# mrluin/TextualDegRemoval

Hardware: AMD Instinct MI355X
Metric: train images/sec (512x512, bs=4/GPU) (higher is better)
Workload: dtype f32 (3xbf16-split MFMA: 24-bit operand significands on the full fp32 exponent range, fp32 accumulate; unscaled gradients, no loss scale, no step-skip guard; tensors fp32 -- the MASA-encoder ResidualBlock activations / gradients as three bf16 planes whose sum IS the fp32 value, bit for bit)

## Files before the change

### include/tdr.h

```cpp
#ifndef TDR_H
#define TDR_H
#include <stdint.h>
#ifdef __cplusplus
extern "C" {
#endif

#define TDR_ABI_VERSION 110
int tdr_version(void);
const char* tdr_last_error(void);

typedef struct TdrStepGuard {
    float scale, inv_scale, max_scale;
    int good, growth_interval;
    int step, skipped, finite;
    float bc1, bc2_sqrt;
} TdrStepGuard;

typedef struct TdrConvDesc {
    int N, Cin, H, W;
    int Cout, OH, OW;
    int KH, stride, dil, pad;
    const float* in;  int64_t in_ns;
    int gate;
    const float* kscale; int64_t kscale_ns;
    const void* wp;  int64_t wp_ns;  int Mpad;
    int wp_fmt;
    float* out; int64_t out_ns;
    int epi;
    const float* bias;  int64_t bias_ns;
    const float* scale; int64_t scale_ns;
    const float* bias2; int64_t bias2_ns; float bias2_mul;
    const float* res;   int64_t res_ns;
    const float* mask;  int64_t mask_ns;
    const float* aux;   int64_t aux_ns;
    int relu;
} TdrConvDesc;

int tdr_conv_forward(const TdrConvDesc* d, void* stream);

int tdr_conv_ck(int KH_eff);
int64_t tdr_packed_weight_floats(int M, int Kch, int KH_eff);
int tdr_pack_weights(const float* w, int Cout, int Cin, int KH, int mode, float* wp, void* stream);
int64_t tdr_packed_weight_bytes_bx3(int M, int Kch, int KH_eff);
int tdr_pack_weights_bx3(const float* w, int Cout, int Cin, int KH, int mode, void* wp, void* stream);
int tdr_pack_weights_bx3_batch(const float* w, int64_t w_stride, int B, int Cout, int Cin, int KH, int mode, void* wp,
                               void* stream);
int64_t tdr_packed_weight_bytes_hx2(int M, int Kch, int KH_eff);
int tdr_pack_weights_hx2(const float* w, int Cout, int Cin, int KH, int mode, void* wp, void* stream);
int tdr_conv_force_cfg(int kh, int cfg);
typedef struct TdrPackJob {
    const float* w; void* wp;
    int Cout, Cin, KH, mode, fmt;
    int M, Kch, KHe, CK, Mx;
    int64_t total;
    int64_t first_block;
} TdrPackJob;
int tdr_pack_job_init(TdrPackJob* job, const float* w, int Cout, int Cin, int KH, int mode, int fmt, void* wp);
int tdr_pack_weights_multi(const TdrPackJob* jobs_dev, int n_jobs, int64_t total_blocks, void* stream);
int tdr_pack_patches(const float* blk, int B, int G, int C, int BH, int BW, int PH, int PW, int pstep, int dil,
                     int off, float* wp, void* stream);

typedef struct TdrConvP16Desc {
    int N, Cin, H, W, Cout;
    const void* in;
    const void* wp; int Mpad; int wp_fmt;
    const float* bias;
    const float* res32;  int64_t res32_ns;
    const void*  res16;
    const float* mask32; int64_t mask32_ns;
    const void*  mask16;
    int relu;
    float* out32; int64_t out32_ns;
    void*  out16;
} TdrConvP16Desc;
int64_t tdr_p16_bytes(int N, int C, int H, int W);
int tdr_p16_from_f32(const float* src, int64_t src_ns, int N, int C, int H, int W, void* dst, void* stream);
int tdr_p16_to_f32(const void* src, int N, int C, int H, int W, float* dst, int64_t dst_ns, void* stream);
int64_t tdr_p16_bytes_fmt(int N, int C, int H, int W, int fmt);
int tdr_p16_from_f32_fmt(const float* src, int64_t src_ns, int N, int C, int H, int W, void* dst, int fmt, void* stream);
int tdr_p16_to_f32_fmt(const void* src, int N, int C, int H, int W, float* dst, int64_t dst_ns, int fmt, void* stream);
int tdr_conv3x3_p16(const TdrConvP16Desc* d, void* stream);
int tdr_conv3x3_p16_force_cfg(int cfg);
typedef struct TdrWgradP16Desc {
    int N, Cin, H, W, Cout;
    const void* in16;
    const void* dout16;
    float* g;
    float* db;
    float* ws; int64_t ws_floats;
    int fmt;
} TdrWgradP16Desc;
int64_t tdr_wgrad3x3_p16_ws_floats(const TdrWgradP16Desc* d);
int tdr_wgrad3x3_p16(const TdrWgradP16Desc* d, void* stream);

typedef struct TdrWgradDesc {
    int N, Cin, H, W, Cout, OH, OW, KH, stride, pad;
    const float* in;   int64_t in_ns;  int gate;
    const float* dout; int64_t dout_ns;
    float* g;
    float* db;
    int per_image;
    float* ws; int64_t ws_floats;
    int math;
} TdrWgradDesc;
int64_t tdr_wgrad_ws_floats(const TdrWgradDesc* d);
int tdr_conv_wgrad(const TdrWgradDesc* d, void* stream);

typedef struct TdrWg1GroupEntry {
    const float* in; const float* dout; float* part; float* dbpart; float* g; float* db;
} TdrWg1GroupEntry;
int tdr_wgrad1x1_group_supported(const TdrWgradDesc* d);
int64_t tdr_wgrad1x1_group_ws_floats(const TdrWgradDesc* d, int nprob);
int tdr_wgrad1x1_group(const TdrWgradDesc* d, int nprob, const void* table, void* stream);

int64_t tdr_wgrad3x3_p16_group_ws_floats(const TdrWgradP16Desc* d, int nprob);
int tdr_wgrad3x3_p16_group_plan(const TdrWgradP16Desc* d, int nprob, int* nsplit, int* units, int* units_per_wg);
int tdr_wgrad3x3_p16_group(const TdrWgradP16Desc* d, int nprob, const void* table, void* stream);

int tdr_layernorm2d_fwd(const float* x, int64_t x_ns, const float* w, const float* b, float eps, int center,
                        int N, int C, int HW, float* y, float* mu, float* rstd, void* stream);
int64_t tdr_ln_ws_floats(int N, int C, int HW);
int tdr_layernorm2d_bwd(const float* go, const float* x, int64_t x_ns, const float* mu, const float* rstd,
                        const float* w, const float* add, int64_t add_ns, int add_C, int center,
                        int N, int C, int HW, float* gx, float* gw, float* gb, float* ws, void* stream);

int64_t tdr_dwsg_ws_floats(int N, int C, int H, int W);
int tdr_dwsg_fwd(const float* t, const float* w, const float* b, int N, int C, int H, int W,
                 float* g, float* pooled, float* ws, void* stream);
int tdr_dwsg_bwd(const float* dg, const float* t, const float* w, const float* b, int N, int C, int H, int W,
                 float* dt, float* dw, float* db, float* ws, void* stream);
int tdr_dwsg_bwd_biased(const float* dg, const float* dg_bias, float dg_bias_mul, const float* t, const float* w, const float* b,
                        int N, int C, int H, int W, float* dt, float* dw, float* db, float* ws, void* stream);
int tdr_dwsg_bwd_parts_supported(int W);
int tdr_dw_param_finish(const float* ws, int N, int C, int H, int W, float* dw , float* db , void* stream);

int tdr_dwgelu_fwd(const float* t, const float* w, const float* b, int N, int C, int H, int W, float* g, void* stream);
int tdr_dwgelu_bwd(const float* dg, const float* t, const float* w, const float* b, int N, int C, int H, int W,
                   float* dt, float* dw, float* db, float* ws, void* stream);
int tdr_dwconv_fwd(const float* t, const float* w, const float* b, int N, int planes, int H, int W, float* out,
                   void* stream);
int tdr_dwconv_bwd(const float* dout, const float* t, const float* w, int N, int planes, int H, int W, float* dt,
                   float* dw, float* db, float* ws, void* stream);
int tdr_dwconv_act_fwd(const float* t, const float* w, const float* b, int N, int planes, int H, int W, int relu, float* out,
                       void* stream);
int tdr_dwconv_act_bwd(const float* dout, const float* act, const float* t, const float* w, int N, int planes, int H, int W,
                       float* dt, float* dw, float* db, float* ws, void* stream);
int tdr_dwpair_fwd(const float* t, const float* w, const float* b, int N, int C, int H, int W, int relu, float* out,
                   int64_t out_ns, void* stream);
int tdr_dwpair_bwd(const float* dout, int64_t dout_ns, const float* act, int64_t act_ns, const float* t, const float* w, int N,
                   int C, int H, int W, float* dt, float* dw, float* db, float* ws, void* stream);
int tdr_dwconv_halves_fwd(const float* t, const float* w, const float* b, int N, int planes, int H, int W, int relu, float* outA,
                          float* outB, int64_t out_ns, void* stream);
int tdr_dwconv_halves_bwd(const float* doutA, const float* doutB, int64_t dout_ns, const float* actA, const float* actB,
                          int64_t act_ns, const float* t, const float* w, int N, int planes, int H, int W, float* dt, float* dw,
                          float* db, float* ws, void* stream);

int tdr_row_sumsq(const float* x, int64_t x_ns, int N, int rows, int HW, float* out, void* stream);
int tdr_mdta_pad(int C);
int tdr_mdta_softmax(const float* G, const float* ss, const float* temp, int N, int C, int heads, float* A, float* AT,
                     void* stream);
int tdr_mdta_bwd(const float* G, const float* ss, const float* temp, const float* A, const float* dA, int N, int C,
                 int heads, float* W, float* dtemp, float* ws, void* stream);
int tdr_attn_fold_proj(const float* AT, const float* Wo, int N, int C, int heads, float* Wf, void* stream);
int tdr_axpby_dev(const float* a, const float* alpha, const float* b, int64_t numel, float* out, void* stream);
int tdr_dot(const float* a, const float* b, int64_t numel, float* out, float* ws, void* stream);
int tdr_pixel_shuffle2(const float* in, int N, int C, int H, int W, float* out, void* stream);

int tdr_sca_fwd(const float* pooled, const float* wsca, const float* bsca, int N, int C, float* s, void* stream);
int tdr_sca_bwd(const float* G3, const float* S3, const float* w3, const float* b3, const float* beta,
                const float* s, const float* pooled, const float* wsca, int N, int C,
                float* dw3, float* db3, float* dbeta, float* dwsca, float* dbsca, float* dpooled,
                float* ws , void* stream);
int tdr_scaled_conv_param_grads(const float* G, const float* S, const float* w, const float* b,
                                const float* gamma, int Cout, int Cin, float* dw, float* db, float* dgamma,
                                void* stream);

int64_t tdr_chansum_ws_floats(int N, int C, int HW);
int tdr_channel_sum(const float* x, int64_t x_ns, int N, int C, int HW, float* out, float* ws, void* stream);

int tdr_copy_rows(const float* src, int64_t src_ns, float* dst, int64_t dst_ns, int N, int64_t len, void* stream);
int tdr_add_rows(const float* src, int64_t src_ns, float* dst, int64_t dst_ns, int N, int64_t len, void* stream);
int tdr_pixel_unshuffle2(const float* in, int N, int C, int H, int W, float* out, void* stream);
int tdr_pad_crop(const float* src, int N, int C, int Hs, int Ws, float* dst, int Hd, int Wd, void* stream);
int tdr_crop_augment(const float* src, int64_t src_ns, int N, int C, int Hs, int Ws, const int* top, const int* left,
                     const int* mode, const float* noise, const float* sigma, int P, float* out, void* stream);

int64_t tdr_ssim3d_ws_floats(int H, int W);
int tdr_ssim3d(const float* img1, const float* img2, int H, int W, int C, float max_value, float* ws, float* out,
// ... 309 lines not shown
```

### textualdegremoval_amd/_lib.py

```python
import ctypes as C
import os

import torch

_HERE = os.path.dirname(os.path.abspath(__file__))
LIB_PATH = os.environ.get('TDR_LIB_PATH', os.path.join(_HERE, 'libtdr_hip.so'))

ABI_VERSION = 110
c_fp = C.c_void_p
i32, i64, f32 = C.c_int, C.c_int64, C.c_float


class TdrConvDesc(C.Structure):
    _fields_ = [
        ('N', i32), ('Cin', i32), ('H', i32), ('W', i32),
        ('Cout', i32), ('OH', i32), ('OW', i32),
        ('KH', i32), ('stride', i32), ('dil', i32), ('pad', i32),
        ('inp', c_fp), ('in_ns', i64),
        ('gate', i32),
        ('kscale', c_fp), ('kscale_ns', i64),
        ('wp', c_fp), ('wp_ns', i64), ('Mpad', i32), ('wp_fmt', i32),
        ('out', c_fp), ('out_ns', i64),
        ('epi', i32),
        ('bias', c_fp), ('bias_ns', i64),
        ('scale', c_fp), ('scale_ns', i64),
        ('bias2', c_fp), ('bias2_ns', i64), ('bias2_mul', f32),
        ('res', c_fp), ('res_ns', i64),
        ('mask', c_fp), ('mask_ns', i64),
        ('aux', c_fp), ('aux_ns', i64),
        ('relu', i32),
    ]


class TdrConvP16Desc(C.Structure):
    _fields_ = [
        ('N', i32), ('Cin', i32), ('H', i32), ('W', i32), ('Cout', i32),
        ('inp', c_fp),
        ('wp', c_fp), ('Mpad', i32), ('wp_fmt', i32),
        ('bias', c_fp),
        ('res32', c_fp), ('res32_ns', i64),
        ('res16', c_fp),
        ('mask32', c_fp), ('mask32_ns', i64),
        ('mask16', c_fp),
        ('relu', i32),
        ('out32', c_fp), ('out32_ns', i64),
        ('out16', c_fp),
    ]


class TdrWgradP16Desc(C.Structure):
    _fields_ = [('N', i32), ('Cin', i32), ('H', i32), ('W', i32), ('Cout', i32),
                ('in16', c_fp), ('dout16', c_fp), ('g', c_fp), ('db', c_fp), ('ws', c_fp), ('ws_floats', i64), ('fmt', i32)]


class TdrPackJob(C.Structure):
    _fields_ = [
        ('w', c_fp), ('wp', c_fp),
        ('Cout', i32), ('Cin', i32), ('KH', i32), ('mode', i32), ('fmt', i32),
        ('M', i32), ('Kch', i32), ('KHe', i32), ('CK', i32), ('Mx', i32),
        ('total', i64), ('first_block', i64),
    ]


class TdrWgradDesc(C.Structure):
    _fields_ = [
        ('N', i32), ('Cin', i32), ('H', i32), ('W', i32), ('Cout', i32), ('OH', i32), ('OW', i32),
        ('KH', i32), ('stride', i32), ('pad', i32),
        ('inp', c_fp), ('in_ns', i64), ('gate', i32),
        ('dout', c_fp), ('dout_ns', i64),
        ('g', c_fp),
        ('db', c_fp),
        ('per_image', i32),
        ('ws', c_fp), ('ws_floats', i64),
        ('math', i32),
    ]


class TdrNafTailDesc(C.Structure):
    _fields_ = [('N', i32), ('C', i32), ('HW', i32), ('w_fmt', i32), ('c_out', i32), ('eps', f32),
                ('g', c_fp), ('g_ns', i64), ('sca', c_fp), ('x', c_fp), ('x_ns', i64),
                ('w3', c_fp), ('w4', c_fp), ('w5', c_fp),
                ('b3', c_fp), ('beta', c_fp), ('lnw', c_fp), ('lnb', c_fp), ('b4', c_fp), ('b5', c_fp), ('gamma', c_fp),
                ('y', c_fp), ('y_ns', i64), ('mu', c_fp), ('rs', c_fp), ('yn', c_fp), ('yn_ns', i64),
                ('t4', c_fp), ('t4_ns', i64), ('out', c_fp), ('out_ns', i64)]


class TdrNafTailBwdDesc(C.Structure):
    _fields_ = [('N', i32), ('C', i32), ('HW', i32), ('w_fmt', i32), ('c_out', i32),
                ('dout', c_fp), ('dout_ns', i64), ('gamma', c_fp), ('t4', c_fp), ('t4_ns', i64), ('y', c_fp), ('y_ns', i64),
                ('mu', c_fp), ('rs', c_fp), ('lnw', c_fp), ('w5t', c_fp), ('w4t', c_fp),
                ('dt4', c_fp), ('dt4_ns', i64), ('dy', c_fp), ('dy_ns', i64), ('gw', c_fp), ('gb', c_fp), ('ws', c_fp),
                ('w3t', c_fp), ('beta', c_fp), ('sca', c_fp), ('dgp', c_fp), ('dgp_ns', i64)]


class TdrNafHeadBwdDesc(C.Structure):
    _fields_ = [('N', i32), ('C', i32), ('HW', i32), ('w_fmt', i32),
                ('dt1', c_fp), ('dt1_ns', i64), ('x', c_fp), ('x_ns', i64), ('mu', c_fp), ('rs', c_fp), ('lnw', c_fp),
                ('w1t', c_fp), ('res', c_fp), ('res_ns', i64), ('dx', c_fp), ('dx_ns', i64), ('gw', c_fp), ('gb', c_fp), ('ws', c_fp)]


class TdrNafHeadFwdDesc(C.Structure):
    _fields_ = [('N', i32), ('C', i32), ('HW', i32), ('w_fmt', i32),
                ('x', c_fp), ('x_ns', i64), ('lnw', c_fp), ('lnb', c_fp), ('eps', f32), ('w1', c_fp), ('b1', c_fp),
                ('mu', c_fp), ('rs', c_fp), ('xn', c_fp), ('xn_ns', i64), ('t1', c_fp), ('t1_ns', i64)]


class TdrSfDynVecDesc(C.Structure):
    _fields_ = [('N', i32), ('c', i32), ('GK', i32), ('KK', i32), ('d', i32), ('eps', f32), ('momentum', f32)] + \
               [(k, c_fp) for k in ('ap', 'wconv', 'bn_w', 'bn_b', 'fc_w', 'fc_b', 'f0_w', 'f0_b', 'f1_w', 'f1_b', 'run_mean', 'run_var', 'nbt',
                                    'taps', 'ah', 'al', 'xhat', 'rstd', 'z', 'att')] + [('use_running', i32)]


class TdrSfDynVecBwdDesc(C.Structure):
    _fields_ = [('N', i32), ('c', i32), ('GK', i32), ('KK', i32), ('d', i32)] + \
               [(k, c_fp) for k in ('ap', 'wconv', 'bn_w', 'fc_w', 'f0_w', 'f1_w', 'taps', 'xhat', 'rstd', 'z', 'att', 'dtaps', 'dah', 'dal',
                                    'dap', 'g_wconv', 'g_bn_w', 'g_bn_b', 'g_fc_w', 'g_fc_b', 'g_f0_w', 'g_f0_b', 'g_f1_w', 'g_f1_b', 'ws')]


class TdrStepGuard(C.Structure):
    _fields_ = [('scale', f32), ('inv_scale', f32), ('max_scale', f32), ('good', i32), ('growth_interval', i32),
                ('step', i32), ('skipped', i32), ('finite', i32), ('bc1', f32), ('bc2_sqrt', f32)]


SIGNATURES = {
    'tdr_version': (i32, []),
    'tdr_last_error': (C.c_char_p, []),
    'tdr_conv_forward': (i32, [C.POINTER(TdrConvDesc), c_fp]),
    'tdr_conv_ck': (i32, [i32]),
    'tdr_ssim_y64_ws_doubles': (i64, [i32, i32]),
    'tdr_ssim_y64': (i32, [c_fp, c_fp, i32, i32, c_fp, c_fp, c_fp]),
    'tdr_local_avgpool_ws_floats': (i64, [i32, i32, i32, i32]),
    'tdr_local_avgpool': (i32, [c_fp, i32, i32, i32, i32, i32, c_fp, c_fp, c_fp]),
    'tdr_p16_bytes': (i64, [i32, i32, i32, i32]),
    'tdr_p16_bytes_fmt': (i64, [i32, i32, i32, i32, i32]),
    'tdr_p16_from_f32_fmt': (i32, [c_fp, i64, i32, i32, i32, i32, c_fp, i32, c_fp]),
    'tdr_p16_to_f32_fmt': (i32, [c_fp, i32, i32, i32, i32, c_fp, i64, i32, c_fp]),
    'tdr_p16_from_f32': (i32, [c_fp, i64, i32, i32, i32, i32, c_fp, c_fp]),
    'tdr_p16_to_f32': (i32, [c_fp, i32, i32, i32, i32, c_fp, i64, c_fp]),
    'tdr_conv3x3_p16': (i32, [C.POINTER(TdrConvP16Desc), c_fp]),
    'tdr_conv3x3_p16_force_cfg': (i32, [i32]),
    'tdr_wgrad3x3_p16_ws_floats': (i64, [C.POINTER(TdrWgradP16Desc)]),
    'tdr_wgrad3x3_p16': (i32, [C.POINTER(TdrWgradP16Desc), c_fp]),
    'tdr_packed_weight_floats': (i64, [i32, i32, i32]),
    'tdr_pack_weights': (i32, [c_fp, i32, i32, i32, i32, c_fp, c_fp]),
    'tdr_packed_weight_bytes_bx3': (i64, [i32, i32, i32]),
    'tdr_pack_weights_bx3': (i32, [c_fp, i32, i32, i32, i32, c_fp, c_fp]),
    'tdr_pack_job_init': (i32, [C.POINTER(TdrPackJob), c_fp, i32, i32, i32, i32, i32, c_fp]),
    'tdr_pack_weights_multi': (i32, [c_fp, i32, i64, c_fp]),
    'tdr_pack_patches': (i32, [c_fp, i32, i32, i32, i32, i32, i32, i32, i32, i32, i32, c_fp, c_fp]),
    'tdr_wgrad_ws_floats': (i64, [C.POINTER(TdrWgradDesc)]),
    'tdr_conv_wgrad': (i32, [C.POINTER(TdrWgradDesc), c_fp]),
    'tdr_wgrad1x1_group_supported': (i32, [C.POINTER(TdrWgradDesc)]),
    'tdr_wgrad1x1_group_ws_floats': (i64, [C.POINTER(TdrWgradDesc), i32]),
    'tdr_wgrad1x1_group': (i32, [C.POINTER(TdrWgradDesc), i32, c_fp, c_fp]),
    'tdr_wgrad3x3_p16_group_ws_floats': (i64, [C.POINTER(TdrWgradP16Desc), i32]),
    'tdr_wgrad3x3_p16_group_plan': (i32, [C.POINTER(TdrWgradP16Desc), i32, C.POINTER(i32), C.POINTER(i32), C.POINTER(i32)]),
    'tdr_wgrad3x3_p16_group': (i32, [C.POINTER(TdrWgradP16Desc), i32, c_fp, c_fp]),
    'tdr_layernorm2d_fwd': (i32, [c_fp, i64, c_fp, c_fp, f32, i32, i32, i32, i32, c_fp, c_fp, c_fp, c_fp]),
    'tdr_ln_ws_floats': (i64, [i32, i32, i32]),
    'tdr_layernorm2d_bwd': (i32, [c_fp, c_fp, i64, c_fp, c_fp, c_fp, c_fp, i64, i32, i32, i32, i32, i32, c_fp, c_fp, c_fp,
                                  c_fp, c_fp]),
    'tdr_dwsg_ws_floats': (i64, [i32, i32, i32, i32]),
    'tdr_dwsg_fwd': (i32, [c_fp, c_fp, c_fp, i32, i32, i32, i32, c_fp, c_fp, c_fp, c_fp]),
    'tdr_dwsg_bwd': (i32, [c_fp, c_fp, c_fp, c_fp, i32, i32, i32, i32, c_fp, c_fp, c_fp, c_fp, c_fp]),
    'tdr_dwsg_bwd_biased': (i32, [c_fp, c_fp, f32, c_fp, c_fp, c_fp, i32, i32, i32, i32, c_fp, c_fp, c_fp, c_fp, c_fp]),
    'tdr_dwsg_bwd_parts_supported': (i32, [i32]),
    'tdr_dw_param_finish': (i32, [c_fp, i32, i32, i32, i32, c_fp, c_fp, c_fp]),
    'tdr_dwgelu_fwd': (i32, [c_fp, c_fp, c_fp, i32, i32, i32, i32, c_fp, c_fp]),
    'tdr_dwgelu_bwd': (i32, [c_fp, c_fp, c_fp, c_fp, i32, i32, i32, i32, c_fp, c_fp, c_fp, c_fp, c_fp]),
    'tdr_dwconv_fwd': (i32, [c_fp, c_fp, c_fp, i32, i32, i32, i32, c_fp, c_fp]),
    'tdr_dwconv_act_fwd': (i32, [c_fp, c_fp, c_fp, i32, i32, i32, i32, i32, c_fp, c_fp]),
    'tdr_dwconv_act_bwd': (i32, [c_fp, c_fp, c_fp, c_fp, i32, i32, i32, i32, c_fp, c_fp, c_fp, c_fp, c_fp]),
    'tdr_dwpair_fwd': (i32, [c_fp, c_fp, c_fp, i32, i32, i32, i32, i32, c_fp, i64, c_fp]),
    'tdr_dwpair_bwd': (i32, [c_fp, i64, c_fp, i64, c_fp, c_fp, i32, i32, i32, i32, c_fp, c_fp, c_fp, c_fp, c_fp]),
    'tdr_dwconv_halves_fwd': (i32, [c_fp, c_fp, c_fp, i32, i32, i32, i32, i32, c_fp, c_fp, i64, c_fp]),
    'tdr_dwconv_halves_bwd': (i32, [c_fp, c_fp, i64, c_fp, c_fp, i64, c_fp, c_fp, i32, i32, i32, i32, c_fp, c_fp, c_fp, c_fp, c_fp]),
    'tdr_dwconv_bwd': (i32, [c_fp, c_fp, c_fp, i32, i32, i32, i32, c_fp, c_fp, c_fp, c_fp, c_fp]),
    'tdr_row_sumsq': (i32, [c_fp, i64, i32, i32, i32, c_fp, c_fp]),
    'tdr_mdta_pad': (i32, [i32]),
    'tdr_mdta_softmax': (i32, [c_fp, c_fp, c_fp, i32, i32, i32, c_fp, c_fp, c_fp]),
    'tdr_mdta_bwd': (i32, [c_fp, c_fp, c_fp, c_fp, c_fp, i32, i32, i32, c_fp, c_fp, c_fp, c_fp]),
    'tdr_attn_fold_proj': (i32, [c_fp, c_fp, i32, i32, i32, c_fp, c_fp]),
    'tdr_axpby_dev': (i32, [c_fp, c_fp, c_fp, i64, c_fp, c_fp]),
# ... 192 lines not shown
```

### textualdegremoval_amd/csrc/tdr_conv_bx3.hip

```cpp
#include <stdlib.h>
#include "tdr_common.h"
#include "tdr_conv_epi.h"
#include "tdr_pack.h"
#include "../../include/tdr.h"

typedef __bf16 bf16x8 __attribute__((ext_vector_type(8)));


namespace {

constexpr int bx_cmax(int a, int b) { return a > b ? a : b; }
constexpr int bx_plane(int NT, int TW, int KH, int S) {
    return (((NT * 32 / TW) - 1) * S + KH) * ((TW - 1) * S + KH);
}
constexpr int bx_max_plane(int NT, int KH, int S) {
    return bx_cmax(bx_plane(NT, 8, KH, S), bx_cmax(bx_plane(NT, 16, KH, S), bx_plane(NT, 32, KH, S)));
}

__device__ __forceinline__ void split3(float x, __bf16& h, __bf16& m, __bf16& l) {
    h = (__bf16)x;
    const float r = x - (float)h;
    m = (__bf16)r;
    l = (__bf16)(r - (float)m);
}

typedef _Float16 f16x8 __attribute__((ext_vector_type(8)));
union Frag {
    uint4 u;
    bf16x8 v;
    f16x8 hv;
};

enum { SCH_BX3 = 0, SCH_HX2 = 1, SCH_H1 = 2 };

#ifndef TDR_CONV_OCC
#define TDR_CONV_OCC 4
#endif
template <int KH, int S, int WM, int TM, int TN, int EPI, bool GATE, int SCH, int AD = 0>
__global__ __launch_bounds__(256, (KH == 3 && S == 1 && WM == 1 && TM == 1 && TN == 2 && AD != 9) ? TDR_CONV_OCC : ((KH == 3 && S == 1 && WM == 2 && TM == 1 && TN == 4 && AD == 3) ? 3 : 2)) void conv_bx3_kernel(ConvArgs a) {
    constexpr int NS = SCH == SCH_BX3 ? 3 : (SCH == SCH_HX2 ? 2 : 1);
    constexpr int NSW = SCH == SCH_BX3 ? 3 : 2;
    constexpr int NP = SCH == SCH_BX3 ? 6 : (SCH == SCH_HX2 ? 3 : 1);
    constexpr int WN = 4 / WM;
    constexpr int BM = 32 * TM * WM;
    constexpr int NT = TN * WN;
    constexpr int TAPS = KH * KH;
    constexpr int NIT = (bx_max_plane(NT, KH, S) + 127) / 128;
    constexpr int PF = (KH == 1) ? 2 : 1;
    static_assert(AD == 0 || (KH == 3 && 9 % AD == 0), "ring depth must divide the 9 taps");

    extern __shared__ __attribute__((aligned(16))) uint4 smem4[];

    const int tid = threadIdx.x, lane = tid & 63, wave = __builtin_amdgcn_readfirstlane(tid >> 6);
    const int wm = wave / WN, wn = wave % WN;
    const int j = lane & 31, kk = lane >> 5;
    const int TW = 1 << a.tw_log2, SR = 32 >> a.tw_log2, TH = NT * SR;
    const int LH = (TH - 1) * S + KH, LW = (TW - 1) * S + KH;
    const int plane = LH * LW;
    int logical;
    {
        const int T = gridDim.x, b = blockIdx.x;
        const int q = T >> 3, r = T & 7, xcd = b & 7, slot = b >> 3;
        logical = (xcd < r ? xcd * (q + 1) : r * (q + 1) + (xcd - r) * q) + slot;
    }
    const int mtile = logical % a.mtiles, ptile = logical / a.mtiles;
    const int tx = ptile % a.tiles_x, ty = ptile / a.tiles_x;
    const int m0 = mtile * BM;
    const int n = blockIdx.z;
    const int oy0 = ty * TH, ox0 = tx * TW;
    const int iy0 = oy0 * S - a.pad, ix0 = ox0 * S - a.pad;
    const long HWin = (long)a.H * a.W;

    const int sg = wave >> 1;
    const int sp0 = (wave & 1) * 64 + lane;
    int gsafe[NIT];
    unsigned okmask = 0, inplane = 0;
#pragma unroll
    for (int it = 0; it < NIT; ++it) {
        const int p = sp0 + 128 * it;
        const int r = p / LW, x = p - r * LW;
        const int gy = iy0 + r, gx = ix0 + x;
        const bool inp = p < plane;
        const bool ok = inp && gy >= 0 && gy < a.H && gx >= 0 && gx < a.W;
        gsafe[it] = ok ? gy * a.W + gx : 0;
        okmask |= (ok ? 1u : 0u) << it;
        inplane |= (inp ? 1u : 0u) << it;
    }
    const float* in_n = a.in + (long)n * a.in_ns;
    const float* ks_n = a.kscale ? a.kscale + (long)n * a.kscale_ns : nullptr;
    const int ngroups = (a.Cin + 15) >> 4;

    float rin[PF][NIT][8];
    float rin2[GATE ? PF : 1][GATE ? NIT : 1][GATE ? 8 : 1];
    float rks[PF][8];
    auto load_group = [&](int g, int set) {
#pragma unroll
        for (int i = 0; i < 8; ++i) {
            const int ci = min(g * 16 + sg * 8 + i, a.Cin - 1);
            const float* base = in_n + (long)ci * HWin;
            rks[set][i] = ks_n ? ks_n[ci] : 1.f;
#pragma unroll
            for (int it = 0; it < NIT; ++it) {
                rin[set][it][i] = base[gsafe[it]];
                if (GATE) rin2[set][it][i] = base[gsafe[it] + a.gate_off];
            }
        }
    };
    auto store_group = [&](int g, int set, int buf) {
        uint4* sb = smem4 + (buf * (2 * NS) + sg) * plane;
        const int cbase = g * 16 + sg * 8;
#pragma unroll
        for (int it = 0; it < NIT; ++it) {
            Frag h, m, l;
            const bool ok = (okmask >> it) & 1u;
            float vv[8];
#pragma unroll
            for (int i = 0; i < 8; ++i) {
                float v = rin[set][it][i];
                if (GATE) v *= rin2[set][it][i];
                v *= rks[set][i];
                vv[i] = (ok && cbase + i < a.Cin) ? v : 0.f;
            }
            if constexpr (SCH == SCH_HX2) {
                unsigned hd[4], md[4];
#pragma unroll
                for (int i = 0; i < 4; ++i) tdr_split2_f16(vv[2 * i], vv[2 * i + 1], hd[i], md[i]);
                h.u = make_uint4(hd[0], hd[1], hd[2], hd[3]);
                m.u = make_uint4(md[0], md[1], md[2], md[3]);
            } else {
#pragma unroll
                for (int i = 0; i < 8; ++i) {
                    float v = vv[i];
                    asm volatile("" : "+v"(v));
                    if constexpr (SCH == SCH_H1) {
                        h.hv[i] = (_Float16)v;
                    } else {
                        __bf16 hh, mm, ll;
                        split3(v, hh, mm, ll);
                        h.v[i] = hh; m.v[i] = mm; l.v[i] = ll;
                    }
                }
            }
            if ((inplane >> it) & 1u) {
                const int p = sp0 + 128 * it;
                sb[p] = h.u;
                if constexpr (NS >= 2) sb[2 * plane + p] = m.u;
                if constexpr (NS == 3) sb[4 * plane + p] = l.u;
            }
        }
    };

    int bbase[TN];
#pragma unroll
    for (int tn = 0; tn < TN; ++tn) {
        const int t = wn * TN + tn;
        const int py = t * SR + (j >> a.tw_log2), px = j & (TW - 1);
        bbase[tn] = kk * plane + py * S * LW + px * S;
    }
    const int MT = a.Mpad >> 5;
    const uint4* wfrag[TM];
#pragma unroll
    for (int tm = 0; tm < TM; ++tm) {
        const int mt = min((m0 >> 5) + wm * TM + tm, MT - 1);
        wfrag[tm] = reinterpret_cast<const uint4*>(a.wp) + (long)n * (a.wp_ns >> 2) + (long)mt * (NSW * 64) + lane;
    }
    const long wstep = (long)MT * (NSW * 64);

    f32x16 acc[TM][TN];
#pragma unroll
    for (int tm = 0; tm < TM; ++tm)
#pragma unroll
        for (int tn = 0; tn < TN; ++tn)
#pragma unroll
            for (int r = 0; r < 16; ++r) acc[tm][tn][r] = 0.f;

    Frag af[TM][NS], afn[TM][NS];
    Frag aq[AD > 0 ? AD : 1][TM][NS];
    auto load_a = [&](Frag (&dst)[TM][NS], long gt) {
#pragma unroll
        for (int tm = 0; tm < TM; ++tm)
#pragma unroll
            for (int s = 0; s < NS; ++s) dst[tm][s].u = wfrag[tm][gt * wstep + s * 64];
    };

    if constexpr (AD > 0) {
#pragma unroll
        for (int d = 0; d < AD; ++d) load_a(aq[d], min((long)d, (long)ngroups * TAPS - 1));
    } else {
        load_a(af, 0);
    }
#pragma unroll
    for (int p = 0; p < PF; ++p)
        if (p < ngroups) load_group(p, p);
    store_group(0, 0, 0);
    __syncthreads();

    for (int g0 = 0; g0 < ngroups; g0 += PF) {
#pragma unroll
        for (int u = 0; u < PF; ++u) {
            const int g = g0 + u;
            if (g < ngroups) {
                const int buf = a.single_buf ? 0 : (g & 1);
                const uint4* sb = smem4 + buf * (2 * NS) * plane;
                constexpr int IGT = (PF == 1 && KH == 3 && AD > 0 && AD < TAPS) ? TAPS - AD : -1;
                if (PF == 1 && IGT < 0 && g + 1 < ngroups) load_group(g + 1, 0);
#pragma unroll
                for (int tap = 0; tap < TAPS; ++tap) {
                    const int tapoff = (tap / KH) * LW + (tap % KH);
                    if (tap == IGT && g + 1 < ngroups) {
                        load_group(g + 1, 0);
                        __builtin_amdgcn_sched_barrier(0);
                    }
                    const long gtn = min((long)g * TAPS + tap + 1, (long)ngroups * TAPS - 1);
                    if (AD == 0) load_a(afn, gtn);
                    Frag (&afc)[TM][NS] = AD > 0 ? aq[AD > 0 ? tap % (AD > 0 ? AD : 1) : 0] : af;
                    if (PF > 1 && tap == 0 && g + PF < ngroups) load_group(g + PF, u);
                    Frag bf[TN][NS];
#pragma unroll
                    for (int tn = 0; tn < TN; ++tn)
#pragma unroll
                        for (int s = 0; s < NS; ++s) bf[tn][s].u = sb[s * 2 * plane + bbase[tn] + tapoff];
                    constexpr int SA[6] = {2, 0, 1, 1, 0, 0}, SB[6] = {0, 2, 1, 0, 1, 0};
                    constexpr int HA[3] = {1, 0, 0}, HB[3] = {0, 1, 0};
#pragma unroll
                    for (int q = 0; q < NP; ++q)
#pragma unroll
                        for (int tm = 0; tm < TM; ++tm)
#pragma unroll
                            for (int tn = 0; tn < TN; ++tn) {
                                if constexpr (SCH == SCH_H1)
                                    acc[tm][tn] = __builtin_amdgcn_mfma_f32_32x32x16_f16(afc[tm][0].hv, bf[tn][0].hv, acc[tm][tn], 0, 0, 0);
                                else if constexpr (SCH == SCH_HX2)
                                    acc[tm][tn] = __builtin_amdgcn_mfma_f32_32x32x16_f16(afc[tm][HA[q]].hv, bf[tn][HB[q]].hv, acc[tm][tn], 0, 0, 0);
                                else
                                    acc[tm][tn] = __builtin_amdgcn_mfma_f32_32x32x16_bf16(afc[tm][SA[q]].v, bf[tn][SB[q]].v, acc[tm][tn], 0, 0, 0);
                            }
                    if constexpr (AD > 0) {
                        load_a(aq[tap % (AD > 0 ? AD : 1)], min((long)g * TAPS + tap + AD, (long)ngroups * TAPS - 1));
                    } else {
#pragma unroll
                        for (int tm = 0; tm < TM; ++tm)
#pragma unroll
                            for (int s = 0; s < NS; ++s) af[tm][s] = afn[tm][s];
                    }
                }
                {
                    if (a.single_buf) __syncthreads();
                    if (g + 1 < ngroups) store_group(g + 1, (u + 1) % PF, a.single_buf ? 0 : (buf ^ 1));
                    __syncthreads();
                }
            }
        }
    }

    if constexpr (EPI != EPI_PSHUF) {
        if (a.vec_epi) {
            __syncthreads();
            conv_epilogue_vec<TM, TN, EPI>(a, acc, n, m0, wm, wn, oy0, ox0, lane, reinterpret_cast<float*>(smem4) + wave * (32 * 36));
            return;
        }
    }
    conv_epilogue<TM, TN, EPI>(a, acc, n, m0, wm, wn, oy0, ox0, j, kk);
}

__device__ __forceinline__ int swz1(int slot) { return slot ^ ((slot >> 4) & 3); }

template <int WM, int TM, int TN, int EPI, bool GATE, int SCH = SCH_HX2>
__global__ __launch_bounds__(256, 2) void conv1x1_hx2_kernel(ConvArgs a) {
    constexpr int NS = SCH == SCH_H1 ? 1 : 2, NSW = 2, NP = SCH == SCH_H1 ? 1 : 3;
    constexpr int WN = 4 / WM;
    constexpr int BM = 32 * TM * WM;
    constexpr int NT = TN * WN;
    constexpr int NPX = 32 * NT;
    constexpr int QUADS = NPX / 4;
    constexpr int OCT = 256 / QUADS;
    constexpr int KS = 8 * OCT;
    constexpr int GPS = KS / 16;
    constexpr int PFD = GATE ? 1 : 2;

    extern __shared__ __attribute__((aligned(16))) uint4 smem4[];

    const int tid = threadIdx.x, lane = tid & 63, wave = __builtin_amdgcn_readfirstlane(tid >> 6);
    const int wm = wave / WN, wn = wave % WN;
    const int j = lane & 31, kk = lane >> 5;
    const int TW = 1 << a.tw_log2, SR = 32 >> a.tw_log2, TH = NT * SR;
    int logical;
    {
        const int T = gridDim.x, b = blockIdx.x;
        const int q = T >> 3, r = T & 7, xcd = b & 7, slot = b >> 3;
        logical = (xcd < r ? xcd * (q + 1) : r * (q + 1) + (xcd - r) * q) + slot;
    }
    const int mtile = logical % a.mtiles, ptile = logical / a.mtiles;
    const int tx = ptile % a.tiles_x, ty = ptile / a.tiles_x;
    const int m0 = mtile * BM;
    const int n = blockIdx.z;
    const int oy0 = ty * TH, ox0 = tx * TW;
    const long HWin = (long)a.H * a.W;

    const int so = tid / QUADS, sq = tid % QUADS;
    const int p0 = 4 * sq;
    const int gy = oy0 + (p0 >> a.tw_log2), gx = ox0 + (p0 & (TW - 1));
    const bool pok = gy < a.H && gx < a.W;
    const long goff = pok ? (long)gy * a.W + gx : 0;
    const float* in_n = a.in + (long)n * a.in_ns;
    const float* ks_n = a.kscale ? a.kscale + (long)n * a.kscale_ns : nullptr;
    const int ngroups = (a.Cin + 15) >> 4;
    const int nstages = (a.Cin + KS - 1) / KS;

    float4 rin[PFD][8];
    float4 rin2[GATE ? PFD : 1][GATE ? 8 : 1];
    float rks[PFD][8];
    auto load_stage = [&](int st, int set) {
        const int cbase = st * KS + so * 8;
#pragma unroll
        for (int i = 0; i < 8; ++i) {
            const int ci = cbase + i;
            rin[set][i] = make_float4(0.f, 0.f, 0.f, 0.f);
            rks[set][i] = 1.f;
            if (GATE) rin2[set][i] = make_float4(0.f, 0.f, 0.f, 0.f);
            if (pok && ci < a.Cin) {
                const float* src = in_n + (long)ci * HWin + goff;
                rin[set][i] = *reinterpret_cast<const float4*>(src);
                if (GATE) rin2[set][i] = *reinterpret_cast<const float4*>(src + a.gate_off);
                if (ks_n) rks[set][i] = ks_n[ci];
            }
        }
    };
    int wslot[4];
#pragma unroll
    for (int i = 0; i < 4; ++i) wslot[i] = so * NPX + swz1(p0 + i);
    auto store_stage = [&](int set, int buf) {
        uint4* sb = smem4 + buf * (NS * OCT * NPX);
#pragma unroll
        for (int px = 0; px < 4; ++px) {
            Frag h, m;
            float vv[8];
#pragma unroll
            for (int i = 0; i < 8; ++i) {
                const float4 q4 = rin[set][i];
                float v = px == 0 ? q4.x : (px == 1 ? q4.y : (px == 2 ? q4.z : q4.w));
                if (GATE) {
                    const float4 g4 = rin2[set][i];
                    v *= px == 0 ? g4.x : (px == 1 ? g4.y : (px == 2 ? g4.z : g4.w));
                }
                vv[i] = v * rks[set][i];
            }
            if constexpr (NS == 2) {
                unsigned hd[4], md[4];
#pragma unroll
                for (int i = 0; i < 4; ++i) tdr_split2_f16(vv[2 * i], vv[2 * i + 1], hd[i], md[i]);
                h.u = make_uint4(hd[0], hd[1], hd[2], hd[3]);
                m.u = make_uint4(md[0], md[1], md[2], md[3]);
            } else {
#pragma unroll
                for (int i = 0; i < 8; ++i) h.hv[i] = (_Float16)vv[i];
            }
            sb[wslot[px]] = h.u;
            if constexpr (NS == 2) sb[OCT * NPX + wslot[px]] = m.u;
        }
    };

    int bslot[TN];
#pragma unroll
    for (int tn = 0; tn < TN; ++tn) bslot[tn] = kk * NPX + swz1(32 * (wn * TN + tn) + j);
    const int MT = a.Mpad >> 5;
    const uint4* wfrag[TM];
#pragma unroll
    for (int tm = 0; tm < TM; ++tm) {
        const int mt = min((m0 >> 5) + wm * TM + tm, MT - 1);
        wfrag[tm] = reinterpret_cast<const uint4*>(a.wp) + (long)n * (a.wp_ns >> 2) + (long)mt * (NSW * 64) + lane;
    }
    const long wstep = (long)MT * (NSW * 64);

    f32x16 acc[TM][TN];
#pragma unroll
    for (int tm = 0; tm < TM; ++tm)
#pragma unroll
        for (int tn = 0; tn < TN; ++tn)
#pragma unroll
            for (int r = 0; r < 16; ++r) acc[tm][tn][r] = 0.f;

    Frag af[TM][NS], afn[TM][NS];
    auto load_a = [&](Frag (&dst)[TM][NS], long g) {
#pragma unroll
        for (int tm = 0; tm < TM; ++tm)
#pragma unroll
            for (int s = 0; s < NS; ++s) dst[tm][s].u = wfrag[tm][g * wstep + s * 64];
    };

    load_a(af, 0);
#pragma unroll
    for (int p = 0; p < PFD; ++p)
        if (p < nstages) load_stage(p, p);
    store_stage(0, 0);
    __syncthreads();

    for (int s0 = 0; s0 < nstages; s0 += PFD) {
#pragma unroll
        for (int u = 0; u < PFD; ++u) {
            const int st = s0 + u;
            if (st < nstages) {
                const int buf = st & 1;
                const uint4* sb = smem4 + buf * (NS * OCT * NPX);
#pragma unroll
                for (int gg = 0; gg < GPS; ++gg) {
                    const int g = st * GPS + gg;
                    if (g < ngroups) {
                        load_a(afn, min(g + 1, ngroups - 1));
                        if (gg == 0 && st + PFD < nstages) load_stage(st + PFD, u);
                        Frag bf[TN][NS];
#pragma unroll
                        for (int tn = 0; tn < TN; ++tn)
#pragma unroll
                            for (int s = 0; s < NS; ++s) bf[tn][s].u = sb[s * (OCT * NPX) + 2 * gg * NPX + bslot[tn]];
                        constexpr int HA[3] = {1, 0, 0}, HB[3] = {0, 1, 0};
#pragma unroll
                        for (int q = 0; q < NP; ++q)
#pragma unroll
                            for (int tm = 0; tm < TM; ++tm)
#pragma unroll
                                for (int tn = 0; tn < TN; ++tn) {
                                    if constexpr (SCH == SCH_H1)
                                        acc[tm][tn] = __builtin_amdgcn_mfma_f32_32x32x16_f16(af[tm][0].hv, bf[tn][0].hv, acc[tm][tn], 0, 0, 0);
                                    else
                                        acc[tm][tn] = __builtin_amdgcn_mfma_f32_32x32x16_f16(af[tm][HA[q]].hv, bf[tn][HB[q]].hv, acc[tm][tn], 0, 0, 0);
                                }
#pragma unroll
                        for (int tm = 0; tm < TM; ++tm)
#pragma unroll
                            for (int s = 0; s < NS; ++s) af[tm][s] = afn[tm][s];
                    }
                }
                if (st + 1 < nstages) store_stage((u + 1) % PFD, buf ^ 1);
                __syncthreads();
            }
        }
    }

    if constexpr (EPI != EPI_PSHUF) {
        if (a.vec_epi) {
            conv_epilogue_vec<TM, TN, EPI>(a, acc, n, m0, wm, wn, oy0, ox0, lane, reinterpret_cast<float*>(smem4) + wave * (32 * 36));
            return;
        }
    }
    conv_epilogue<TM, TN, EPI>(a, acc, n, m0, wm, wn, oy0, ox0, j, kk);
}

template <int WM, int TM, int TN, int EPI, bool GATE, int SCH>
int launch_c1_hx2(const ConvArgs& a, int N, hipStream_t st) {
    constexpr int WN = 4 / WM;
    constexpr int BM = 32 * TM * WM;
    constexpr int NT = TN * WN;
    const int TW = 1 << a.tw_log2, SR = 32 >> a.tw_log2, TH = NT * SR;
    ConvArgs b = a;
    b.tiles_x = tdr_cdiv(a.OW, TW);
    const int tiles_y = tdr_cdiv(a.OH, TH);
    b.mtiles = tdr_cdiv(a.Cout, BM);
    dim3 grid(b.tiles_x * tiles_y * b.mtiles, 1, N);
    b.single_buf = 0;
    const size_t lds = 2 * 32768;
    auto kern = conv1x1_hx2_kernel<WM, TM, TN, EPI, GATE, SCH>;
    static bool attr_set = false;
    if (!attr_set) {
        (void)hipFuncSetAttribute(reinterpret_cast<const void*>(kern), hipFuncAttributeMaxDynamicSharedMemorySize, 160 * 1024);
        attr_set = true;
    }
    hipLaunchKernelGGL(kern, grid, dim3(256), lds, st, b);
    TDR_LAUNCH_CHECK("conv1x1_hx2_kernel");
    return TDR_OK;
}

inline bool c1_hx2_ok(const ConvArgs& a, int npx, int bm, int N) {
    static const bool off = tdr_tune_env("TDR_C1_OLD") != nullptr;
    static const int min_stages = tdr_tune_env("TDR_C1_STAGES") ? atoi(tdr_tune_env("TDR_C1_STAGES")) : 4;
    static const long max_blocks = tdr_tune_env("TDR_C1_BLOCKS") ? atol(tdr_tune_env("TDR_C1_BLOCKS")) : 512;
    const int ks = 8192 / npx;
    const long blocks = (long)tdr_cdiv((long)a.OH * a.OW, npx) * tdr_cdiv(a.Cout, bm) * N;
    return !off && blocks <= max_blocks && (a.Cin + ks - 1) / ks >= min_stages && a.pad == 0 && a.W % 4 == 0 && a.in_ns % 4 == 0 && (reinterpret_cast<uintptr_t>(a.in) & 15) == 0 &&
           a.H == a.OH && a.W == a.OW;
}

template <int KH, int S, int WM, int TM, int TN, int EPI, bool GATE, int SCH>
int launch_bx_cfg_s(const ConvArgs& a, int N, hipStream_t st) {
    if constexpr (KH == 1 && S == 1 && SCH != SCH_BX3 && EPI != EPI_PSHUF)
        if (c1_hx2_ok(a, 32 * TN * (4 / WM), 32 * TM * WM, N)) return launch_c1_hx2<WM, TM, TN, EPI, GATE, SCH>(a, N, st);
    constexpr int NS = SCH == SCH_BX3 ? 3 : (SCH == SCH_HX2 ? 2 : 1);
    constexpr int WN = 4 / WM;
    constexpr int BM = 32 * TM * WM;
    constexpr int NT = TN * WN;
    const int TW = 1 << a.tw_log2, SR = 32 >> a.tw_log2, TH = NT * SR;
    const int LH = (TH - 1) * S + KH, LW = (TW - 1) * S + KH;
    ConvArgs b = a;
    static const int single_env = tdr_tune_env("TDR_BX_SINGLE") ? atoi(tdr_tune_env("TDR_BX_SINGLE")) : 2;
    b.single_buf = (KH == 3 && (a.Cin + 15) / 16 <= single_env) ? 1 : 0;
    size_t lds = (size_t)(b.single_buf ? 1 : 2) * (2 * NS) * LH * LW * 16;
    if (lds < 4 * 32 * 36 * sizeof(float)) lds = 4 * 32 * 36 * sizeof(float);
    b.tiles_x = tdr_cdiv(a.OW, TW);
    const int tiles_y = tdr_cdiv(a.OH, TH);
    b.mtiles = tdr_cdiv(a.Cout, BM);
    dim3 grid(b.tiles_x * tiles_y * b.mtiles, 1, N);
    if constexpr (KH == 3 && S == 1 && SCH == SCH_HX2 && EPI == EPI_STD && !GATE) {
        static const int ring3 = tdr_tune_env("TDR_RING3") ? atoi(tdr_tune_env("TDR_RING3")) : 1;
        static const long ring_blocks3 = tdr_tune_env("TDR_RING_BLOCKS") ? atol(tdr_tune_env("TDR_RING_BLOCKS")) : 512;
        if (ring3 && ((long)grid.x * N > ring_blocks3 || TM != 1)) {
            auto kern = conv_bx3_kernel<KH, S, WM, TM, TN, EPI, GATE, SCH, 3>;
            static bool attr_set = false;
            if (!attr_set) {
                (void)hipFuncSetAttribute(reinterpret_cast<const void*>(kern), hipFuncAttributeMaxDynamicSharedMemorySize, 160 * 1024);
                attr_set = true;
            }
            hipLaunchKernelGGL(kern, grid, dim3(256), lds, st, b);
            TDR_LAUNCH_CHECK("conv_bx3_kernel(ring3)");
            return TDR_OK;
        }
    }
    if constexpr (KH == 3 && S == 1 && TM == 1 && SCH == SCH_HX2 && EPI == EPI_STD) {
        static const long ring_blocks = tdr_tune_env("TDR_RING_BLOCKS") ? atol(tdr_tune_env("TDR_RING_BLOCKS")) : 512;
        if ((long)grid.x * N <= ring_blocks) {
            auto kern = conv_bx3_kernel<KH, S, WM, TM, TN, EPI, GATE, SCH, 9>;
            static bool attr_set = false;
            if (!attr_set) {
                (void)hipFuncSetAttribute(reinterpret_cast<const void*>(kern), hipFuncAttributeMaxDynamicSharedMemorySize, 160 * 1024);
                attr_set = true;
            }
            hipLaunchKernelGGL(kern, grid, dim3(256), lds, st, b);
            TDR_LAUNCH_CHECK("conv_bx3_kernel(ring)");
            return TDR_OK;
        }
    }
    auto kern = conv_bx3_kernel<KH, S, WM, TM, TN, EPI, GATE, SCH>;
    static bool attr_set = false;
    if (!attr_set) {
        (void)hipFuncSetAttribute(reinterpret_cast<const void*>(kern), hipFuncAttributeMaxDynamicSharedMemorySize, 160 * 1024);
        attr_set = true;
    }
    hipLaunchKernelGGL(kern, grid, dim3(256), lds, st, b);
    TDR_LAUNCH_CHECK("conv_bx3_kernel");
    return TDR_OK;
}

int g_force_cfg[2] = {tdr_tune_env("TDR_BX_CFG1") ? atoi(tdr_tune_env("TDR_BX_CFG1")) : 0, tdr_tune_env("TDR_BX_CFG3") ? atoi(tdr_tune_env("TDR_BX_CFG3")) : 0};

template <int KH, int S, int WM, int TM, int TN, int EPI, bool GATE>
int launch_bx_cfg(const ConvArgs& a, int N, hipStream_t st) {
    if (a.scheme == SCH_HX2) return launch_bx_cfg_s<KH, S, WM, TM, TN, EPI, GATE, SCH_HX2>(a, N, st);
    if (a.scheme == SCH_H1) return launch_bx_cfg_s<KH, S, WM, TM, TN, EPI, GATE, SCH_H1>(a, N, st);
    return launch_bx_cfg_s<KH, S, WM, TM, TN, EPI, GATE, SCH_BX3>(a, N, st);
}

template <int KH, int S, int EPI, bool GATE>
int launch_bx_shape(const ConvArgs& a, int N, hipStream_t st) {
    const long pix = (long)a.OH * a.OW;
    auto blocks = [&](int bm, int bn) { return (long)tdr_cdiv(a.Cout, bm) * tdr_cdiv(pix, bn) * N; };
    if constexpr (S == 2) {
        if (a.Cout <= 32) return launch_bx_cfg<KH, S, 1, 1, 1, EPI, GATE>(a, N, st);
        if (a.Cout <= 64 || blocks(128, 64) < 512) return launch_bx_cfg<KH, S, 2, 1, 1, EPI, GATE>(a, N, st);
        return launch_bx_cfg<KH, S, 2, 2, 1, EPI, GATE>(a, N, st);
    } else {
        if (a.Cout <= 32) {
            if (blocks(32, 256) >= 512) return launch_bx_cfg<KH, S, 1, 1, 2, EPI, GATE>(a, N, st);
            return launch_bx_cfg<KH, S, 1, 1, 1, EPI, GATE>(a, N, st);
        }
        if (g_force_cfg[KH == 1 ? 0 : 1] == 0 && a.scheme == SCH_BX3 && a.Cin <= (KH == 1 ? 128 : 64) && blocks(64, 128) >= 2048)
            return launch_bx_cfg<KH, S, 2, 1, 2, EPI, GATE>(a, N, st);
        if constexpr (KH == 1) {
            const int force = g_force_cfg[0];
            if (force == 1) return launch_bx_cfg<KH, S, 2, 2, 2, EPI, GATE>(a, N, st);
            if (force == 2) return launch_bx_cfg<KH, S, 2, 1, 4, EPI, GATE>(a, N, st);
            if (force == 3) return launch_bx_cfg<KH, S, 2, 1, 2, EPI, GATE>(a, N, st);
            if (force == 4) return launch_bx_cfg<KH, S, 1, 1, 2, EPI, GATE>(a, N, st);
            if (force == 5) return launch_bx_cfg<KH, S, 4, 2, 2, EPI, GATE>(a, N, st);
            if (a.Cout > 64 && blocks(128, 128) >= 512) return launch_bx_cfg<KH, S, 2, 2, 2, EPI, GATE>(a, N, st);
            if (a.Cin >= 768 && a.Cout >= 256 && blocks(256, 64) >= 256 && blocks(256, 64) <= 512)
                return launch_bx_cfg<KH, S, 4, 2, 2, EPI, GATE>(a, N, st);
        } else {
            const int force3 = g_force_cfg[1];
            if (force3 == 1) return launch_bx_cfg<KH, S, 2, 2, 4, EPI, GATE>(a, N, st);
            if (force3 == 2) return launch_bx_cfg<KH, S, 2, 1, 4, EPI, GATE>(a, N, st);
            if (force3 == 3) return launch_bx_cfg<KH, S, 2, 1, 2, EPI, GATE>(a, N, st);
            if (force3 == 4) return launch_bx_cfg<KH, S, 2, 2, 2, EPI, GATE>(a, N, st);
            const bool tall_ok = blocks(128, 256) >= 1024 || a.Cout % 128 != 0 || a.scheme != SCH_HX2;
            if (a.Cout > 64 && blocks(128, 256) >= 512 && tall_ok) return launch_bx_cfg<KH, S, 2, 2, 4, EPI, GATE>(a, N, st);
        }
        if (blocks(64, 256) >= 512) return launch_bx_cfg<KH, S, 2, 1, 4, EPI, GATE>(a, N, st);
        return launch_bx_cfg<KH, S, 2, 1, 2, EPI, GATE>(a, N, st);
    }
}

__global__ void pack_weights_bx3_kernel(const float* __restrict__ w, long w_bs, int Cout, int Cin, int KH, int mode, int M,
                                        int Kch, int KHe, int MT, long total, uint4* __restrict__ wp, long wp_bs16) {
    const float* wb = w + (long)blockIdx.y * w_bs;
    uint4* ob = wp + (long)blockIdx.y * wp_bs16;
    for (long i = blockIdx.x * (long)blockDim.x + threadIdx.x; i < total; i += (long)gridDim.x * blockDim.x)
        tdr_pack_bx3_frag(wb, Cin, KH, mode, M, Kch, KHe, MT, i, ob);
}

__global__ void pack_weights_hx2_kernel(const float* __restrict__ w, int Cout, int Cin, int KH, int mode, int M, int Kch, int KHe,
                                        int MT, long total, uint4* __restrict__ wp) {
    for (long i = blockIdx.x * (long)blockDim.x + threadIdx.x; i < total; i += (long)gridDim.x * blockDim.x)
        tdr_pack_hx2_frag(w, Cin, KH, mode, M, Kch, KHe, MT, i, wp);
}

}

extern "C" int tdr_conv_force_cfg(int kh, int cfg) {
    g_force_cfg[kh == 1 ? 0 : 1] = cfg;
    return TDR_OK;
}

extern "C" int64_t tdr_packed_weight_bytes_bx3(int M, int Kch, int KH_eff) {
    const long MT = (M + 31) / 32;
    return (long)((Kch + 15) / 16) * KH_eff * KH_eff * MT * 3 * 1024;
}

extern "C" int tdr_pack_weights_bx3(const float* w, int Cout, int Cin, int KH, int mode, void* wp, void* stream) {
    TDR_REQUIRE(w && wp, "tdr_pack_weights_bx3: null pointer");
    TDR_REQUIRE(mode >= 0 && mode <= 3, "tdr_pack_weights_bx3: bad mode %d", mode);
    int M, Kch, KHe;
    if (mode == 0) { M = Cout; Kch = Cin; KHe = KH; }
    else if (mode == 1) { M = Cin; Kch = Cout; KHe = KH; }
    else if (mode == 2) { TDR_REQUIRE(KH == 2, "mode 2 needs a 2x2 kernel"); M = 4 * Cin; Kch = Cout; KHe = 1; }
    else { TDR_REQUIRE(KH == 3, "mode 3 needs a 3x3 kernel"); M = 4 * Cin; Kch = Cout; KHe = 2; }
    const int MT = (M + 31) / 32;
    const long total = (long)((Kch + 15) / 16) * KHe * KHe * MT * 64;
    const int blocks = (int)((total + 255) / 256 < 4096 ? (total + 255) / 256 : 4096);
    hipLaunchKernelGGL(pack_weights_bx3_kernel, dim3(blocks), dim3(256), 0, (hipStream_t)stream, w, 0L, Cout, Cin, KH, mode, M,
                       Kch, KHe, MT, total, (uint4*)wp, 0L);
    TDR_LAUNCH_CHECK("pack_weights_bx3_kernel");
    return TDR_OK;
}

extern "C" int64_t tdr_packed_weight_bytes_hx2(int M, int Kch, int KH_eff) {
    const long MT = (M + 31) / 32;
    return (long)((Kch + 15) / 16) * KH_eff * KH_eff * MT * 2 * 1024;
}

extern "C" int tdr_pack_weights_hx2(const float* w, int Cout, int Cin, int KH, int mode, void* wp, void* stream) {
    TDR_REQUIRE(w && wp, "tdr_pack_weights_hx2: null pointer");
    TDR_REQUIRE(mode >= 0 && mode <= 3, "tdr_pack_weights_hx2: bad mode %d", mode);
    int M, Kch, KHe;
    if (mode == 0) { M = Cout; Kch = Cin; KHe = KH; }
    else if (mode == 1) { M = Cin; Kch = Cout; KHe = KH; }
    else if (mode == 2) { TDR_REQUIRE(KH == 2, "mode 2 needs a 2x2 kernel"); M = 4 * Cin; Kch = Cout; KHe = 1; }
    else { TDR_REQUIRE(KH == 3, "mode 3 needs a 3x3 kernel"); M = 4 * Cin; Kch = Cout; KHe = 2; }
    const int MT = (M + 31) / 32;
    const long total = (long)((Kch + 15) / 16) * KHe * KHe * MT * 64;
    const int blocks = (int)((total + 255) / 256 < 4096 ? (total + 255) / 256 : 4096);
    hipLaunchKernelGGL(pack_weights_hx2_kernel, dim3(blocks), dim3(256), 0, (hipStream_t)stream, w, Cout, Cin, KH, mode, M, Kch,
                       KHe, MT, total, (uint4*)wp);
    TDR_LAUNCH_CHECK("pack_weights_hx2_kernel");
    return TDR_OK;
}

extern "C" int tdr_pack_weights_bx3_batch(const float* w, int64_t w_stride, int B, int Cout, int Cin, int KH, int mode, void* wp,
                                          void* stream) {
    TDR_REQUIRE(w && wp && B > 0, "tdr_pack_weights_bx3_batch: bad argument");
    TDR_REQUIRE(mode == 0 || mode == 1, "tdr_pack_weights_bx3_batch: mode 0 or 1 only (got %d)", mode);
    const int M = mode == 0 ? Cout : Cin, Kch = mode == 0 ? Cin : Cout;
    const int MT = (M + 31) / 32;
    const long total = (long)((Kch + 15) / 16) * KH * KH * MT * 64;
    const long per_b16 = tdr_packed_weight_bytes_bx3(M, Kch, KH) / 16;
    const int blocks = (int)((total + 255) / 256 < 1024 ? (total + 255) / 256 : 1024);
    hipLaunchKernelGGL(pack_weights_bx3_kernel, dim3(blocks, B), dim3(256), 0, (hipStream_t)stream, w, (long)w_stride, Cout, Cin,
                       KH, mode, M, Kch, KH, MT, total, (uint4*)wp, per_b16);
    TDR_LAUNCH_CHECK("pack_weights_bx3_kernel(batch)");
    return TDR_OK;
}

int tdr_conv_forward_bx3(const TdrConvDesc* d, void* stream) {
    TDR_REQUIRE(d->dil == 1 && d->wp_ns % 4 == 0, "tdr_conv_forward: split-bf16 path needs dil=1 (and wp_ns a multiple of 4 floats)");
    ConvArgs a;
    a.in = d->in; a.in_ns = d->in_ns; a.Cin = d->Cin; a.H = d->H; a.W = d->W;
    a.wp = (const float*)d->wp; a.wp_ns = d->wp_ns; a.Mpad = d->Mpad; a.Cout = d->Cout;
    a.scheme = d->wp_fmt == 3 ? SCH_H1 : (d->wp_fmt == 2 ? SCH_HX2 : SCH_BX3);
    a.out = d->out; a.out_ns = d->out_ns; a.OH = d->OH; a.OW = d->OW;
    a.pad = d->pad;
    a.tw_log2 = d->OW >= 24 ? 5 : (d->OW >= 12 ? 4 : 3);
    a.tiles_x = 0;
    a.kscale = d->kscale; a.kscale_ns = d->kscale_ns;
    a.gate_off = (long)d->Cin * d->H * d->W;
    a.bias = d->bias; a.bias_ns = d->bias_ns; a.scale = d->scale; a.scale_ns = d->scale_ns;
    a.bias2 = d->bias2; a.bias2_ns = d->bias2_ns; a.bias2_mul = d->bias2_mul;
    a.res = d->res; a.res_ns = d->res_ns; a.mask = d->mask; a.mask_ns = d->mask_ns;
    a.aux = d->aux; a.aux_ns = d->aux_ns; a.relu = d->relu;
    auto al16 = [](const void* p) { return (reinterpret_cast<uintptr_t>(p) & 15) == 0; };
    a.vec_epi = (d->OW % 4 == 0 && d->out_ns % 4 == 0 && al16(d->out) && (!d->res || (d->res_ns % 4 == 0 && al16(d->res))) &&
                 (!d->mask || (d->mask_ns % 4 == 0 && al16(d->mask))) && (!d->aux || (d->aux_ns % 4 == 0 && al16(d->aux)))) ? 1 : 0;
    hipStream_t st = (hipStream_t)stream;
    const int N = d->N;
    const int key = d->KH * 100 + d->stride * 10 + d->epi;
    const bool g = d->gate != 0;
    switch (key) {
        case 110: return g ? launch_bx_shape<1, 1, EPI_STD, true>(a, N, st) : launch_bx_shape<1, 1, EPI_STD, false>(a, N, st);
        case 111: if (!g) return launch_bx_shape<1, 1, EPI_GATEBWD, false>(a, N, st); break;
        case 112: if (!g) return launch_bx_shape<1, 1, EPI_PSHUF, false>(a, N, st); break;
        case 310: if (!g) return launch_bx_shape<3, 1, EPI_STD, false>(a, N, st); break;
        case 312: if (!g) return launch_bx_shape<3, 1, EPI_PSHUF, false>(a, N, st); break;
        case 320: if (!g) return launch_bx_shape<3, 2, EPI_STD, false>(a, N, st); break;
        case 220: if (!g) return launch_bx_shape<2, 2, EPI_STD, false>(a, N, st); break;
        case 212: if (!g) return launch_bx_shape<2, 1, EPI_PSHUF, false>(a, N, st); break;
        default: break;
    }
    tdr_set_error("tdr_conv_forward(bx3): unsupported (KH=%d stride=%d epi=%d gate=%d)", d->KH, d->stride, d->epi, d->gate);
    return TDR_ERR_UNSUPPORTED;
}
```

### textualdegremoval_amd/csrc/tdr_conv_epi.h

```cpp
#pragma once
#include "tdr_common.h"

namespace {

enum { EPI_STD = 0, EPI_GATEBWD = 1, EPI_PSHUF = 2 };

struct ConvArgs {
    const float* in; long in_ns; int Cin, H, W;
    const float* wp; long wp_ns; int Mpad, Cout;
    float* out; long out_ns; int OH, OW;
    int pad, tw_log2, tiles_x, mtiles;
    const float* kscale; long kscale_ns;
    long gate_off;
    const float* bias; long bias_ns;
    const float* scale; long scale_ns;
    const float* bias2; long bias2_ns; float bias2_mul;
    const float* res; long res_ns;
    const float* mask; long mask_ns;
    const float* aux; long aux_ns;
    int relu;
    int vec_epi;
    int single_buf;
    int scheme;
};

template <int TM, int TN, int EPI>
__device__ __forceinline__ void conv_epilogue(const ConvArgs& a, f32x16 (&acc)[TM][TN], int n, int m0, int wm, int wn,
                                              int oy0, int ox0, int j, int kk) {
    const int TW = 1 << a.tw_log2, SR = 32 >> a.tw_log2;
    const long HWo = (long)a.OH * a.OW;
#pragma unroll
    for (int tn = 0; tn < TN; ++tn) {
        const int t = wn * TN + tn;
        const int oy = oy0 + t * SR + (j >> a.tw_log2), ox = ox0 + (j & (TW - 1));
        const bool pvalid = oy < a.OH && ox < a.OW;
        const long pix = pvalid ? (long)oy * a.OW + ox : 0;
#pragma unroll
        for (int tm = 0; tm < TM; ++tm) {
            const int mb = m0 + (wm * TM + tm) * 32 + 4 * kk;
            if (EPI == EPI_PSHUF) {
                const long OW2 = 2L * a.OW;
                const long p2 = pvalid ? (2L * oy) * OW2 + 2L * ox : 0;
                float2 r0[4], r1[4];
                if (a.res) {
#pragma unroll
                    for (int q = 0; q < 4; ++q) {
                        const int c = min(mb + 8 * q, a.Cout - 4) >> 2;
                        const float* rp = a.res + (long)n * a.res_ns + (long)c * 4 * HWo + p2;
                        r0[q] = *reinterpret_cast<const float2*>(rp);
                        r1[q] = *reinterpret_cast<const float2*>(rp + OW2);
                    }
                }
#pragma unroll
                for (int q = 0; q < 4; ++q) {
                    const int m = mb + 8 * q;
                    float v0 = acc[tm][tn][4 * q + 0], v1 = acc[tm][tn][4 * q + 1];
                    float v2 = acc[tm][tn][4 * q + 2], v3 = acc[tm][tn][4 * q + 3];
                    if (a.res) { v0 += r0[q].x; v1 += r0[q].y; v2 += r1[q].x; v3 += r1[q].y; }
                    if (pvalid && m < a.Cout) {
                        float* o = a.out + (long)n * a.out_ns + (long)(m >> 2) * 4 * HWo + p2;
                        *reinterpret_cast<float2*>(o) = make_float2(v0, v1);
                        *reinterpret_cast<float2*>(o + OW2) = make_float2(v2, v3);
                    }
                }
            } else if (EPI == EPI_GATEBWD) {
                const float* ax = a.aux + (long)n * a.aux_ns;
                const long half = (long)a.Cout * HWo;
                float a0[16], a1[16];
#pragma unroll
                for (int r = 0; r < 16; ++r) {
                    const int mc = min(mb + (r & 3) + 8 * (r >> 2), a.Cout - 1);
                    const long o = (long)mc * HWo + pix;
                    a0[r] = ax[o];
                    a1[r] = ax[o + half];
                }
                float* op = a.out + (long)n * a.out_ns;
#pragma unroll
                for (int r = 0; r < 16; ++r) {
                    const int m = mb + (r & 3) + 8 * (r >> 2);
                    if (pvalid && m < a.Cout) {
                        const long o = (long)m * HWo + pix;
                        const float v = acc[tm][tn][r];
                        op[o] = v * a1[r];
                        op[o + half] = v * a0[r];
                    }
                }
            } else {
                float v[16];
#pragma unroll
                for (int r = 0; r < 16; ++r) v[r] = acc[tm][tn][r];
                if (a.bias) {
                    float tv[16];
#pragma unroll
                    for (int r = 0; r < 16; ++r) tv[r] = a.bias[(long)n * a.bias_ns + min(mb + (r & 3) + 8 * (r >> 2), a.Cout - 1)];
#pragma unroll
                    for (int r = 0; r < 16; ++r) v[r] += tv[r];
                }
                if (a.scale) {
                    float tv[16];
#pragma unroll
                    for (int r = 0; r < 16; ++r) tv[r] = a.scale[(long)n * a.scale_ns + min(mb + (r & 3) + 8 * (r >> 2), a.Cout - 1)];
#pragma unroll
                    for (int r = 0; r < 16; ++r) v[r] *= tv[r];
                }
                if (a.bias2) {
                    float tv[16];
#pragma unroll
                    for (int r = 0; r < 16; ++r) tv[r] = a.bias2[(long)n * a.bias2_ns + min(mb + (r & 3) + 8 * (r >> 2), a.Cout - 1)];
#pragma unroll
                    for (int r = 0; r < 16; ++r) v[r] += a.bias2_mul * tv[r];
                }
                if (a.res) {
                    float tv[16];
#pragma unroll
                    for (int r = 0; r < 16; ++r)
                        tv[r] = a.res[(long)n * a.res_ns + (long)min(mb + (r & 3) + 8 * (r >> 2), a.Cout - 1) * HWo + pix];
#pragma unroll
                    for (int r = 0; r < 16; ++r) v[r] += tv[r];
                }
                if (a.relu == 1) {
#pragma unroll
                    for (int r = 0; r < 16; ++r) v[r] = fmaxf(v[r], 0.f);
                } else if (a.relu == 2) {
#pragma unroll
                    for (int r = 0; r < 16; ++r) v[r] = 0.5f * v[r] * (1.f + erff(v[r] * 0.70710678118654752f));
                } else if (a.relu == 3) {
#pragma unroll
                    for (int r = 0; r < 16; ++r) v[r] = v[r] / (1.f + expf(-1.702f * v[r]));
                }
                if (a.mask) {
                    float tv[16];
#pragma unroll
                    for (int r = 0; r < 16; ++r)
                        tv[r] = a.mask[(long)n * a.mask_ns + (long)min(mb + (r & 3) + 8 * (r >> 2), a.Cout - 1) * HWo + pix];
#pragma unroll
                    for (int r = 0; r < 16; ++r) v[r] = tv[r] > 0.f ? v[r] : 0.f;
                }
                float* op = a.out + (long)n * a.out_ns + pix;
#pragma unroll
                for (int r = 0; r < 16; ++r) {
                    const int m = mb + (r & 3) + 8 * (r >> 2);
                    if (pvalid && m < a.Cout) op[(long)m * HWo] = v[r];
                }
            }
        }
    }
}


template <int TM, int TN, int EPI>
__device__ __forceinline__ void conv_epilogue_vec(const ConvArgs& a, f32x16 (&acc)[TM][TN], int n, int m0, int wm, int wn,
                                                  int oy0, int ox0, int lane, float* sw) {
    static_assert(EPI == EPI_STD || EPI == EPI_GATEBWD, "vector epilogue: STD / GATEBWD");
    const int j = lane & 31, kk = lane >> 5;
    const int TW = 1 << a.tw_log2, SR = 32 >> a.tw_log2;
    const long HWo = (long)a.OH * a.OW;
    const int c4 = (lane & 7) * 4;
    const int r0 = lane >> 3;
    const f32x4 z4 = {0.f, 0.f, 0.f, 0.f};
#pragma unroll
    for (int tn = 0; tn < TN; ++tn) {
        const int t = wn * TN + tn;
        const int oy = oy0 + t * SR + (c4 >> a.tw_log2), ox = ox0 + (c4 & (TW - 1));
        const bool pvalid = oy < a.OH && ox < a.OW;
        const long pix = pvalid ? (long)oy * a.OW + ox : 0;
#pragma unroll
        for (int tm = 0; tm < TM; ++tm) {
#pragma unroll
            for (int r = 0; r < 16; ++r) sw[((r & 3) + 8 * (r >> 2) + 4 * kk) * 36 + j] = acc[tm][tn][r];
            f32x4 v[4];
            int mrow[4];
#pragma unroll
            for (int i = 0; i < 4; ++i) {
                v[i] = *reinterpret_cast<const f32x4*>(sw + (r0 + 8 * i) * 36 + c4);
                mrow[i] = m0 + (wm * TM + tm) * 32 + r0 + 8 * i;
            }
            if (EPI == EPI_GATEBWD) {
                const float* ax = a.aux + (long)n * a.aux_ns;
                const long half = (long)a.Cout * HWo;
                f32x4 a0[4], a1[4];
#pragma unroll
                for (int i = 0; i < 4; ++i) {
                    const long o = (long)min(mrow[i], a.Cout - 1) * HWo + pix;
                    a0[i] = *reinterpret_cast<const f32x4*>(ax + o);
                    a1[i] = *reinterpret_cast<const f32x4*>(ax + o + half);
                }
                float* op = a.out + (long)n * a.out_ns;
#pragma unroll
                for (int i = 0; i < 4; ++i)
                    if (pvalid && mrow[i] < a.Cout) {
                        const long o = (long)mrow[i] * HWo + pix;
                        *reinterpret_cast<f32x4*>(op + o) = v[i] * a1[i];
                        *reinterpret_cast<f32x4*>(op + o + half) = v[i] * a0[i];
                    }
            } else {
                f32x4 rv[4], mv[4];
                if (a.res) {
#pragma unroll
                    for (int i = 0; i < 4; ++i)
                        rv[i] = *reinterpret_cast<const f32x4*>(a.res + (long)n * a.res_ns + (long)min(mrow[i], a.Cout - 1) * HWo + pix);
                }
                if (a.mask) {
#pragma unroll
                    for (int i = 0; i < 4; ++i)
                        mv[i] = *reinterpret_cast<const f32x4*>(a.mask + (long)n * a.mask_ns + (long)min(mrow[i], a.Cout - 1) * HWo + pix);
                }
#pragma unroll
                for (int i = 0; i < 4; ++i) {
                    const int mc = min(mrow[i], a.Cout - 1);
                    f32x4 x = v[i];
                    if (a.bias) x += a.bias[(long)n * a.bias_ns + mc];
                    if (a.scale) x *= a.scale[(long)n * a.scale_ns + mc];
                    if (a.bias2) x += a.bias2_mul * a.bias2[(long)n * a.bias2_ns + mc];
                    if (a.res) x += rv[i];
                    if (a.relu == 1) {
#pragma unroll
                        for (int e = 0; e < 4; ++e) x[e] = fmaxf(x[e], 0.f);
                    } else if (a.relu == 2) {
#pragma unroll
                        for (int e = 0; e < 4; ++e) x[e] = 0.5f * x[e] * (1.f + erff(x[e] * 0.70710678118654752f));
                    } else if (a.relu == 3) {
#pragma unroll
                        for (int e = 0; e < 4; ++e) x[e] = x[e] / (1.f + expf(-1.702f * x[e]));
                    }
                    if (a.mask) {
#pragma unroll
                        for (int e = 0; e < 4; ++e) x[e] = mv[i][e] > 0.f ? x[e] : 0.f;
                    }
                    if (pvalid && mrow[i] < a.Cout)
                        *reinterpret_cast<f32x4*>(a.out + (long)n * a.out_ns + (long)mrow[i] * HWo + pix) = x;
                }
            }
        }
    }
    (void)z4;
}

}
```

### textualdegremoval_amd/csrc/tdr_conv_mfma.hip

```cpp
#include "tdr_common.h"
#include "tdr_conv_epi.h"
#include "tdr_pack.h"
#include "../../include/tdr.h"

namespace {

constexpr int cmax(int a, int b) { return a > b ? a : b; }
constexpr int plane_elems(int NT, int TW, int KH, int S, int D) {
    return (((NT * 32 / TW) - 1) * S + (KH - 1) * D + 1) * ((TW - 1) * S + (KH - 1) * D + 1);
}
constexpr int max_plane(int NT, int KH, int S, int D) {
    return cmax(plane_elems(NT, 8, KH, S, D), cmax(plane_elems(NT, 16, KH, S, D), plane_elems(NT, 32, KH, S, D)));
}

template <int KH, int S, int D, int CK, int WM, int TM, int TN, int EPI, bool GATE>
__global__ __launch_bounds__(256) void conv_mfma_kernel(ConvArgs a) {
    constexpr int WN = 4 / WM;
    constexpr int BM = 32 * TM * WM;
    constexpr int NT = TN * WN;
    constexpr int TAPS = KH * KH;
    constexpr int KC = CK * TAPS;
    constexpr int MAXPIT = (max_plane(NT, KH, S, D) + 63) / 64;
    constexpr int CPW = CK / 4;
    constexpr int W4 = KC * BM / 4;
// ... 92 lines not shown
        const int t = wn * TN + tn;
        const int py = t * SR + (j >> a.tw_log2), px = j & (TW - 1);
        bbase[tn] = kk * plane + py * S * LW + px * S;
    }
    const int abase = kk * BM + wm * TM * 32 + j;

    f32x16 acc[TM][TN];
#pragma unroll
    for (int tm = 0; tm < TM; ++tm)
#pragma unroll
        for (int tn = 0; tn < TN; ++tn)
#pragma unroll
            for (int r = 0; r < 16; ++r) acc[tm][tn][r] = 0.f;

    load_chunk(0);
    for (int ch = 0; ch < nchunks; ++ch) {
        {
            __syncthreads();
            store_chunk(ch);
            __syncthreads();
        }
        if (ch + 1 < nchunks) load_chunk(ch + 1);
#pragma unroll
        for (int tap = 0; tap < TAPS; ++tap) {
            const int tapoff = (tap / KH) * D * LW + (tap % KH) * D;
#pragma unroll
            for (int c2 = 0; c2 < CK / 2; ++c2) {
                float af[TM], bf[TN];
#pragma unroll
                for (int tm = 0; tm < TM; ++tm)
                    af[tm] = s_w[abase + (tap * CK + 2 * c2) * BM + tm * 32];
#pragma unroll
                for (int tn = 0; tn < TN; ++tn)
                    bf[tn] = s_in[bbase[tn] + 2 * c2 * plane + tapoff];
#pragma unroll
                for (int tm = 0; tm < TM; ++tm)
#pragma unroll
                    for (int tn = 0; tn < TN; ++tn)
                        acc[tm][tn] = __builtin_amdgcn_mfma_f32_32x32x2f32(af[tm], bf[tn], acc[tm][tn], 0, 0, 0);
            }
        }
    }

    conv_epilogue<TM, TN, EPI>(a, acc, n, m0, wm, wn, oy0, ox0, j, kk);
}

template <int KH, int S, int D, int CK, int WM, int TM, int TN, int EPI, bool GATE>
int launch_cfg(const ConvArgs& a, int N, hipStream_t st) {
    constexpr int WN = 4 / WM;
    constexpr int BM = 32 * TM * WM;
    constexpr int NT = TN * WN;
    constexpr int KC = CK * KH * KH;
    const int TW = 1 << a.tw_log2, SR = 32 >> a.tw_log2, TH = NT * SR;
    const int LH = (TH - 1) * S + (KH - 1) * D + 1, LW = (TW - 1) * S + (KH - 1) * D + 1;
    const size_t lds = (size_t)(KC * BM + CK * LH * LW) * sizeof(float);
    ConvArgs b = a;
    b.tiles_x = tdr_cdiv(a.OW, TW);
    const int tiles_y = tdr_cdiv(a.OH, TH);
    dim3 grid(b.tiles_x * tiles_y, tdr_cdiv(a.Cout, BM), N);
    auto kern = conv_mfma_kernel<KH, S, D, CK, WM, TM, TN, EPI, GATE>;
    static bool attr_set = false;
    if (!attr_set) {
        (void)hipFuncSetAttribute(reinterpret_cast<const void*>(kern), hipFuncAttributeMaxDynamicSharedMemorySize, 160 * 1024);
        attr_set = true;
    }
    hipLaunchKernelGGL(kern, grid, dim3(256), lds, st, b);
    TDR_LAUNCH_CHECK("conv_mfma_kernel");
    return TDR_OK;
}

template <int KH, int S, int D, int CK, int EPI, bool GATE>
int launch_shape(const ConvArgs& a, int N, hipStream_t st) {
    const long pix = (long)a.OH * a.OW;
    auto blocks = [&](int bm, int bn) { return (long)tdr_cdiv(a.Cout, bm) * tdr_cdiv(pix, bn) * N; };
    if (a.Cout <= 32) {
        if (blocks(32, 256) < 256) return launch_cfg<KH, S, D, CK, 1, 1, 1, EPI, GATE>(a, N, st);
        return launch_cfg<KH, S, D, CK, 1, 1, 2, EPI, GATE>(a, N, st);
    }
    if (a.Cout > 64 && blocks(128, 128) >= 512) return launch_cfg<KH, S, D, CK, 2, 2, 2, EPI, GATE>(a, N, st);
    if (blocks(64, 128) >= 512) return launch_cfg<KH, S, D, CK, 2, 1, 2, EPI, GATE>(a, N, st);
    return launch_cfg<KH, S, D, CK, 2, 1, 1, EPI, GATE>(a, N, st);
}

__global__ void pack_weights_kernel(const float* __restrict__ w, int Cout, int Cin, int KH, int mode, int CK,
                                    int M, int Kch, int KHe, int Mpad, long total, float* __restrict__ wp) {
    for (long i = blockIdx.x * (long)blockDim.x + threadIdx.x; i < total; i += (long)gridDim.x * blockDim.x)
        wp[i] = tdr_pack_f32_elem(w, Cin, KH, mode, CK, M, Kch, KHe, Mpad, i);
}

__global__ void pack_patches_kernel(const float* __restrict__ blk, int G, int C, int BH, int BW, int PH, int PW, int pstep,
                                    int dil, int off, int CK, int Mpad, long per_b, long total, float* __restrict__ wp) {
    for (long i = blockIdx.x * (long)blockDim.x + threadIdx.x; i < total; i += (long)gridDim.x * blockDim.x) {
        const long b = i / per_b;
        long r = i % per_b;
        const int m = (int)(r % Mpad); r /= Mpad;
        const int ck = (int)(r % CK); r /= CK;
        const int tap = (int)(r % 9);
        const int chunk = (int)(r / 9);
        const int c = chunk * CK + ck;
        float v = 0.f;
        if (m < G * PH * PW && c < C) {
            const int g = m / (PH * PW), q = m % (PH * PW);
            const int py = q / PW, px = q % PW;
            const int y = py * pstep + (tap / 3) * dil + off, x = px * pstep + (tap % 3) * dil + off;
            v = blk[(((b * G + g) * C + c) * BH + y) * BW + x];
        }
        wp[i] = v;
    }
}

}

extern "C" int tdr_conv_ck(int KH_eff) { return KH_eff == 1 ? 32 : (KH_eff == 2 ? 16 : 8); }

extern "C" int64_t tdr_packed_weight_floats(int M, int Kch, int KH_eff) {
    const int CK = tdr_conv_ck(KH_eff);
    const long Mpad = (M + 31) / 32 * 32;
    return (long)((Kch + CK - 1) / CK) * KH_eff * KH_eff * CK * Mpad;
}

extern "C" int tdr_pack_weights(const float* w, int Cout, int Cin, int KH, int mode, float* wp, void* stream) {
    TDR_REQUIRE(w && wp, "tdr_pack_weights: null pointer");
    TDR_REQUIRE(mode >= 0 && mode <= 3, "tdr_pack_weights: bad mode %d", mode);
    int M, Kch, KHe;
    if (mode == 0) { M = Cout; Kch = Cin; KHe = KH; }
    else if (mode == 1) { M = Cin; Kch = Cout; KHe = KH; }
    else if (mode == 2) { TDR_REQUIRE(KH == 2, "mode 2 needs a 2x2 kernel"); M = 4 * Cin; Kch = Cout; KHe = 1; }
    else { TDR_REQUIRE(KH == 3, "mode 3 needs a 3x3 kernel"); M = 4 * Cin; Kch = Cout; KHe = 2; }
    const int CK = tdr_conv_ck(KHe);
    const int Mpad = (M + 31) / 32 * 32;
    const long total = tdr_packed_weight_floats(M, Kch, KHe);
    const int blocks = (int)((total + 255) / 256 < 4096 ? (total + 255) / 256 : 4096);
    hipLaunchKernelGGL(pack_weights_kernel, dim3(blocks), dim3(256), 0, (hipStream_t)stream, w, Cout, Cin, KH, mode, CK,
                       M, Kch, KHe, Mpad, total, wp);
    TDR_LAUNCH_CHECK("pack_weights_kernel");
    return TDR_OK;
}

extern "C" int tdr_pack_patches(const float* blk, int B, int G, int C, int BH, int BW, int PH, int PW, int pstep, int dil,
                                int off, float* wp, void* stream) {
    TDR_REQUIRE(blk && wp, "tdr_pack_patches: null pointer");
    const int CK = 8;
    const int Mpad = (G * PH * PW + 31) / 32 * 32;
    const long per_b = (long)((C + CK - 1) / CK) * 9 * CK * Mpad;
    const long total = per_b * B;
    const int blocks = (int)((total + 255) / 256 < 8192 ? (total + 255) / 256 : 8192);
    hipLaunchKernelGGL(pack_patches_kernel, dim3(blocks), dim3(256), 0, (hipStream_t)stream, blk, G, C, BH, BW, PH, PW,
                       pstep, dil, off, CK, Mpad, per_b, total, wp);
    TDR_LAUNCH_CHECK("pack_patches_kernel");
    return TDR_OK;
}

extern "C" int tdr_conv_forward(const TdrConvDesc* d, void* stream) {
    TDR_REQUIRE(d && d->in && d->wp && d->out, "tdr_conv_forward: null pointer");
    TDR_REQUIRE(d->N > 0 && d->Cin > 0 && d->Cout > 0 && d->OH > 0 && d->OW > 0, "tdr_conv_forward: bad shape");
    TDR_REQUIRE(d->Mpad % 32 == 0 && d->Mpad >= d->Cout, "tdr_conv_forward: Mpad %d invalid for Cout %d", d->Mpad, d->Cout);
    TDR_REQUIRE(d->epi != EPI_GATEBWD || d->aux, "tdr_conv_forward: GATEBWD needs aux");
    if (d->wp_fmt >= 1 && d->wp_fmt <= 3) return tdr_conv_forward_bx3(d, stream);
    TDR_REQUIRE(d->wp_fmt == 0, "tdr_conv_forward: unknown wp_fmt %d", d->wp_fmt);
    ConvArgs a;
    a.in = d->in; a.in_ns = d->in_ns; a.Cin = d->Cin; a.H = d->H; a.W = d->W;
    a.wp = (const float*)d->wp; a.wp_ns = d->wp_ns; a.Mpad = d->Mpad; a.Cout = d->Cout;
    a.out = d->out; a.out_ns = d->out_ns; a.OH = d->OH; a.OW = d->OW;
    a.pad = d->pad;
    a.tw_log2 = d->OW >= 24 ? 5 : (d->OW >= 12 ? 4 : 3);
    a.tiles_x = 0;
    a.kscale = d->kscale; a.kscale_ns = d->kscale_ns;
    a.gate_off = (long)d->Cin * d->H * d->W;
    a.bias = d->bias; a.bias_ns = d->bias_ns; a.scale = d->scale; a.scale_ns = d->scale_ns;
    a.bias2 = d->bias2; a.bias2_ns = d->bias2_ns; a.bias2_mul = d->bias2_mul;
    a.res = d->res; a.res_ns = d->res_ns; a.mask = d->mask; a.mask_ns = d->mask_ns;
    a.aux = d->aux; a.aux_ns = d->aux_ns; a.relu = d->relu;
    a.vec_epi = 0; a.single_buf = 0; a.scheme = 0;
    hipStream_t st = (hipStream_t)stream;
    const int N = d->N;
    const int key = d->KH * 1000 + d->stride * 100 + d->dil * 10 + d->epi;
    const bool g = d->gate != 0;
    switch (key) {
        case 1110: return g ? launch_shape<1, 1, 1, 32, EPI_STD, true>(a, N, st)
                            : launch_shape<1, 1, 1, 32, EPI_STD, false>(a, N, st);
        case 1111: if (!g) return launch_shape<1, 1, 1, 32, EPI_GATEBWD, false>(a, N, st); break;
        case 1112: if (!g) return launch_shape<1, 1, 1, 32, EPI_PSHUF, false>(a, N, st); break;
        case 3110: if (!g) return launch_shape<3, 1, 1, 8, EPI_STD, false>(a, N, st); break;
        case 3112: if (!g) return launch_shape<3, 1, 1, 8, EPI_PSHUF, false>(a, N, st); break;
        case 3120: if (!g) return launch_shape<3, 1, 2, 8, EPI_STD, false>(a, N, st); break;
        case 3130: if (!g) return launch_shape<3, 1, 3, 8, EPI_STD, false>(a, N, st); break;
        case 3210: if (!g) return launch_shape<3, 2, 1, 8, EPI_STD, false>(a, N, st); break;
        case 2210: if (!g) return launch_shape<2, 2, 1, 16, EPI_STD, false>(a, N, st); break;
        case 2112: if (!g) return launch_shape<2, 1, 1, 16, EPI_PSHUF, false>(a, N, st); break;
        default: break;
    }
    tdr_set_error("tdr_conv_forward: unsupported (KH=%d stride=%d dil=%d epi=%d gate=%d)", d->KH, d->stride, d->dil,
                  d->epi, d->gate);
    return TDR_ERR_UNSUPPORTED;
}

namespace {
__global__ __launch_bounds__(256) void pack_multi_kernel(const TdrPackJob* __restrict__ jobs, int n_jobs) {
    int lo = 0, hi = n_jobs - 1;
    while (lo < hi) {
        const int mid = (lo + hi + 1) >> 1;
        if (jobs[mid].first_block <= (long)blockIdx.x) lo = mid; else hi = mid - 1;
    }
    const TdrPackJob jb = jobs[lo];
    const long i = ((long)blockIdx.x - jb.first_block) * 256 + threadIdx.x;
    if (i >= jb.total) return;
    if (jb.fmt == 0)
        reinterpret_cast<float*>(jb.wp)[i] = tdr_pack_f32_elem(jb.w, jb.Cin, jb.KH, jb.mode, jb.CK, jb.M, jb.Kch, jb.KHe, jb.Mx, i);
    else if (jb.fmt == 1 && jb.KHe == 3 && jb.mode == 0)
        tdr_pack_bx3_alltaps9<0>(jb.w, jb.Cin, jb.M, jb.Kch, jb.Mx, i, reinterpret_cast<uint4*>(jb.wp));
    else if (jb.fmt == 1 && jb.KHe == 3 && jb.mode == 1)
        tdr_pack_bx3_alltaps9<1>(jb.w, jb.Cin, jb.M, jb.Kch, jb.Mx, i, reinterpret_cast<uint4*>(jb.wp));
    else if (jb.fmt == 1)
        tdr_pack_bx3_frag(jb.w, jb.Cin, jb.KH, jb.mode, jb.M, jb.Kch, jb.KHe, jb.Mx, i, reinterpret_cast<uint4*>(jb.wp));
    else if (jb.mode == 0 && jb.KHe == 1)
        tdr_pack_hx2_fwd_alltaps<1>(jb.w, jb.Cin, jb.M, jb.Kch, jb.Mx, i, reinterpret_cast<uint4*>(jb.wp));
    else if (jb.mode == 0 && jb.KHe == 2)
        tdr_pack_hx2_fwd_alltaps<4>(jb.w, jb.Cin, jb.M, jb.Kch, jb.Mx, i, reinterpret_cast<uint4*>(jb.wp));
    else if (jb.mode == 0 && jb.KHe == 3)
        tdr_pack_hx2_fwd_alltaps<9>(jb.w, jb.Cin, jb.M, jb.Kch, jb.Mx, i, reinterpret_cast<uint4*>(jb.wp));
    else
        tdr_pack_hx2_frag(jb.w, jb.Cin, jb.KH, jb.mode, jb.M, jb.Kch, jb.KHe, jb.Mx, i, reinterpret_cast<uint4*>(jb.wp));
}
}

extern "C" int tdr_pack_job_init(TdrPackJob* job, const float* w, int Cout, int Cin, int KH, int mode, int fmt, void* wp) {
    TDR_REQUIRE(job && w && wp, "tdr_pack_job_init: null pointer");
    TDR_REQUIRE(mode >= 0 && mode <= 3 && fmt >= 0 && fmt <= 2, "tdr_pack_job_init: bad mode/fmt");
    int M, Kch, KHe;
    if (mode == 0) { M = Cout; Kch = Cin; KHe = KH; }
    else if (mode == 1) { M = Cin; Kch = Cout; KHe = KH; }
    else if (mode == 2) { TDR_REQUIRE(KH == 2, "mode 2 needs a 2x2 kernel"); M = 4 * Cin; Kch = Cout; KHe = 1; }
    else { TDR_REQUIRE(KH == 3, "mode 3 needs a 3x3 kernel"); M = 4 * Cin; Kch = Cout; KHe = 2; }
    job->w = w; job->wp = wp; job->Cout = Cout; job->Cin = Cin; job->KH = KH; job->mode = mode; job->fmt = fmt;
    job->M = M; job->Kch = Kch; job->KHe = KHe;
    if (fmt == 0) {
        job->CK = tdr_conv_ck(KHe);
        job->Mx = (M + 31) / 32 * 32;
        job->total = tdr_packed_weight_floats(M, Kch, KHe);
    } else {
        job->CK = 16;
        job->Mx = (M + 31) / 32;
        job->total = (long)((Kch + 15) / 16) * KHe * KHe * job->Mx * 64;
        if (fmt == 2 && mode == 0 && KHe >= 1 && KHe <= 3) job->total = (long)((Kch + 15) / 16) * job->Mx * 64;
        if (fmt == 1 && KHe == 3 && mode <= 1) job->total = (long)((Kch + 15) / 16) * job->Mx * 64;
    }
    job->first_block = 0;
    return TDR_OK;
}

extern "C" int tdr_pack_weights_multi(const TdrPackJob* jobs_dev, int n_jobs, int64_t total_blocks, void* stream) {
    TDR_REQUIRE(jobs_dev && n_jobs > 0 && total_blocks > 0 && total_blocks < (1LL << 31), "tdr_pack_weights_multi: bad argument");
    hipLaunchKernelGGL(pack_multi_kernel, dim3((unsigned)total_blocks), dim3(256), 0, (hipStream_t)stream, jobs_dev, n_jobs);
    TDR_LAUNCH_CHECK("pack_multi_kernel");
    return TDR_OK;
}
```

### textualdegremoval_amd/csrc/tdr_conv_p16.hip

```cpp
#include <stdlib.h>
#include <stdint.h>
#include <type_traits>
#include "tdr_common.h"
#include "../../include/tdr.h"

typedef _Float16 pf16x8 __attribute__((ext_vector_type(8)));
typedef _Float16 pf16x4 __attribute__((ext_vector_type(4)));
typedef __bf16 pbf16x8 __attribute__((ext_vector_type(8)));
typedef unsigned pu32x4 __attribute__((ext_vector_type(4)));

namespace {

enum { PF_TRI = 1, PF_PAIR = 2 };
template <int PF> struct PlaneFmt { static constexpr int NS = PF == PF_TRI ? 3 : 2; };

__device__ __forceinline__ _Float16 p16_head(float x) {
    const _Float16 h = (_Float16)x;
    return x == 0.f ? __builtin_bit_cast(_Float16, (unsigned short)0x8000) : h;
}
__device__ __forceinline__ bool p16_positive(_Float16 head) { return (__builtin_bit_cast(unsigned short, head) & 0x8000u) == 0; }
__device__ __forceinline__ void p16_split4(float x0, float x1, float x2, float x3, uint2& h, uint2& m) {
    unsigned h0, h1, m0, m1;
    tdr_split2_f16(x0, x1, h0, m0);
    tdr_split2_f16(x2, x3, h1, m1);
    h0 |= (x0 == 0.f ? 0x8000u : 0u) | (x1 == 0.f ? 0x80000000u : 0u);
    h1 |= (x2 == 0.f ? 0x8000u : 0u) | (x3 == 0.f ? 0x80000000u : 0u);
    h = make_uint2(h0, h1);
    m = make_uint2(m0, m1);
}

__device__ __forceinline__ void p24_split4(float x0, float x1, float x2, float x3, uint2& h, uint2& m, uint2& l) {
    unsigned h0, h1, m0, m1, l0, l1;
    tdr_split3_bf16(x0, x1, h0, m0, l0);
    tdr_split3_bf16(x2, x3, h1, m1, l1);
    h0 |= (x0 == 0.f ? 0x8000u : 0u) | (x1 == 0.f ? 0x80000000u : 0u);
    h1 |= (x2 == 0.f ? 0x8000u : 0u) | (x3 == 0.f ? 0x80000000u : 0u);
    h = make_uint2(h0, h1);
    m = make_uint2(m0, m1);
    l = make_uint2(l0, l1);
}
template <int PF>
__device__ __forceinline__ void plane4_to_f32(uint2 v, float (&o)[4]) {
    if constexpr (PF == PF_TRI) {
        o[0] = __builtin_bit_cast(float, v.x << 16); o[1] = __builtin_bit_cast(float, v.x & 0xffff0000u);
        o[2] = __builtin_bit_cast(float, v.y << 16); o[3] = __builtin_bit_cast(float, v.y & 0xffff0000u);
    } else {
        const pf16x4 h = __builtin_bit_cast(pf16x4, v);
#pragma unroll
        for (int e = 0; e < 4; ++e) o[e] = (float)h[e];
    }
}

struct P16Args {
    const uint4* in; long in_ns;
    int Cin, H, W, Hp, Wp;
    const uint4* wp; int MT;
    int Cout;
    const float* bias;
    const float* res32; long res32_ns;
    const uint4* res16; long res16_ns;
    const float* mask32; long mask32_ns;
    const uint4* mask16; long mask16_ns;
    int relu;
    float* out32; long out32_ns;
    uint4* out16; long out16_ns;
    int tiles_x, tiles_y, mtiles;
};

#define P16_GLDS(gptr, lptr)                                                                          \
    __builtin_amdgcn_global_load_lds((__attribute__((address_space(1))) const void*)(gptr),          \
                                     (__attribute__((address_space(3))) void*)(lptr), 16, 0, 0)

template <int N>
__device__ __forceinline__ void wait_barrier() {
    asm volatile("s_waitcnt vmcnt(%0) lgkmcnt(0)\n\ts_barrier" ::"n"(N) : "memory");
}

template <int TM, int TN, int PF = PF_PAIR>
__device__ __forceinline__ void p16_epilogue(const P16Args& a, f32x16 (&acc)[TM][TN], int n, int m0, int wm, int wn, int oy0, int ox0, int j, int kk) {
    constexpr int NS = PlaneFmt<PF>::NS;
    const long PS = (long)a.Hp * a.Wp;
    const long HW = (long)a.H * a.W;
#pragma unroll
    for (int tn = 0; tn < TN; ++tn) {
        const int oy = oy0 + wn * TN + tn, ox = ox0 + j;
        const bool pvalid = oy < a.H && ox < a.W;
        const long pix = pvalid ? (long)oy * a.W + ox : 0;
        const long pslot = pvalid ? (long)(oy + 1) * a.Wp + ox + 1 : 0;
#pragma unroll
        for (int tm = 0; tm < TM; ++tm) {
            __builtin_amdgcn_sched_barrier(0);
            const int mt0 = m0 + (wm * TM + tm) * 32;
            const int mb = mt0 + 4 * kk;
            float v[16];
#pragma unroll
            for (int r = 0; r < 16; ++r) v[r] = acc[tm][tn][r];
            if (a.bias) {
#pragma unroll
                for (int r = 0; r < 16; ++r) v[r] += a.bias[min(mb + (r & 3) + 8 * (r >> 2), a.Cout - 1)];
            }
            if (a.res32) {
                float tv[16];
#pragma unroll
                for (int r = 0; r < 16; ++r)
                    tv[r] = a.res32[(long)n * a.res32_ns + (long)min(mb + (r & 3) + 8 * (r >> 2), a.Cout - 1) * HW + pix];
#pragma unroll
                for (int r = 0; r < 16; ++r) v[r] += tv[r];
            }
            if (a.res16) {
#pragma unroll
                for (int q = 0; q < 4; ++q) {
                    const int oc = min((mt0 >> 3) + q, (a.Cout >> 3) - 1);
                    const char* p = reinterpret_cast<const char*>(a.res16 + (long)n * a.res16_ns + (long)oc * NS * PS + pslot) + kk * 8;
                    float h[4], m[4];
                    plane4_to_f32<PF>(*reinterpret_cast<const uint2*>(p), h);
                    plane4_to_f32<PF>(*reinterpret_cast<const uint2*>(p + PS * 16), m);
                    if constexpr (PF == PF_TRI) {
                        float l[4];
                        plane4_to_f32<PF>(*reinterpret_cast<const uint2*>(p + 2 * PS * 16), l);
#pragma unroll
                        for (int e = 0; e < 4; ++e) v[4 * q + e] += (h[e] + m[e]) + l[e];
                    } else {
#pragma unroll
                        for (int e = 0; e < 4; ++e) v[4 * q + e] += h[e] + m[e];
                    }
                }
            }
            if (a.relu) {
#pragma unroll
                for (int r = 0; r < 16; ++r) v[r] = fmaxf(v[r], 0.f);
            }
            if (a.mask32) {
                float tv[16];
#pragma unroll
                for (int r = 0; r < 16; ++r)
                    tv[r] = a.mask32[(long)n * a.mask32_ns + (long)min(mb + (r & 3) + 8 * (r >> 2), a.Cout - 1) * HW + pix];
#pragma unroll
                for (int r = 0; r < 16; ++r) v[r] = tv[r] > 0.f ? v[r] : 0.f;
            }
            if (a.mask16) {
#pragma unroll
                for (int q = 0; q < 4; ++q) {
                    const int oc = min((mt0 >> 3) + q, (a.Cout >> 3) - 1);
                    const char* p = reinterpret_cast<const char*>(a.mask16 + (long)n * a.mask16_ns + (long)oc * NS * PS + pslot) + kk * 8;
                    const pf16x4 h = *reinterpret_cast<const pf16x4*>(p);
#pragma unroll
                    for (int e = 0; e < 4; ++e) v[4 * q + e] = p16_positive(h[e]) ? v[4 * q + e] : 0.f;
                }
            }
            if (a.out32) {
                float* op = a.out32 + (long)n * a.out32_ns + pix;
#pragma unroll
                for (int r = 0; r < 16; ++r) {
                    const int m = mb + (r & 3) + 8 * (r >> 2);
                    if (pvalid && m < a.Cout) op[(long)m * HW] = v[r];
                }
            }
            if (a.out16) {
#pragma unroll
                for (int q = 0; q < 4; ++q) {
                    if (!pvalid || mt0 + 8 * q >= a.Cout) continue;
                    uint2 pl[NS];
                    if constexpr (PF == PF_TRI) p24_split4(v[4 * q + 0], v[4 * q + 1], v[4 * q + 2], v[4 * q + 3], pl[0], pl[1], pl[2]);
                    else p16_split4(v[4 * q + 0], v[4 * q + 1], v[4 * q + 2], v[4 * q + 3], pl[0], pl[1]);
                    char* base = reinterpret_cast<char*>(a.out16 + (long)n * a.out16_ns + (long)((mt0 >> 3) + q) * NS * PS) + kk * 8;
#pragma unroll
                    for (int s = 0; s < NS; ++s) *reinterpret_cast<uint2*>(base + (s * PS + pslot) * 16) = pl[s];
                    const pf16x4 z = {0, 0, 0, 0};
                    const bool top = oy == 0, bot = oy == a.H - 1, lef = ox == 0, rig = ox == a.W - 1;
                    if (top | bot | lef | rig) {
                        const long Wp = a.Wp;
                        auto zero_at = [&](long sl) {
#pragma unroll
                            for (int s = 0; s < NS; ++s) *reinterpret_cast<pf16x4*>(base + (s * PS + sl) * 16) = z;
                        };
                        if (top) zero_at(ox + 1);
                        if (bot) zero_at((long)(a.H + 1) * Wp + ox + 1);
                        if (lef) zero_at((long)(oy + 1) * Wp);
                        if (rig) zero_at((long)(oy + 1) * Wp + a.W + 1);
                        if (top && lef) zero_at(0);
                        if (top && rig) zero_at(a.W + 1);
                        if (bot && lef) zero_at((long)(a.H + 1) * Wp);
                        if (bot && rig) zero_at((long)(a.H + 1) * Wp + a.W + 1);
                    }
                }
            }
        }
    }
}

template <int TM, int TN>
__device__ __forceinline__ void p16_epilogue_lean(const P16Args& a, f32x16 (&acc)[TM][TN], int n, int m0, int wm, int wn, int oy0, int ox0, int j, int kk) {
    const long PS = (long)a.Hp * a.Wp;
// ... 420 lines not shown
    a.mtiles = 1;
    const int ngroups = a.Cin >> 4;
    const long ntiles = (long)a.tiles_x * a.tiles_y * N;
    const size_t lds = (size_t)(2 * BREG + ngroups * 9 * 128) * 16;
    static const int wgs = tdr_tune_env("TDR_P16_THIN_WGS") ? atoi(tdr_tune_env("TDR_P16_THIN_WGS")) : 512;
    const int grid = (int)(ntiles < wgs ? ntiles : wgs);
    auto kern = conv3x3_p16_thin_kernel<TN, ABL>;
    static bool attr_set = false;
    if (!attr_set) {
        (void)hipFuncSetAttribute(reinterpret_cast<const void*>(kern), hipFuncAttributeMaxDynamicSharedMemorySize, 160 * 1024);
        attr_set = true;
    }
    hipLaunchKernelGGL(kern, dim3(grid), dim3(256), lds, st, a, (int)ntiles);
    TDR_LAUNCH_CHECK("conv3x3_p16_thin_kernel");
    return TDR_OK;
}

__device__ __forceinline__ void p16_glds_asm(const char* src, const uint4* dst) {
    const unsigned l = (unsigned)(uintptr_t)(__attribute__((address_space(3))) const char*)dst;
    unsigned keep;
    asm volatile("s_mov_b32 %0, m0\n\ts_mov_b32 m0, %2\n\ts_nop 0\n\tglobal_load_lds_dwordx4 %1, off\n\ts_mov_b32 m0, %0"
                 : "=&s"(keep) : "v"(src), "s"(l) : "memory");
}

template <int TN, int ABL = 0>
__global__ __launch_bounds__(512) void conv3x3_p16_thin8_kernel(P16Args a, int ntiles) {
    constexpr int TH = 8 * TN, LH = TH + 2, LW = 34, TS = LH * LW;
    constexpr int NBW = (4 * TS + 511) / 512, BREG = 4 * TS;
    extern __shared__ __attribute__((aligned(1024))) uint4 smem4[];
    const int tid = threadIdx.x, lane = tid & 63, wave = __builtin_amdgcn_readfirstlane(tid >> 6);
    const int j = lane & 31, kk = lane >> 5;
    const long PS = (long)a.Hp * a.Wp;
    const int ngroups = a.Cin >> 4;
    pf16x8 aw[18][2];
#pragma unroll
    for (int s2 = 0; s2 < 18; ++s2) {
        const int sc = min(s2, ngroups * 9 - 1);
#pragma unroll
        for (int pl = 0; pl < 2; ++pl)
            aw[s2][pl] = __builtin_bit_cast(pf16x8, a.wp[((long)sc * a.MT * 2 + pl) * 64 + lane]);
    }
    int prc[NBW];
    unsigned plin[NBW];
    bool pok[NBW];
#pragma unroll
    for (int k = 0; k < NBW; ++k) {
        const int f0 = (k * 8 + wave) * 64 + lane;
        pok[k] = f0 < 4 * TS;
        const int f = min(f0, 4 * TS - 1);
        const int op = f / TS, sl = f - op * TS;
        const int r = sl / LW, c = sl - r * LW;
        prc[k] = (r << 8) | c;
        plin[k] = (unsigned)(op * PS * 16);
    }
    const uint4* pb0 = smem4 + kk * 2 * TS + (wave * TN) * LW + j;
    constexpr int HA[3] = {1, 0, 0}, HB[3] = {0, 1, 0};
    const int tiles_xy = a.tiles_x * a.tiles_y;

    auto issue_tile = [&](int t, int buf) {
        const int n = t / tiles_xy, r0 = t - n * tiles_xy;
        const int ty = r0 / a.tiles_x, tx = r0 - ty * a.tiles_x;
        const char* base = reinterpret_cast<const char*>(a.in + (long)n * a.in_ns);
#pragma unroll
        for (int k = 0; k < NBW; ++k) {
            const int gy = min(ty * TH + (prc[k] >> 8), a.Hp - 1), gx = min(tx * 32 + (prc[k] & 255), a.Wp - 1);
            const unsigned off = plin[k] + (unsigned)((gy * a.Wp + gx) * 16);
            if (pok[k])
                for (int g = 0; g < ngroups; ++g)
                    p16_glds_asm(base + (long)g * 64 * PS + off, smem4 + (buf * 2 + g) * BREG + (k * 8 + wave) * 64);
        }
    };
    auto tile_epilogue = [&](int t, f32x16 (&acc)[1][TN]) {
        const int n = t / tiles_xy, r0 = t - n * tiles_xy;
        const int ty = r0 / a.tiles_x, tx = r0 - ty * a.tiles_x;
        p16_epilogue_lean<1, TN>(a, acc, n, 0, 0, wave, ty * TH, tx * 32, j, kk);
    };

    f32x16 acc[1][TN];
    int tprev = -1, it = 0;
    int t = blockIdx.x;
    if (t < ntiles) issue_tile(t, 0);
    asm volatile("s_waitcnt vmcnt(0) lgkmcnt(0)\n\ts_barrier" ::: "memory");
    for (; t < ntiles; t += gridDim.x, ++it) {
        const int buf = it & 1;
        if (tprev >= 0 && !(ABL & 16)) tile_epilogue(tprev, acc);
        const int tnext = t + gridDim.x;
        if (tnext < ntiles && !(ABL & 1)) issue_tile(tnext, buf ^ 1);
#pragma unroll
        for (int tn = 0; tn < TN; ++tn)
#pragma unroll
            for (int r = 0; r < 16; ++r) acc[0][tn][r] = 0.f;
#pragma unroll
        for (int g = 0; g < 2; ++g) {
            if (g < ngroups) {
#pragma unroll
                for (int tap = 0; tap < 9; ++tap) {
                    const uint4* pb = pb0 + (buf * 2 + g) * BREG + (tap / 3) * LW + (tap % 3);
                    pf16x8 bf[TN][2];
#pragma unroll
                    for (int tn = 0; tn < TN; ++tn)
#pragma unroll
                        for (int s2 = 0; s2 < 2; ++s2) bf[tn][s2] = __builtin_bit_cast(pf16x8, pb[s2 * TS + tn * LW]);
#pragma unroll
                    for (int q = 0; q < 3; ++q)
#pragma unroll
                        for (int tn = 0; tn < TN; ++tn)
                            acc[0][tn] = __builtin_amdgcn_mfma_f32_32x32x16_f16(aw[g * 9 + tap][HA[q]], bf[tn][HB[q]], acc[0][tn], 0, 0, 0);
                }
            }
        }
        asm volatile("s_waitcnt vmcnt(0) lgkmcnt(0)\n\ts_barrier" ::: "memory");
        tprev = t;
    }
    if (tprev >= 0) tile_epilogue(tprev, acc);
}

template <int TN, int ABL = 0>
int launch_p16_thin8(const P16Args& a0, int N, hipStream_t st) {
    constexpr int TH = 8 * TN, TS = (TH + 2) * 34, BREG = 4 * TS;
    P16Args a = a0;
    a.tiles_x = tdr_cdiv(a.W, 32);
    a.tiles_y = tdr_cdiv(a.H, TH);
    a.mtiles = 1;
    const long ntiles = (long)a.tiles_x * a.tiles_y * N;
    const size_t lds = (size_t)(4 * BREG) * 16;
    static const int wgs = tdr_tune_env("TDR_P16_THIN8_WGS") ? atoi(tdr_tune_env("TDR_P16_THIN8_WGS")) : 256;
    const int grid = (int)(ntiles < wgs ? ntiles : wgs);
    auto kern = conv3x3_p16_thin8_kernel<TN, ABL>;
    static bool attr_set = false;
    if (!attr_set) {
        (void)hipFuncSetAttribute(reinterpret_cast<const void*>(kern), hipFuncAttributeMaxDynamicSharedMemorySize, 160 * 1024);
        attr_set = true;
    }
    hipLaunchKernelGGL(kern, dim3(grid), dim3(512), lds, st, a, (int)ntiles);
    TDR_LAUNCH_CHECK("conv3x3_p16_thin8_kernel");
    return TDR_OK;
}

template <int PF>
__global__ void p16_from_f32_kernel(const float* __restrict__ src, long src_ns, int C, int H, int W, uint4* __restrict__ dst) {
    constexpr int NS = PlaneFmt<PF>::NS;
    const int Hp = H + 2, Wp = W + 2;
    const long PS = (long)Hp * Wp, HW = (long)H * W;
    const int G = C >> 3;
    const long total = (long)G * PS;
    const int n = blockIdx.y;
    for (long i = blockIdx.x * (long)blockDim.x + threadIdx.x; i < total; i += (long)gridDim.x * blockDim.x) {
        const int oc = (int)(i / PS);
        const long s = i - oc * PS;
        const int y = (int)(s / Wp), x = (int)(s - (long)y * Wp);
        const bool in = y >= 1 && y <= H && x >= 1 && x <= W;
        const float* p = src + (long)n * src_ns + (long)oc * 8 * HW + (in ? (long)(y - 1) * W + x - 1 : 0);
        uint4* o = dst + ((long)n * G + oc) * NS * PS + s;
        if constexpr (PF == PF_TRI) {
            float v[8];
#pragma unroll
            for (int e = 0; e < 8; ++e) v[e] = in ? p[e * HW] : 0.f;
            uint2 h0, m0, l0, h1, m1, l1;
            p24_split4(v[0], v[1], v[2], v[3], h0, m0, l0);
            p24_split4(v[4], v[5], v[6], v[7], h1, m1, l1);
            if (!in) { h0 = make_uint2(0, 0); h1 = h0; }
            o[0] = make_uint4(h0.x, h0.y, h1.x, h1.y);
            o[PS] = make_uint4(m0.x, m0.y, m1.x, m1.y);
            o[2 * PS] = make_uint4(l0.x, l0.y, l1.x, l1.y);
        } else {
            pf16x8 h, m;
#pragma unroll
            for (int e = 0; e < 8; ++e) {
                float v = in ? p[e * HW] : 0.f;
                asm volatile("" : "+v"(v));
                const _Float16 hh = (_Float16)v;
                h[e] = in ? p16_head(v) : hh;
                m[e] = (_Float16)(v - (float)hh);
            }
            o[0] = __builtin_bit_cast(uint4, h);
            o[PS] = __builtin_bit_cast(uint4, m);
        }
    }
}

template <int PF>
__global__ void p16_to_f32_kernel(const uint4* __restrict__ src, int C, int H, int W, float* __restrict__ dst, long dst_ns) {
    constexpr int NS = PlaneFmt<PF>::NS;
    const int Hp = H + 2, Wp = W + 2;
    const long PS = (long)Hp * Wp, HW = (long)H * W;
    const int G = C >> 3;
    const long total = (long)G * HW;
    const int n = blockIdx.y;
    for (long i = blockIdx.x * (long)blockDim.x + threadIdx.x; i < total; i += (long)gridDim.x * blockDim.x) {
        const int oc = (int)(i / HW);
        const long s = i - oc * HW;
        const int y = (int)(s / W), x = (int)(s - (long)y * W);
        const uint4* p = src + ((long)n * G + oc) * NS * PS + (long)(y + 1) * Wp + x + 1;
        float* o = dst + (long)n * dst_ns + (long)(oc * 8) * HW + s;
        if constexpr (PF == PF_TRI) {
            const uint4 h = p[0], m = p[PS], l = p[2 * PS];
            const unsigned hh[4] = {h.x, h.y, h.z, h.w}, mm[4] = {m.x, m.y, m.z, m.w}, ll[4] = {l.x, l.y, l.z, l.w};
#pragma unroll
            for (int e = 0; e < 4; ++e) {
                o[(long)(2 * e) * HW] = (__builtin_bit_cast(float, hh[e] << 16) + __builtin_bit_cast(float, mm[e] << 16)) + __builtin_bit_cast(float, ll[e] << 16);
                o[(long)(2 * e + 1) * HW] = (__builtin_bit_cast(float, hh[e] & 0xffff0000u) + __builtin_bit_cast(float, mm[e] & 0xffff0000u)) +
                                            __builtin_bit_cast(float, ll[e] & 0xffff0000u);
            }
        } else {
            const pf16x8 h = __builtin_bit_cast(pf16x8, p[0]), m = __builtin_bit_cast(pf16x8, p[PS]);
#pragma unroll
            for (int e = 0; e < 8; ++e) o[(long)e * HW] = (float)h[e] + (float)m[e];
        }
    }
}

}

extern "C" int64_t tdr_p16_bytes_fmt(int N, int C, int H, int W, int fmt) {
    return (int64_t)N * (C / 8) * (fmt == PF_TRI ? 3 : 2) * (H + 2) * (W + 2) * 16;
}
extern "C" int64_t tdr_p16_bytes(int N, int C, int H, int W) { return tdr_p16_bytes_fmt(N, C, H, W, PF_PAIR); }

extern "C" int tdr_p16_from_f32_fmt(const float* src, int64_t src_ns, int N, int C, int H, int W, void* dst, int fmt, void* stream) {
    TDR_REQUIRE(src && dst && N > 0, "tdr_p16_from_f32: bad argument");
    TDR_REQUIRE(C % 16 == 0, "tdr_p16_from_f32: C = %d is not a multiple of 16", C);
    TDR_REQUIRE(fmt == PF_TRI || fmt == PF_PAIR, "tdr_p16_from_f32: plane format %d (1: bf16 triple, 2: fp16 pair)", fmt);
    const long total = (long)(C / 8) * (H + 2) * (W + 2);
    const int blocks = (int)((total + 255) / 256 < 8192 ? (total + 255) / 256 : 8192);
    if (fmt == PF_TRI) hipLaunchKernelGGL(p16_from_f32_kernel<PF_TRI>, dim3(blocks, N), dim3(256), 0, (hipStream_t)stream, src, (long)src_ns, C, H, W, (uint4*)dst);
    else hipLaunchKernelGGL(p16_from_f32_kernel<PF_PAIR>, dim3(blocks, N), dim3(256), 0, (hipStream_t)stream, src, (long)src_ns, C, H, W, (uint4*)dst);
    TDR_LAUNCH_CHECK("p16_from_f32_kernel");
    return TDR_OK;
}
extern "C" int tdr_p16_from_f32(const float* src, int64_t src_ns, int N, int C, int H, int W, void* dst, void* stream) {
    return tdr_p16_from_f32_fmt(src, src_ns, N, C, H, W, dst, PF_PAIR, stream);
}

extern "C" int tdr_p16_to_f32_fmt(const void* src, int N, int C, int H, int W, float* dst, int64_t dst_ns, int fmt, void* stream) {
    TDR_REQUIRE(src && dst && N > 0, "tdr_p16_to_f32: bad argument");
    TDR_REQUIRE(C % 16 == 0, "tdr_p16_to_f32: C = %d is not a multiple of 16", C);
    TDR_REQUIRE(fmt == PF_TRI || fmt == PF_PAIR, "tdr_p16_to_f32: plane format %d (1: bf16 triple, 2: fp16 pair)", fmt);
    const long total = (long)(C / 8) * H * W;
    const int blocks = (int)((total + 255) / 256 < 8192 ? (total + 255) / 256 : 8192);
    if (fmt == PF_TRI) hipLaunchKernelGGL(p16_to_f32_kernel<PF_TRI>, dim3(blocks, N), dim3(256), 0, (hipStream_t)stream, (const uint4*)src, C, H, W, dst, (long)dst_ns);
    else hipLaunchKernelGGL(p16_to_f32_kernel<PF_PAIR>, dim3(blocks, N), dim3(256), 0, (hipStream_t)stream, (const uint4*)src, C, H, W, dst, (long)dst_ns);
    TDR_LAUNCH_CHECK("p16_to_f32_kernel");
    return TDR_OK;
}
extern "C" int tdr_p16_to_f32(const void* src, int N, int C, int H, int W, float* dst, int64_t dst_ns, void* stream) {
    return tdr_p16_to_f32_fmt(src, N, C, H, W, dst, dst_ns, PF_PAIR, stream);
}

static int p16_env_cfg() {
    const int c = tdr_tune_env("TDR_P16_CFG") ? atoi(tdr_tune_env("TDR_P16_CFG")) : 0;
    return (((c >= 100 && c < 300) || c >= 400) && !tdr_tune_env("TDR_PROBES")) ? 0 : c;
}
static int g_p16_cfg = p16_env_cfg();
extern "C" int tdr_conv3x3_p16_force_cfg(int cfg) {
    static const bool probes = tdr_tune_env("TDR_PROBES") != nullptr;
    TDR_REQUIRE(probes || cfg < 100 || (cfg >= 300 && cfg < 400), "tdr_conv3x3_p16_force_cfg: configuration %d is a timing ablation (set TDR_PROBES=1)", cfg);
    g_p16_cfg = cfg;
    return TDR_OK;
}

extern "C" int tdr_conv3x3_p16(const TdrConvP16Desc* d, void* stream) {
    TDR_REQUIRE(d && d->in && d->wp && (d->out32 || d->out16), "tdr_conv3x3_p16: null pointer");
    TDR_REQUIRE(d->Cin % 16 == 0 && d->Cin >= 16, "tdr_conv3x3_p16: Cin = %d is not a multiple of 16", d->Cin);
    TDR_REQUIRE(!d->out16 || d->Cout % 16 == 0, "tdr_conv3x3_p16: P16 output needs Cout %% 16 == 0 (got %d)", d->Cout);
    TDR_REQUIRE((!d->res16 && !d->mask16) || d->Cout % 8 == 0, "tdr_conv3x3_p16: P16 residual / mask need Cout %% 8 == 0");
    TDR_REQUIRE(d->wp_fmt == 2 || d->wp_fmt == 1, "tdr_conv3x3_p16: weights must be the 2-way fp16 split pack (wp_fmt 2, pair planes) or the 3-way bf16 split pack (wp_fmt 1, triple planes)");
    const int NSd = d->wp_fmt == 1 ? 3 : 2;
    P16Args a;
    a.in = (const uint4*)d->in; a.in_ns = (long)(d->Cin / 8) * NSd * (d->H + 2) * (d->W + 2);
    a.Cin = d->Cin; a.H = d->H; a.W = d->W; a.Hp = d->H + 2; a.Wp = d->W + 2;
    a.wp = (const uint4*)d->wp; a.MT = d->Mpad >> 5; a.Cout = d->Cout;
    a.bias = d->bias;
    a.res32 = d->res32; a.res32_ns = d->res32_ns;
    a.res16 = (const uint4*)d->res16; a.res16_ns = (long)(d->Cout / 8) * NSd * (d->H + 2) * (d->W + 2);
    a.mask32 = d->mask32; a.mask32_ns = d->mask32_ns;
    a.mask16 = (const uint4*)d->mask16; a.mask16_ns = a.res16_ns;
    a.relu = d->relu;
    a.out32 = d->out32; a.out32_ns = d->out32_ns;
    a.out16 = (uint4*)d->out16; a.out16_ns = a.res16_ns;
    a.tiles_x = a.tiles_y = a.mtiles = 0;
    hipStream_t st = (hipStream_t)stream;
    const int N = d->N;
    auto blocks = [&](int bm, int th) { return (long)tdr_cdiv(d->Cout, bm) * tdr_cdiv(d->H, th) * tdr_cdiv(d->W, 32) * N; };
    int cfg = g_p16_cfg;
    if (d->wp_fmt == 1) {
        constexpr int T = PF_TRI;
        if (cfg < 300) cfg = 0;
        if (cfg == 0) {
            if (d->Cout <= 32) cfg = 308;
            else if (d->Cout <= 64) cfg = 303;
            else if (d->Cout % 128 == 0 && blocks(128, 8) >= 256) cfg = 302;
            else cfg = 301;
        }
        switch (cfg) {
            case 301: return launch_p16<2, 2, 1, 4, true, 0, true, T>(a, N, st);
            case 302: return launch_p16<2, 2, 2, 4, true, 0, true, T>(a, N, st);
            case 303: return launch_p16<1, 2, 2, 2, true, 0, true, T>(a, N, st);
            case 304: return launch_p16<2, 2, 2, 2, true, 0, true, T>(a, N, st);
            case 306: return launch_p16<2, 2, 4, 2, true, 0, true, T>(a, N, st);
            case 307: return launch_p16<2, 1, 2, 4, true, 0, true, T>(a, N, st);
            case 308: return launch_p16<1, 2, 1, 4, true, 0, true, T>(a, N, st);
            case 309: return launch_p16<1, 1, 1, 4, true, 0, true, T>(a, N, st);
            case 311: return launch_p16<2, 2, 1, 4, true, 0, false, T>(a, N, st);
            case 312: return launch_p16<2, 2, 2, 4, true, 0, false, T>(a, N, st);
            case 321: return launch_p16<2, 2, 1, 4, false, 0, false, T>(a, N, st);
            case 401: return launch_p16<2, 2, 1, 4, true, 1, true, T>(a, N, st);
            case 402: return launch_p16<2, 2, 1, 4, true, 2, true, T>(a, N, st);
            case 403: return launch_p16<2, 2, 1, 4, true, 3, true, T>(a, N, st);
            case 404: return launch_p16<2, 2, 1, 4, true, 4, true, T>(a, N, st);
            case 407: return launch_p16<2, 2, 1, 4, true, 7, true, T>(a, N, st);
            case 408: return launch_p16<2, 2, 1, 4, true, 8, true, T>(a, N, st);
            case 416: return launch_p16<2, 2, 1, 4, true, 16, true, T>(a, N, st);
            case 423: return launch_p16<2, 2, 1, 4, true, 23, true, T>(a, N, st);
            case 431: return launch_p16<2, 2, 1, 4, true, 31, true, T>(a, N, st);
            case 501: return launch_p16<2, 2, 2, 4, true, 1, true, T>(a, N, st);
            case 507: return launch_p16<2, 2, 2, 4, true, 7, true, T>(a, N, st);
            case 516: return launch_p16<2, 2, 2, 4, true, 16, true, T>(a, N, st);
            case 523: return launch_p16<2, 2, 2, 4, true, 23, true, T>(a, N, st);
            default: break;
        }
        tdr_set_error("tdr_conv3x3_p16: unknown triple-plane tile configuration %d", cfg);
        return TDR_ERR_ARG;
    }
    if (cfg >= 300) cfg = 0;
    if (cfg >= 32 && cfg <= 36 && d->Cin <= 32 && d->Cout <= 32)
        return cfg == 32 ? launch_p16_thin8<1>(a, N, st) : (cfg == 33 ? launch_p16_thin8<2>(a, N, st) : (cfg == 34 ? launch_p16_thin8<1, 1>(a, N, st) :
               (cfg == 35 ? launch_p16_thin8<1, 16>(a, N, st) : launch_p16_thin8<1, 17>(a, N, st))));
    if (cfg >= 130 && cfg <= 132 && d->Cin <= 32 && d->Cout <= 32)
        return cfg == 130 ? launch_p16_thin<2, 1>(a, N, st) : (cfg == 131 ? launch_p16_thin<2, 16>(a, N, st) : launch_p16_thin<2, 17>(a, N, st));
    if ((cfg == 0 || cfg == 30 || cfg == 31) && d->Cin <= 32 && d->Cout <= 32) {
// ... 47 lines not shown
```

### textualdegremoval_amd/csrc/tdr_error.cpp

```cpp
#include <stdarg.h>
#include <stdio.h>
#include "../../include/tdr.h"
static thread_local char g_err[512] = "";
void tdr_set_error(const char* fmt, ...) {
    va_list ap;
    va_start(ap, fmt);
    vsnprintf(g_err, sizeof(g_err), fmt, ap);
    va_end(ap);
}
extern "C" const char* tdr_last_error(void) { return g_err; }
extern "C" int tdr_version(void) { return 110; }
```

### textualdegremoval_amd/engine.py

```python
import contextlib
import os
import types

import torch

from . import kernels as K
from . import leaves as L
from .kernels import (EPI_GATEBWD, EPI_PSHUF, PACK_DGRAD_2X2S2, PACK_DGRAD_3X3S2, PACK_DGRAD_S1, PACK_FWD)

LN_EPS = 1e-6
FUSE_TAIL = True
FUSE_HEAD = True
FUSE_CONV3_DGRAD = True
INFER_KERNELS = True


def _sub(P, pre):
    n = len(pre)
    return {k[n:]: v for k, v in P.items() if k.startswith(pre)}


def _put(G, pre, g):
    for k, v in g.items():
        G[pre + k] = v
# ... 44 lines not shown
                w5p, P['conv5.bias'], P['gamma'].view(-1))
        if lean:
            return K.naf_tail_infer(*args, c_out=c_out), None
        out, y, mu2, rs2, yn, t4 = K.naf_tail_fwd(*args, c_out=c_out)
        if not keep:
            return out, None
        return out, (x, xn, mu1, rs1, t1, g, pooled, s, y, yn, mu2, rs2, t4, c_out)
    wp, mp, *_ = K.pack_weights(P['conv3.weight'], PACK_FWD)
    y = K.conv_forward(g, wp, mp, c, 1, kscale=s, bias=P['conv3.bias'], scale=P['beta'].view(-1), res=x)
    if not keep:
        g = None
    yn, mu2, rs2 = K.layernorm2d_fwd(y, P['norm2.weight'], P['norm2.bias'], LN_EPS)
    wp, mp, *_ = K.pack_weights(P['conv4.weight'], PACK_FWD)
    t4 = K.conv_forward(yn, wp, mp, 2 * c, 1, bias=P['conv4.bias'])
    if not keep:
        yn = None
    wp, mp, *_ = K.pack_weights(P['conv5.weight'][:c_out], PACK_FWD)
    out = K.conv_forward(t4, wp, mp, c_out, 1, gate=True, bias=P['conv5.bias'], scale=P['gamma'].view(-1), res=y)
    if not keep:
        return out, None
    saved = (x, xn, mu1, rs1, t1, g, pooled, s, y, yn, mu2, rs2, t4, c_out)
    return out, saved


def _dgrad_is_hx2():
    return K.MATH == 'hx2' and K.GRAD_SCALED


def _dgrad_fused_ok():
    return _dgrad_is_hx2() or K.MATH == 'bx3'


def naf_bwd(dout, P, saved):
    x, xn, mu1, rs1, t1, g, pooled, s, y, yn, mu2, rs2, t4, c_out = saved
    N, c, H, W = x.shape
    dev = x.device
    G = {}
    beta, gamma = P['beta'].view(-1), P['gamma'].view(-1)
    late = L.current is not None and DEFER_LN_FINISH
    def fmt5(dw5, db5, dgam):
        g = {}
        if c_out == c:
            g['conv5.weight'], g['conv5.bias'], g['gamma'] = dw5.view(c, c, 1, 1), db5, dgam.view(1, c, 1, 1)
        else:
            fw = torch.zeros(c, c, 1, 1, dtype=torch.float32, device=dev)
            fb = torch.zeros(c, dtype=torch.float32, device=dev)
            fg = torch.zeros(1, c, 1, 1, dtype=torch.float32, device=dev)
            K.copy_rows(dw5, 0, fw, 0, 1, c_out * c)
            K.copy_rows(db5, 0, fb, 0, 1, c_out)
            K.copy_rows(dgam, 0, fg, 0, 1, c_out)
            g['conv5.weight'], g['conv5.bias'], g['gamma'] = fw, fb, fg
        return g

    def post5(G5, S5):
        return fmt5(*K.side_keep(*K.scaled_conv_param_grads(G5.view(c_out, c), S5, P['conv5.weight'], P['conv5.bias'], gamma)))
    L.leaf_wgrad1x1((t4, dout), (t4, dout, c_out, c, True), post5, G, scp=(P['conv5.weight'], P['conv5.bias'], gamma, c_out, c, fmt5))
    fused = FUSE_TAIL and K.naf_tail_supported(c, H * W, c_out) and dout.is_contiguous() and \
        _dgrad_fused_ok()
    if fused:
        w5t, w4t = K.pack_weights(P['conv5.weight'][:c_out], PACK_DGRAD_S1)[0], K.pack_weights(P['conv4.weight'], PACK_DGRAD_S1)[0]
        if FUSE_CONV3_DGRAD:
            w3t = K.pack_weights(P['conv3.weight'], PACK_DGRAD_S1)[0]
            dy, dt4, gw2, gb2, dgp = K.naf_tail_bwd(dout, gamma, t4, y, mu2, rs2, P['norm2.weight'], w5t, w4t, w3tp=w3t, beta=beta,
                                                    sca=s.contiguous(), defer_finish=late)
        else:
            dy, dt4, gw2, gb2 = K.naf_tail_bwd(dout, gamma, t4, y, mu2, rs2, P['norm2.weight'], w5t, w4t, defer_finish=late)
        if late:
            L.leaf_fin(('norm2.weight', 'norm2.bias'), gw2, G)
        else:
            G['norm2.weight'], G['norm2.bias'] = gw2, gb2
    else:
        wp, mp, *_ = K.pack_weights(P['conv5.weight'][:c_out], PACK_DGRAD_S1)
        dt4 = K.conv_forward(dout, wp, mp, c, 1, epi=EPI_GATEBWD, kscale=gamma, aux=t4)
    L.leaf_wgrad1x1((yn, dt4), (yn, dt4, 2 * c, c, False),
                    lambda g4, b4: {'conv4.weight': g4.view(2 * c, c, 1, 1), 'conv4.bias': b4}, G)
    if not fused:
        wp, mp, *_ = K.pack_weights(P['conv4.weight'], PACK_DGRAD_S1)
        dyn = K.conv_forward(dt4, wp, mp, c, 1)
        dy, G['norm2.weight'], G['norm2.bias'] = K.layernorm2d_bwd(dyn, y, mu2, rs2, P['norm2.weight'], add=dout)
    G3, S3 = K.conv_wgrad(g, dy, c, c, 1, per_image=True, want_db=True)
    dw3, db3, dbeta, dwsca, dbsca, dpooled = K.sca_bwd(G3, S3, P['conv3.weight'], P['conv3.bias'], beta, s, pooled,
                                                       P['sca.1.weight'])
    G['conv3.weight'], G['conv3.bias'], G['beta'] = dw3, db3, dbeta
    G['sca.1.weight'], G['sca.1.bias'] = dwsca, dbsca
    if fused and FUSE_CONV3_DGRAD:
        dt1, gdw, gdb = K.dwsg_bwd(dgp, t1, P['conv2.weight'], P['conv2.bias'], dg_bias=dpooled, dg_bias_mul=1.0 / (H * W),
                                   defer_finish=late)
    else:
        wp, mp, *_ = K.pack_weights(P['conv3.weight'], PACK_DGRAD_S1)
        dg = K.conv_forward(dy, wp, mp, c, 1, kscale=beta, scale=s, bias2=dpooled, bias2_mul=1.0 / (H * W))
        dt1, gdw, gdb = K.dwsg_bwd(dg, t1, P['conv2.weight'], P['conv2.bias'], defer_finish=late)
    if isinstance(gdw, K.Finisher):
        L.leaf_fin(('conv2.weight', 'conv2.bias'), gdw, G)
    else:
        G['conv2.weight'], G['conv2.bias'] = gdw, gdb
    L.leaf_wgrad1x1((xn, dt1), (xn, dt1, 2 * c, c, False),
                    lambda g1, b1: {'conv1.weight': g1.view(2 * c, c, 1, 1), 'conv1.bias': b1}, G)
    if FUSE_TAIL and K.naf_tail_supported(c, H * W) and _dgrad_fused_ok() and x.is_contiguous() and dy.is_contiguous():
        w1t = K.pack_weights(P['conv1.weight'], PACK_DGRAD_S1)[0]
        dx, gw1, gb1 = K.naf_head_bwd(dt1, x, mu1, rs1, P['norm1.weight'], w1t, dy, defer_finish=late)
        if late:
            L.leaf_fin(('norm1.weight', 'norm1.bias'), gw1, G)
        else:
            G['norm1.weight'], G['norm1.bias'] = gw1, gb1
    else:
        wp, mp, *_ = K.pack_weights(P['conv1.weight'], PACK_DGRAD_S1)
        dxn = K.conv_forward(dt1, wp, mp, c, 1)
        dx, G['norm1.weight'], G['norm1.bias'] = K.layernorm2d_bwd(dxn, x, mu1, rs1, P['norm1.weight'], add=dy)
    L.maybe_join()
    return dx, G


def naf_seq_fwd(x, P, pre, n, c_out_last=None, local=None, keep=True):
    saved = []
    for i in range(n):
        if local is not None:
            x = naf_fwd_local(x, _sub(P, f'{pre}{i}.'), *local)
            continue
        x, sv = naf_fwd(x, _sub(P, f'{pre}{i}.'), c_out_last if i == n - 1 else None, keep=keep)
        saved.append(sv)
    return x, (saved if keep else None)


def naf_fwd_local(x, P, k1, k2):
    N, c, H, W = x.shape
    if k1 >= H and k2 >= W:
        return naf_fwd(x, P)[0]
    wp, mp, *_ = K.pack_weights(P['conv1.weight'], PACK_FWD)
    xn, _, _ = K.layernorm2d_fwd(x, P['norm1.weight'], P['norm1.bias'], LN_EPS)
    t1 = K.conv_forward(xn, wp, mp, 2 * c, 1, bias=P['conv1.bias'])
    g, _ = K.dwsg_fwd(t1, P['conv2.weight'], P['conv2.bias'])
    cat = torch.empty(N, 2 * c, H, W, dtype=torch.float32, device=x.device)
    K.copy_rows(g, c * H * W, cat, 2 * c * H * W, N, c * H * W)
    wp, mp, *_ = K.pack_weights(P['sca.1.weight'], PACK_FWD)
    K.conv_forward(K.local_avgpool(g, k1, k2), wp, mp, c, 1, bias=P['sca.1.bias'], out=cat[:, c:])
    wp, mp, *_ = K.pack_weights(P['conv3.weight'], PACK_FWD)
    y = K.conv_forward(cat, wp, mp, c, 1, gate=True, bias=P['conv3.bias'], scale=P['beta'].view(-1), res=x)
    yn, _, _ = K.layernorm2d_fwd(y, P['norm2.weight'], P['norm2.bias'], LN_EPS)
    wp, mp, *_ = K.pack_weights(P['conv4.weight'], PACK_FWD)
    t4 = K.conv_forward(yn, wp, mp, 2 * c, 1, bias=P['conv4.bias'])
    wp, mp, *_ = K.pack_weights(P['conv5.weight'], PACK_FWD)
    return K.conv_forward(t4, wp, mp, c, 1, gate=True, bias=P['conv5.bias'], scale=P['gamma'].view(-1), res=y)


def naf_seq_bwd(dout, P, pre, n, saved, G):
    for i in reversed(range(n)):
        L.set_prefix(f'{pre}{i}.')
        dout, g = naf_bwd(dout, _sub(P, f'{pre}{i}.'), saved[i])
        _put(G, f'{pre}{i}.', g)
    L.set_prefix('')
    return dout


def conv_fwd(x, w, b, stride, pad, res=None, relu=False, out=None):
    Cout, Cin, KH, _ = w.shape
    wp, mp, *_ = K.pack_weights(w, PACK_FWD)
    out = K.conv_forward(x, wp, mp, Cout, KH, stride=stride, pad=pad, bias=b, res=res, relu=relu, out=out)
    return out


def conv_bwd(dout, x, w, stride, pad, need_dx=True, add_to_dx=None, bias=True, into=None):
    Cout, Cin, KH, _ = w.shape

    def leaf():
        if bias:
            gw, gb = K.conv_wgrad(x, dout, Cout, Cin, KH, stride=stride, pad=pad, want_db=True)
        else:
            gw, gb = K.conv_wgrad(x, dout, Cout, Cin, KH, stride=stride, pad=pad), None
        return gw.view(Cout, Cin, KH, KH), gb
    dw = db = None
    if into is not None:
        Gc, wname, bname = into
        L.set_prefix('')

        def leaf_named():
            gw, gb = leaf()
            return {wname: gw} if (gb is None or bname is None) else {wname: gw, bname: gb}
        L.leaf((x, dout), leaf_named, Gc)
    else:
        with K.on_side(x, dout):
            dw, db = leaf()
    dx = None
    if need_dx:
        N, _, OH, OW = dout.shape
        if stride == 1:
            wp, mp, *_ = K.pack_weights(w, PACK_DGRAD_S1)
            dx = K.conv_forward(dout, wp, mp, Cin, KH, pad=KH - 1 - pad, res=add_to_dx)
        elif KH == 2 and stride == 2 and pad == 0:
            wp, mp, *_ = K.pack_weights(w, PACK_DGRAD_2X2S2)
            dx = K.conv_forward(dout, wp, mp, 4 * Cin, 1, epi=EPI_PSHUF, res=add_to_dx)
        elif KH == 3 and stride == 2 and pad == 1:
            wp, mp, *_ = K.pack_weights(w, PACK_DGRAD_3X3S2)
            dx = K.conv_forward(dout, wp, mp, 4 * Cin, 2, pad=0, OH=OH, OW=OW, epi=EPI_PSHUF, res=add_to_dx)
        else:
            raise NotImplementedError(f'conv dgrad KH={KH} stride={stride} pad={pad}')
    L.maybe_join()
    return dx, dw, db


def up_fwd(x, w, skip):
    C2 = w.shape[0]
    wp, mp, *_ = K.pack_weights(w, PACK_FWD)
    return K.conv_forward(x, wp, mp, C2, 1, epi=EPI_PSHUF, res=skip)


def up_bwd(dout, x, w, into=None):
    C2, Cc = w.shape[0], w.shape[1]
    dT = K.pixel_unshuffle2(dout)
    dw = None
    if into is not None:
        L.set_prefix('')
        L.leaf((x, dT), lambda: {into[1]: K.conv_wgrad(x, dT, C2, Cc, 1).view(C2, Cc, 1, 1)}, into[0])
    else:
        with K.on_side(x, dT):
            dw = K.conv_wgrad(x, dT, C2, Cc, 1).view(C2, Cc, 1, 1)
    wp, mp, *_ = K.pack_weights(w, PACK_DGRAD_S1)
    dx = K.conv_forward(dT, wp, mp, Cc, 1)
    L.maybe_join()
    return dx, dw


def _enc_counts(ext):
    return [ext[0], ext[1], ext[2], ext[2], ext[2]]


P16_ON = True
P16_MIN_C = None


def _p16_level(Cc, n_blocks):
    fmt = K.plane_fmt()
    min_c = P16_MIN_C if P16_MIN_C is not None else (32 if fmt == K.FMT_BX3 else 64)
    return P16_ON and n_blocks > 0 and fmt is not None and K.p16_supported(Cc) and Cc >= min_c


def encoder_fwd(x, P, pre, ext_n_blocks, levels=5, keep=True, deep_only=False):
    feats, saved = [], []
    cnt = _enc_counts(ext_n_blocks)
    for lvl in range(levels):
        k = lvl + 1
        xin = x
        a = conv_fwd(xin, P[f'{pre}conv_L{k}.weight'], P[f'{pre}conv_L{k}.bias'], 1 if lvl == 0 else 2, 1, relu=True)
        blocks = []
        x = a
        Cc = a.shape[1]
        if _p16_level(Cc, cnt[lvl]):
            fmt = K.plane_fmt()
            tri = fmt == K.FMT_BX3
            x16, x32 = K.p16_from_f32(a, fmt=fmt), a
            for i in range(cnt[lvl]):
                bp = f'{pre}blk_L{k}.{i}.'
                wp1, mp1, *_ = K.pack_weights(P[bp + 'conv1.weight'], PACK_FWD)
                wp2, mp2, *_ = K.pack_weights(P[bp + 'conv2.weight'], PACK_FWD)
                last = i == cnt[lvl] - 1
                _, h16 = K.conv3x3_p16(x16, wp1, mp1, Cc, bias=P[bp + 'conv1.bias'], relu=True, want32=False, want16=True)
                o32, o16 = K.conv3x3_p16(h16, wp2, mp2, Cc, bias=P[bp + 'conv2.bias'], res=x16 if tri else x32,
                                         want32=last or not tri, want16=not last)
                if keep:
                    blocks.append((x16, h16))
                x16, x32 = o16, o32
            x = x32
        else:
            for i in range(cnt[lvl]):
                bp = f'{pre}blk_L{k}.{i}.'
                h = conv_fwd(x, P[bp + 'conv1.weight'], P[bp + 'conv1.bias'], 1, 1, relu=True)
                o = conv_fwd(h, P[bp + 'conv2.weight'], P[bp + 'conv2.bias'], 1, 1, res=x)
                if keep:
                    blocks.append((x, h))
                x = o
        feats.append(x if not deep_only or lvl == levels - 1 else None)
        if keep:
            saved.append((xin, a, blocks))
    return feats, (saved if keep else None)


def encoder_bwd(dfeats, P, pre, ext_n_blocks, saved, G):
    cnt = _enc_counts(ext_n_blocks)
    dnext = None
    with L.deferred_join():
        _encoder_bwd_levels(dfeats, P, pre, cnt, saved, G, dnext)
    L.maybe_join()
    return None


def _encoder_bwd_levels(dfeats, P, pre, cnt, saved, G, dnext):
    for lvl in reversed(range(len(dfeats))):
        k = lvl + 1
        xin, a, blocks = saved[lvl]
        d = dnext if dnext is not None else dfeats[lvl]
        if d is None:
            continue
        if blocks and isinstance(blocks[0][0], K.P16):
            d16, d32 = K.p16_from_f32(d, fmt=blocks[0][0].fmt), d
            fmts = {t.fmt for bl in blocks for t in bl} | {d16.fmt}
            grouped = GROUP_LEAVES and 2 * cnt[lvl] > 1 and len(fmts) == 1
            late = []
            for i in reversed(range(cnt[lvl])):
                bp = f'{pre}blk_L{k}.{i}.'
                x16, h16 = blocks[i]
                w1, w2 = P[bp + 'conv1.weight'], P[bp + 'conv2.weight']
                Cc = w1.shape[0]
                if grouped:
                    late.append((bp + 'conv2', h16, d16))
                else:
                    with K.on_side(h16.buf, d16.buf):
                        gw, G[bp + 'conv2.bias'] = K.wgrad3x3_p16(h16, d16, want_db=True)
                        G[bp + 'conv2.weight'] = gw.view(Cc, Cc, 3, 3)
                wp, mp, *_ = K.pack_weights(w2, PACK_DGRAD_S1)
                _, dh16 = K.conv3x3_p16(d16, wp, mp, Cc, mask=h16, want32=False, want16=True)
                if grouped:
                    late.append((bp + 'conv1', x16, dh16))
                else:
                    with K.on_side(x16.buf, dh16.buf):
                        gw, G[bp + 'conv1.bias'] = K.wgrad3x3_p16(x16, dh16, want_db=True)
                        G[bp + 'conv1.weight'] = gw.view(Cc, Cc, 3, 3)
                wp, mp, *_ = K.pack_weights(w1, PACK_DGRAD_S1)
                first = i == 0
                d32, d16 = K.conv3x3_p16(dh16, wp, mp, Cc, res=d32 if d32 is not None else d16, mask=a if first else None,
                                         want32=first, want16=not first)
            if late:
                with K.on_side(*[t.buf for _, x16, g16 in late for t in (x16, g16)]):
                    res = K.wgrad3x3_p16_group([(x16, g16) for _, x16, g16 in late], seq=('enc3x3', pre, lvl), want_db=True)
                    for (name, x16, g16), (gw, gb) in zip(late, res):
                        G[name + '.bias'] = gb
                        G[name + '.weight'] = gw.view(g16.C, x16.C, 3, 3)
                late.clear()
            d = d32
        else:
            for i in reversed(range(cnt[lvl])):
                bp = f'{pre}blk_L{k}.{i}.'
                x_in, h = blocks[i]
                w1, w2 = P[bp + 'conv1.weight'], P[bp + 'conv2.weight']
                Cc = w1.shape[0]
                with K.on_side(h, d):
                    gw, G[bp + 'conv2.bias'] = K.conv_wgrad(h, d, Cc, Cc, 3, pad=1, want_db=True)
                    G[bp + 'conv2.weight'] = gw.view(Cc, Cc, 3, 3)
                wp, mp, *_ = K.pack_weights(w2, PACK_DGRAD_S1)
                dh = K.conv_forward(d, wp, mp, Cc, 3, pad=1, mask=h)
                with K.on_side(x_in, dh):
                    gw, G[bp + 'conv1.bias'] = K.conv_wgrad(x_in, dh, Cc, Cc, 3, pad=1, want_db=True)
                    G[bp + 'conv1.weight'] = gw.view(Cc, Cc, 3, 3)
                wp, mp, *_ = K.pack_weights(w1, PACK_DGRAD_S1)
                d = K.conv_forward(dh, wp, mp, Cc, 3, pad=1, res=d, mask=a if i == 0 else None)
        dpre = d if cnt[lvl] > 0 else K.relu_bwd(d, a)
        w = P[f'{pre}conv_L{k}.weight']
        dnext, G[f'{pre}conv_L{k}.weight'], G[f'{pre}conv_L{k}.bias'] = conv_bwd(
            dpre, xin, w, 1 if lvl == 0 else 2, 1, need_dx=(lvl > 0), add_to_dx=dfeats[lvl - 1] if lvl > 0 else None)
    L.maybe_join()
    return None


class MasaGeom:
    def __init__(self, h, w, hr, wr, n_enc, lr_block_size, ref_down_block_size, dilations):
        padder = 2 ** n_enc
        self.px = w // padder // lr_block_size
        self.py = h // padder // lr_block_size
        self.kx = w // padder // self.px
        self.ky = h // padder // self.py
        self.dia_x = 2 * int(wr // padder // (2 * self.px) * ref_down_block_size) + 1
        self.dia_y = 2 * int(hr // padder // (2 * self.py) * ref_down_block_size) + 1
        if self.dia_x != self.dia_y or self.kx != self.ky:
            raise ValueError('MASA geometry must be square (the reference only runs for square geometry, :668-669)')
        self.dilations = list(dilations)
        self.P = self.py * self.px
        self.K = self.kx
        self.side = self.dia_x + 2


class Pyramids:
    __slots__ = ('N', 'stacked', 'inp_p', 'geo', 'feats', 'sv_enc', 'lq_deep', 'ref_feats', 'levels')


def pyramids_fwd(P, cfg, inp, ref, padder_log2, levels, keep=True):
    N, Ci, H0, W0 = inp.shape
    mult = (2 ** padder_log2) * cfg['lr_block_size']
    Hp, Wp = -(-H0 // mult) * mult, -(-W0 // mult) * mult
    Hr0, Wr0 = ref.shape[-2:]
    Hrp, Wrp = -(-Hr0 // mult) * mult, -(-Wr0 // mult) * mult
    if ref.shape[0] != N:
        raise ValueError('inp and ref must have the same batch size')
    py = Pyramids()
    py.N, py.levels = N, levels
    py.geo = MasaGeom(Hp, Wp, Hrp, Wrp, padder_log2, cfg['lr_block_size'], cfg['ref_down_block_size'], cfg['dilations'])
    py.stacked = (Hrp, Wrp) == (Hp, Wp)
    if py.stacked:
        both = torch.empty(2 * N, Ci, Hp, Wp, dtype=torch.float32, device=inp.device)
        _pad_into(inp.contiguous(), both[:N])
        _pad_into(ref.contiguous(), both[N:])
        py.inp_p = both[:N]
        py.feats, py.sv_enc = encoder_fwd(both, P, 'masa_enc.', cfg['ext_n_blocks'], levels=levels, keep=keep)
        py.lq_deep = py.feats[levels - 1][:N]
        py.ref_feats = [f[N:] for f in py.feats]
    else:
        py.inp_p = torch.empty(N, Ci, Hp, Wp, dtype=torch.float32, device=inp.device)
        ref_p = torch.empty(N, Ci, Hrp, Wrp, dtype=torch.float32, device=inp.device)
        _pad_into(inp.contiguous(), py.inp_p)
        _pad_into(ref.contiguous(), ref_p)
        fl, svl = encoder_fwd(py.inp_p, P, 'masa_enc.', cfg['ext_n_blocks'], levels=levels, keep=keep, deep_only=not keep)
        fr, svr = encoder_fwd(ref_p, P, 'masa_enc.', cfg['ext_n_blocks'], levels=levels, keep=keep)
        py.feats, py.sv_enc = (fl, fr), (svl, svr)
        py.lq_deep, py.ref_feats = fl[levels - 1], fr
    if not keep:
        py.feats = py.sv_enc = None
    return py, (H0, W0, Hp, Wp)


def pyramids_bwd(dwarp, py, P, cfg, sv_masa, G):
    N, L = py.N, py.levels
    if py.stacked:
        dfeats = [torch.zeros_like(f) for f in py.feats]
        masa_bwd(dwarp, py.lq_deep, py.ref_feats, N, py.geo, sv_masa, dfeats[L - 1][:N], [d[N:] for d in dfeats])
        encoder_bwd(dfeats, P, 'masa_enc.', cfg['ext_n_blocks'], py.sv_enc, G)
        return
    fl, fr = py.feats
    dlq = torch.empty_like(fl[L - 1])
    dref = [torch.zeros_like(f) for f in fr]
    masa_bwd(dwarp, py.lq_deep, py.ref_feats, N, py.geo, sv_masa, dlq, dref)
    Gl, Gr = {}, {}
    encoder_bwd([None] * (L - 1) + [dlq], P, 'masa_enc.', cfg['ext_n_blocks'], py.sv_enc[0], Gl)
    encoder_bwd(dref, P, 'masa_enc.', cfg['ext_n_blocks'], py.sv_enc[1], Gr)
    for k, g in Gr.items():
        G[k] = K.add_(g.contiguous().view(1, -1), Gl[k].contiguous().view(1, -1)).view(g.shape) if k in Gl else g


def masa_fwd(lq4, ref_feats, N, geo, outs=None, keep=True):
    P, Kk, side = geo.P, geo.K, geo.side
    L = len(ref_feats)
    ref4 = ref_feats[L - 1]
    _, Cc, H, W = lq4.shape
    Hr, Wr = ref4.shape[-2:]
    dev = lq4.device
    lrb = K.lr_blocks_fwd(lq4, geo.py, geo.px, Kk, Kk)
    ND = len(geo.dilations)
    R = Hr * Wr
    dots = torch.empty(ND, N, P, Hr, Wr, dtype=torch.float32, device=dev)
    invq = torch.empty(ND, N * P, dtype=torch.float32, device=dev)
    invk = torch.empty(ND, N, R, dtype=torch.float32, device=dev)
    cc = (Kk + 2) // 2
    for di, d in enumerate(geo.dilations):
        wp, mp, per_b = K.pack_patches(lrb, P, 1, 1, 1, d, cc - d)
        K.conv_forward(ref4, wp, mp, P, 3, dil=d, pad=d, wp_ns=per_b, out=dots[di])
        K.patch_inv_norm(lrb, 1, 1, dil=d, off=cc - d, out=invq[di])
        K.patch_inv_norm(ref4, Hr, Wr, dil=d, pad=d, out=invk[di])
    index, y1, x1 = K.coarse_argmax_box(dots, invq, invk, N, P, Hr, Wr, geo.dia_x)
    if not keep:
        dots = invq = invk = wp = None
    refb = K.gather_ref_block(ref4, y1, x1, P, side, 1)
    wp, mp, per_b = K.pack_patches(lrb, 1, Kk, Kk, 1, 1, 0)
    R1 = side - 2
    fdots = K.conv_forward(refb, wp, mp, Kk * Kk, 3, pad=0, wp_ns=per_b)
    finvq = K.patch_inv_norm(lrb, Kk, Kk)
    finvk = K.patch_inv_norm(refb, R1, R1)
    index_all, soft_att = K.fine_argmax(fdots, finvq, finvk, N * P, Kk * Kk, R1 * R1)
    if not keep:
        lq4 = ref4 = lrb = refb = wp = fdots = finvq = finvk = None
    warp = []
    for lvl in range(L):
        s = 2 ** (L - 1 - lvl)
        warp.append(K.transfer_fwd(ref_feats[lvl], y1, x1, index_all, soft_att, geo.py, geo.px, Kk, side, s,
                                   out=None if outs is None else outs[lvl]))
        if not keep:
            ref_feats[lvl] = None
    if not keep:
        return warp, None
    saved = (lrb, refb, finvq, finvk, index, y1, x1, index_all, soft_att)
    return warp, saved


def masa_bwd(dwarp, lq4, ref_feats, N, geo, saved, dlq_out, dref_out):
    lrb, refb, finvq, finvk, index, y1, x1, index_all, soft_att = saved
    P, Kk, side = geo.P, geo.K, geo.side
    L = len(ref_feats)
    dev = lq4.device
    datt = torch.zeros(N * P, Kk * Kk, dtype=torch.float32, device=dev)
    for lvl in range(L):
        s = 2 ** (L - 1 - lvl)
        K.transfer_bwd(dwarp[lvl], ref_feats[lvl], y1, x1, index_all, soft_att, geo.py, geo.px, Kk, side, s,
                       dref_out[lvl], datt)
    dlrb, drefb = K.fine_search_bwd(datt, soft_att, index_all, lrb, refb, finvq, finvk, Kk, side)
    K.scatter_ref_block(drefb, dref_out[L - 1], y1, x1, P, side)
    _, Cc, H, W = lq4.shape
    dlq4 = K.lr_blocks_bwd(dlrb, N, Cc, H, W, geo.py, geo.px, Kk, Kk)
    K.copy_rows(dlq4, Cc * H * W, dlq_out, Cc * H * W, N, Cc * H * W)


def _pad_into(src, dst_view):
    N, Cc, Hs, Ws = src.shape
    _, _, Hd, Wd = dst_view.shape
    if (Hs, Ws) == (Hd, Wd):
        K.copy_rows(src, Cc * Hs * Ws, dst_view, Cc * Hd * Wd, N, Cc * Hs * Ws)
    else:
        tmp = K.pad_crop(src, Hd, Wd)
        K.copy_rows(tmp, Cc * Hd * Wd, dst_view, Cc * Hd * Wd, N, Cc * Hd * Wd)


def tlsc_kernel_sizes(cfg, train_size):
    _, _, Ht, Wt = train_size
    n_enc = len(cfg['enc_blk_nums'])
    mult = 1 << n_enc
    Hp, Wp = -(-Ht // mult) * mult, -(-Wt // mult) * mult
# ... 124 lines not shown
```

### textualdegremoval_amd/kernels.py

```python
import contextlib
import ctypes as C
import os

import torch

from . import _lib
from ._lib import TdrConvDesc, TdrConvP16Desc, TdrWgradDesc, TdrWgradP16Desc, check

EPI_STD, EPI_GATEBWD, EPI_PSHUF = 0, 1, 2
PACK_FWD, PACK_DGRAD_S1, PACK_DGRAD_2X2S2, PACK_DGRAD_3X3S2 = 0, 1, 2, 3

MATH = os.environ.get('TDR_MATH', 'bx3')
WGRAD_1X1_BX3 = True
FMT_F32, FMT_BX3, FMT_HX2, FMT_H1 = 0, 1, 2, 3


def fp16_path():
    return MATH in ('hx2', 'h1')


GRAD_SCALED = False
BACKWARD_PHASE = False


# ... 223 lines not shown

def packed_floats(M, Kch, kh_eff):
    return _lib.load().tdr_packed_weight_floats(M, Kch, kh_eff)


def _pack_dims(w, mode):
    Cout, Cin, KH, _ = w.shape
    if mode == PACK_FWD:
        return Cout, Cin, KH
    if mode == PACK_DGRAD_S1:
        return Cin, Cout, KH
    if mode == PACK_DGRAD_2X2S2:
        return 4 * Cin, Cout, 1
    return 4 * Cin, Cout, 2


def _packed_buffer(w, mode, math):
    lib = _lib.load()
    M, Kch, KHe = _pack_dims(w, mode)
    if math in ('hx2', 'h1') and (mode == PACK_FWD or GRAD_SCALED):
        n = lib.tdr_packed_weight_bytes_hx2(M, Kch, KHe) // 4
        fmt = FMT_HX2 if math == 'hx2' else FMT_H1
    elif math in ('bx3', 'hx2', 'h1'):
        n = lib.tdr_packed_weight_bytes_bx3(M, Kch, KHe) // 4
        fmt = FMT_BX3
    else:
        n = lib.tdr_packed_weight_floats(M, Kch, KHe)
        fmt = FMT_F32
    return PackedWeights(torch.empty(n, dtype=torch.float32, device=w.device), fmt)


class PackPlan:

    def __init__(self):
        self.entries = {}
        self.grouped = {}
        self.table = None
        self.dirty = True
        self.valid = False

    def lookup(self, w, mode, math):
        key = (w.data_ptr(), tuple(w.shape), mode, math, GRAD_SCALED)
        e = self.entries.get(key)
        if e is None:
            pw = _packed_buffer(w, mode, math)
            self.entries[key] = (w, mode, math, pw)
            self.dirty = True
            _pack_into(w, mode, pw)
            return pw
        if not self.valid:
            _pack_into(w, mode, e[3])
        return e[3]

    def run(self):
        if not self.entries:
            return
        lib = _lib.load()
        if self.dirty or self.table is None:
            jobs = (_lib.TdrPackJob * len(self.entries))()
            blocks = 0
            for j, (w, mode, math, pw) in enumerate(self.entries.values()):
                Cout, Cin, KH, _ = w.shape
                check(lib.tdr_pack_job_init(C.byref(jobs[j]), w.data_ptr(), Cout, Cin, KH, mode, min(pw.fmt, FMT_HX2), pw.data_ptr()),
                      'tdr_pack_job_init')
                jobs[j].first_block = blocks
                blocks += (jobs[j].total + 255) // 256
            raw = torch.frombuffer(bytearray(bytes(jobs)), dtype=torch.uint8).clone()
            dev = next(iter(self.entries.values()))[0].device
            self.table = (raw.to(dev), len(self.entries), blocks)
            self.dirty = False
        tab, n, blocks = self.table
        check(lib.tdr_pack_weights_multi(tab.data_ptr(), n, blocks, _stream()), 'tdr_pack_weights_multi')
        self.valid = True

    def invalidate(self):
        self.valid = False


_active_plan = None


def set_pack_plan(plan):
    global _active_plan
    prev = _active_plan
    _active_plan = plan
    return prev


def _pack_into(w, mode, pw):
    lib = _lib.load()
    Cout, Cin, KH, _ = w.shape
    assert w.is_contiguous()
    if pw.fmt in (FMT_HX2, FMT_H1):
        check(lib.tdr_pack_weights_hx2(w.data_ptr(), Cout, Cin, KH, mode, pw.data_ptr(), _stream()), 'tdr_pack_weights_hx2')
    elif pw.fmt == FMT_BX3:
        check(lib.tdr_pack_weights_bx3(w.data_ptr(), Cout, Cin, KH, mode, pw.data_ptr(), _stream()), 'tdr_pack_weights_bx3')
    else:
        check(lib.tdr_pack_weights(w.data_ptr(), Cout, Cin, KH, mode, pw.data_ptr(), _stream()), 'tdr_pack_weights')


def pack_weights(w, mode, out=None, math=None):
    M, Kch, KHe = _pack_dims(w, mode)
    math = math or MATH
    if _active_plan is not None and out is None:
        pw = _active_plan.lookup(w, mode, math)
    else:
        pw = PackedWeights(out, FMT_F32) if (out is not None and math == 'f32') else _packed_buffer(w, mode, math)
        _pack_into(w, mode, pw)
    return pw, (M + 31) // 32 * 32, M, Kch, KHe


def pack_weights_grouped(W, mode):
    G, Cout, Cin = W.shape
    assert W.is_contiguous()
    plan = _active_plan
    key = ('grouped', W.data_ptr(), (G, Cout, Cin), mode, MATH, GRAD_SCALED)
    store = plan.grouped if plan is not None else None
    e = store.get(key) if store is not None else None
    if e is None:
        w4 = [W[g].view(Cout, Cin, 1, 1) for g in range(G)]
        proto = _packed_buffer(w4[0], mode, MATH)
        per = proto.buf.numel()
        big = torch.empty(G * per, dtype=torch.float32, device=W.device)
        views = [PackedWeights(big[g * per:(g + 1) * per], proto.fmt) for g in range(G)]
        for g in range(G):
            _pack_into(w4[g], mode, views[g])
            if plan is not None:
                plan.entries[(w4[g].data_ptr(), tuple(w4[g].shape), mode, MATH, GRAD_SCALED)] = (w4[g], mode, MATH, views[g])
        M = _pack_dims(w4[0], mode)[0]
        e = (PackedWeights(big, proto.fmt), (M + 31) // 32 * 32, per, w4, views)
        if plan is not None:
            plan.dirty = True
            store[key] = e
    elif not plan.valid:
        for w, v in zip(e[3], e[4]):
            _pack_into(w, mode, v)
    return e[0], e[1], e[2]


def pack_patches(blk, G, PH, PW, pstep, dil, off):
    lib = _lib.load()
    BG, Cc, BH, BW = blk.shape
    B = BG // G
    M = G * PH * PW
    per_b = lib.tdr_packed_weight_floats(M, Cc, 3)
    wp = torch.empty(B * per_b, dtype=torch.float32, device=blk.device)
    check(lib.tdr_pack_patches(blk.data_ptr(), B, G, Cc, BH, BW, PH, PW, pstep, dil, off, wp.data_ptr(), _stream()),
          'tdr_pack_patches')
    return wp, (M + 31) // 32 * 32, per_b


def conv_forward(x, wp, Mpad, Cout, KH, stride=1, dil=1, pad=0, OH=None, OW=None, out=None, Cin=None, epi=EPI_STD,
                 gate=False, kscale=None, wp_ns=0, bias=None, scale=None, bias2=None, bias2_mul=1.0, res=None,
                 mask=None, aux=None, relu=False):
    lib = _lib.load()
    N, Cx, H, W = x.shape
    if Cin is None:
        Cin = Cx // 2 if gate else Cx
    if OH is None:
        OH = (H + 2 * pad - dil * (KH - 1) - 1) // stride + 1
        OW = (W + 2 * pad - dil * (KH - 1) - 1) // stride + 1
    if out is None:
        if epi == EPI_PSHUF:
            out = torch.empty(N, Cout // 4, 2 * OH, 2 * OW, dtype=torch.float32, device=x.device)
        elif epi == EPI_GATEBWD:
            out = torch.empty(N, 2 * Cout, OH, OW, dtype=torch.float32, device=x.device)
        else:
            out = torch.empty(N, Cout, OH, OW, dtype=torch.float32, device=x.device)
    d = TdrConvDesc()
    d.N, d.Cin, d.H, d.W = N, Cin, H, W
    d.Cout, d.OH, d.OW = Cout, OH, OW
    d.KH, d.stride, d.dil, d.pad = KH, stride, dil, pad
    d.inp, d.in_ns = x.data_ptr(), _dense_nchw(x)
    d.gate = 1 if gate else 0
    d.kscale, d.kscale_ns = _p(kscale), _vec_ns(kscale)
    d.wp, d.wp_ns, d.Mpad = wp.data_ptr(), wp_ns, Mpad
    d.wp_fmt = getattr(wp, 'fmt', FMT_F32)
    d.out, d.out_ns = out.data_ptr(), _dense_nchw(out)
    d.epi = epi
    d.bias, d.bias_ns = _p(bias), _vec_ns(bias)
    d.scale, d.scale_ns = _p(scale), _vec_ns(scale)
    d.bias2, d.bias2_ns, d.bias2_mul = _p(bias2), _vec_ns(bias2), float(bias2_mul)
    d.res, d.res_ns = _p(res), (_dense_nchw(res) if res is not None else 0)
    d.mask, d.mask_ns = _p(mask), (_dense_nchw(mask) if mask is not None else 0)
    d.aux, d.aux_ns = _p(aux), (_dense_nchw(aux) if aux is not None else 0)
    d.relu = int(relu) if not isinstance(relu, bool) else (1 if relu else 0)
    if _survey is not None and d.wp_fmt in (FMT_HX2, FMT_H1):
        _survey.probe(x, 'grad' if BACKWARD_PHASE else 'fwd')
    check(lib.tdr_conv_forward(C.byref(d), _stream()), 'tdr_conv_forward')
    return out


class P16:
    __slots__ = ('buf', 'N', 'C', 'H', 'W', 'fmt')

    def __init__(self, buf, N, Cc, H, W, fmt=FMT_HX2):
        self.buf, self.N, self.C, self.H, self.W, self.fmt = buf, N, Cc, H, W, fmt

    @staticmethod
    def empty(N, Cc, H, W, device, fmt=FMT_HX2):
        assert Cc % 16 == 0, f'plane tensors need C % 16 == 0 (got {Cc})'
        assert fmt in (FMT_HX2, FMT_BX3)
        n = _lib.load().tdr_p16_bytes_fmt(N, Cc, H, W, fmt) // 4
        return P16(torch.empty(n, dtype=torch.int32, device=device), N, Cc, H, W, fmt)

    def data_ptr(self):
        return self.buf.data_ptr()

    def to_f32(self):
        out = torch.empty(self.N, self.C, self.H, self.W, dtype=torch.float32, device=self.buf.device)
        check(_lib.load().tdr_p16_to_f32_fmt(self.buf.data_ptr(), self.N, self.C, self.H, self.W, out.data_ptr(), _dense_nchw(out),
                                             self.fmt, _stream()), 'tdr_p16_to_f32')
        return out


def p16_supported(Cc):
    return Cc % 16 == 0 and Cc >= 16


def plane_fmt():
    if MATH == 'hx2' and GRAD_SCALED:
        return FMT_HX2
    if MATH == 'bx3':
        return FMT_BX3
    return None


def p16_from_f32(x, out=None, fmt=FMT_HX2):
    N, Cc, H, W = x.shape
    out = out if out is not None else P16.empty(N, Cc, H, W, x.device, fmt)
    if _survey is not None and out.fmt == FMT_HX2:
        _survey.probe(x, 'grad' if BACKWARD_PHASE else 'fwd')
    check(_lib.load().tdr_p16_from_f32_fmt(x.data_ptr(), _dense_nchw(x), N, Cc, H, W, out.data_ptr(), out.fmt, _stream()), 'tdr_p16_from_f32')
    return out


def conv3x3_p16(x16, wp, Mpad, Cout, bias=None, res=None, mask=None, relu=False, want32=True, want16=False, out32=None):
    lib = _lib.load()
    d = TdrConvP16Desc()
    d.N, d.Cin, d.H, d.W, d.Cout = x16.N, x16.C, x16.H, x16.W, Cout
    d.inp = x16.data_ptr()
    d.wp, d.Mpad, d.wp_fmt = wp.data_ptr(), Mpad, getattr(wp, 'fmt', FMT_F32)
    assert d.wp_fmt == x16.fmt, f'weight pack format {d.wp_fmt} does not match the plane format {x16.fmt} of the input'
    assert all(t.fmt == x16.fmt for t in (res, mask) if isinstance(t, P16))
    d.bias = _p(bias)
    if isinstance(res, P16):
        d.res16 = res.data_ptr()
    elif res is not None:
        d.res32, d.res32_ns = res.data_ptr(), _dense_nchw(res)
    if isinstance(mask, P16):
        d.mask16 = mask.data_ptr()
    elif mask is not None:
        d.mask32, d.mask32_ns = mask.data_ptr(), _dense_nchw(mask)
    d.relu = 1 if relu else 0
    o32 = o16 = None
    if want32:
        o32 = out32 if out32 is not None else torch.empty(x16.N, Cout, x16.H, x16.W, dtype=torch.float32, device=x16.buf.device)
        d.out32, d.out32_ns = o32.data_ptr(), _dense_nchw(o32)
    if want16:
        o16 = P16.empty(x16.N, Cout, x16.H, x16.W, x16.buf.device, x16.fmt)
        d.out16 = o16.data_ptr()
    check(lib.tdr_conv3x3_p16(C.byref(d), _stream()), 'tdr_conv3x3_p16')
    if _survey is not None and o16 is not None and o16.fmt == FMT_HX2:
        _survey.probe(o32 if o32 is not None else o16.to_f32(), 'grad' if BACKWARD_PHASE else 'fwd')
    return o32, o16


def wgrad3x3_p16(x16, d16, want_db=False):
    lib = _lib.load()
    d = TdrWgradP16Desc()
    d.N, d.Cin, d.H, d.W, d.Cout = x16.N, x16.C, x16.H, x16.W, d16.C
    d.in16, d.dout16 = x16.data_ptr(), d16.data_ptr()
    assert x16.fmt == d16.fmt
    d.fmt = x16.fmt
    dev = x16.buf.device
    g = torch.empty(1, d16.C, x16.C, 3, 3, dtype=torch.float32, device=dev)
    db = torch.empty(d16.C, dtype=torch.float32, device=dev) if want_db else None
    d.g, d.db = g.data_ptr(), _p(db)
    ws = workspace(lib.tdr_wgrad3x3_p16_ws_floats(C.byref(d)), dev, 'wgrad')
    d.ws, d.ws_floats = ws.data_ptr(), ws.numel()
    check(lib.tdr_wgrad3x3_p16(C.byref(d), _stream()), 'tdr_wgrad3x3_p16')
    return (g, db) if want_db else g


def conv_wgrad(x, dout, Cout, Cin, KH, stride=1, pad=0, gate=False, per_image=False, want_db=False, fp16_range=False):
    lib = _lib.load()
    N, _, H, W = x.shape
    _, _, OH, OW = dout.shape
    d = TdrWgradDesc()
    d.N, d.Cin, d.H, d.W, d.Cout, d.OH, d.OW = N, Cin, H, W, Cout, OH, OW
    d.KH, d.stride, d.pad = KH, stride, pad
    d.inp, d.in_ns, d.gate = x.data_ptr(), _dense_nchw(x), 1 if gate else 0
    d.dout, d.dout_ns = dout.data_ptr(), _dense_nchw(dout)
    groups = N if per_image else 1
    g = torch.empty(groups, Cout, Cin, KH, KH, dtype=torch.float32, device=x.device)
    d.g = g.data_ptr()
    db = torch.empty(Cout, dtype=torch.float32, device=x.device) if want_db else None
    d.db = _p(db)
    d.per_image = 1 if per_image else 0
    if fp16_path() and (fp16_range or GRAD_SCALED) and (KH == 3 or WGRAD_1X1_BX3):
        d.math = 2 if MATH == 'hx2' else 3
    else:
        d.math = 1 if (MATH != 'f32' and (KH == 3 or WGRAD_1X1_BX3)) else 0
    if _survey is not None and d.math >= 2:
        _survey.probe(dout, 'fwd' if fp16_range else 'grad')
    need = lib.tdr_wgrad_ws_floats(C.byref(d))
    ws = workspace(need, x.device, 'wgrad')
    d.ws, d.ws_floats = ws.data_ptr(), ws.numel()
    check(lib.tdr_conv_wgrad(C.byref(d), _stream()), 'tdr_conv_wgrad')
    return (g, db) if want_db else g


def _wgrad1x1_desc(x, dout, Cout, Cin, gate):
    N, _, H, W = x.shape
    d = TdrWgradDesc()
    d.N, d.Cin, d.H, d.W, d.Cout, d.OH, d.OW = N, Cin, H, W, Cout, H, W
    d.KH, d.stride, d.pad = 1, 1, 0
    d.in_ns, d.gate, d.dout_ns = _dense_nchw(x), 1 if gate else 0, _dense_nchw(dout)
    d.per_image = 0
    if fp16_path() and GRAD_SCALED and WGRAD_1X1_BX3:
        d.math = 2 if MATH == 'hx2' else 3
    else:
        d.math = 1 if (MATH != 'f32' and WGRAD_1X1_BX3) else 0
    return d


def wgrad1x1_group_key(x, dout, Cout, Cin, gate):
    if x.dim() != 4 or dout.dim() != 4 or x.shape[2:] != dout.shape[2:] or x.data_ptr() % 16 or dout.data_ptr() % 16:
        return None
    d = _wgrad1x1_desc(x, dout, Cout, Cin, gate)
    if not _lib.load().tdr_wgrad1x1_group_supported(C.byref(d)):
        return None
    return (d.N, Cin, Cout, d.H, d.W, int(d.in_ns), int(d.dout_ns), int(d.gate), int(d.math))


GRP_CAP_SPARE = 4
_grp_pool = {}
_grp_owner = 0


def set_group_owner(token):
    global _grp_owner
    _grp_owner = token
# ... 1685 lines not shown
```

Baseline: 59.63.

## Write plane-format outputs directly from conv epilogue for encoder level convs

Adds an optional plane-format (bf16 triple or fp16 pair, zero-padded border) destination to the split-bf16 conv forward kernel, so the encoder level-entry convs and their stride-2 data-gradient convs emit the plane tensor consumed by the residual blocks directly. For the bf16-triple format the fp32 output is skipped. This removes the separate fp32-to-plane conversion pass and its extra read and write of the activation and gradient tensors. The cost is a heavier epilogue that uses cross-lane shuffles and border zeroing, plus more template instantiations.

```diff
diff --git a/include/tdr.h b/include/tdr.h
--- a/include/tdr.h
+++ b/include/tdr.h
@@ -5,7 +5,7 @@
 extern "C" {
 #endif
 
-#define TDR_ABI_VERSION 110
+#define TDR_ABI_VERSION 111
 int tdr_version(void);
 const char* tdr_last_error(void);
 
@@ -34,6 +34,8 @@
     const float* mask;  int64_t mask_ns;
     const float* aux;   int64_t aux_ns;
     int relu;
+    void* out16; int64_t out16_ns;
+    int out16_fmt;
 } TdrConvDesc;
 
 int tdr_conv_forward(const TdrConvDesc* d, void* stream);
diff --git a/textualdegremoval_amd/_lib.py b/textualdegremoval_amd/_lib.py
--- a/textualdegremoval_amd/_lib.py
+++ b/textualdegremoval_amd/_lib.py
@@ -6,7 +6,7 @@
 _HERE = os.path.dirname(os.path.abspath(__file__))
 LIB_PATH = os.environ.get('TDR_LIB_PATH', os.path.join(_HERE, 'libtdr_hip.so'))
 
-ABI_VERSION = 110
+ABI_VERSION = 111
 c_fp = C.c_void_p
 i32, i64, f32 = C.c_int, C.c_int64, C.c_float
 
@@ -29,6 +29,7 @@
         ('mask', c_fp), ('mask_ns', i64),
         ('aux', c_fp), ('aux_ns', i64),
         ('relu', i32),
+        ('out16', c_fp), ('out16_ns', i64), ('out16_fmt', i32),
     ]
 
 
diff --git a/textualdegremoval_amd/csrc/tdr_conv_bx3.hip b/textualdegremoval_amd/csrc/tdr_conv_bx3.hip
--- a/textualdegremoval_amd/csrc/tdr_conv_bx3.hip
+++ b/textualdegremoval_amd/csrc/tdr_conv_bx3.hip
@@ -36,8 +36,8 @@
 #ifndef TDR_CONV_OCC
 #define TDR_CONV_OCC 4
 #endif
-template <int KH, int S, int WM, int TM, int TN, int EPI, bool GATE, int SCH, int AD = 0>
-__global__ __launch_bounds__(256, (KH == 3 && S == 1 && WM == 1 && TM == 1 && TN == 2 && AD != 9) ? TDR_CONV_OCC : ((KH == 3 && S == 1 && WM == 2 && TM == 1 && TN == 4 && AD == 3) ? 3 : 2)) void conv_bx3_kernel(ConvArgs a) {
+template <int KH, int S, int WM, int TM, int TN, int EPI, bool GATE, int SCH, int AD = 0, bool PL = false>
+__global__ __launch_bounds__(256, (KH == 3 && S == 1 && WM == 1 && TM == 1 && TN == 2 && AD != 9) ? TDR_CONV_OCC : ((KH == 3 && S == 1 && WM == 2 && TM == 1 && TN == 4 && AD == 3) ? 3 : 2)) void conv_bx3_kernel(ConvArgsT<PL> a) {
     constexpr int NS = SCH == SCH_BX3 ? 3 : (SCH == SCH_HX2 ? 2 : 1);
     constexpr int NSW = SCH == SCH_BX3 ? 3 : 2;
     constexpr int NP = SCH == SCH_BX3 ? 6 : (SCH == SCH_HX2 ? 3 : 1);
@@ -253,6 +253,11 @@
         }
     }
 
+    if constexpr (PL) {
+        if (a.out16_fmt == PF_TRI) conv_epilogue<TM, TN, EPI, PF_TRI>(a, acc, n, m0, wm, wn, oy0, ox0, j, kk);
+        else conv_epilogue<TM, TN, EPI, PF_PAIR>(a, acc, n, m0, wm, wn, oy0, ox0, j, kk);
+        return;
+    }
     if constexpr (EPI != EPI_PSHUF) {
         if (a.vec_epi) {
             __syncthreads();
@@ -480,9 +485,9 @@
            a.H == a.OH && a.W == a.OW;
 }
 
-template <int KH, int S, int WM, int TM, int TN, int EPI, bool GATE, int SCH>
-int launch_bx_cfg_s(const ConvArgs& a, int N, hipStream_t st) {
-    if constexpr (KH == 1 && S == 1 && SCH != SCH_BX3 && EPI != EPI_PSHUF)
+template <int KH, int S, int WM, int TM, int TN, int EPI, bool GATE, int SCH, bool PL = false>
+int launch_bx_cfg_s(const ConvArgsT<PL>& a, int N, hipStream_t st) {
+    if constexpr (KH == 1 && S == 1 && SCH != SCH_BX3 && EPI != EPI_PSHUF && !PL)
         if (c1_hx2_ok(a, 32 * TN * (4 / WM), 32 * TM * WM, N)) return launch_c1_hx2<WM, TM, TN, EPI, GATE, SCH>(a, N, st);
     constexpr int NS = SCH == SCH_BX3 ? 3 : (SCH == SCH_HX2 ? 2 : 1);
     constexpr int WN = 4 / WM;
@@ -490,7 +495,7 @@
     constexpr int NT = TN * WN;
     const int TW = 1 << a.tw_log2, SR = 32 >> a.tw_log2, TH = NT * SR;
     const int LH = (TH - 1) * S + KH, LW = (TW - 1) * S + KH;
-    ConvArgs b = a;
+    ConvArgsT<PL> b = a;
     static const int single_env = tdr_tune_env("TDR_BX_SINGLE") ? atoi(tdr_tune_env("TDR_BX_SINGLE")) : 2;
     b.single_buf = (KH == 3 && (a.Cin + 15) / 16 <= single_env) ? 1 : 0;
     size_t lds = (size_t)(b.single_buf ? 1 : 2) * (2 * NS) * LH * LW * 16;
@@ -503,7 +508,7 @@
         static const int ring3 = tdr_tune_env("TDR_RING3") ? atoi(tdr_tune_env("TDR_RING3")) : 1;
         static const long ring_blocks3 = tdr_tune_env("TDR_RING_BLOCKS") ? atol(tdr_tune_env("TDR_RING_BLOCKS")) : 512;
         if (ring3 && ((long)grid.x * N > ring_blocks3 || TM != 1)) {
-            auto kern = conv_bx3_kernel<KH, S, WM, TM, TN, EPI, GATE, SCH, 3>;
+            auto kern = conv_bx3_kernel<KH, S, WM, TM, TN, EPI, GATE, SCH, 3, PL>;
             static bool attr_set = false;
             if (!attr_set) {
                 (void)hipFuncSetAttribute(reinterpret_cast<const void*>(kern), hipFuncAttributeMaxDynamicSharedMemorySize, 160 * 1024);
@@ -517,7 +522,7 @@
     if constexpr (KH == 3 && S == 1 && TM == 1 && SCH == SCH_HX2 && EPI == EPI_STD) {
         static const long ring_blocks = tdr_tune_env("TDR_RING_BLOCKS") ? atol(tdr_tune_env("TDR_RING_BLOCKS")) : 512;
         if ((long)grid.x * N <= ring_blocks) {
-            auto kern = conv_bx3_kernel<KH, S, WM, TM, TN, EPI, GATE, SCH, 9>;
+            auto kern = conv_bx3_kernel<KH, S, WM, TM, TN, EPI, GATE, SCH, 9, PL>;
             static bool attr_set = false;
             if (!attr_set) {
                 (void)hipFuncSetAttribute(reinterpret_cast<const void*>(kern), hipFuncAttributeMaxDynamicSharedMemorySize, 160 * 1024);
@@ -528,7 +533,7 @@
             return TDR_OK;
         }
     }
-    auto kern = conv_bx3_kernel<KH, S, WM, TM, TN, EPI, GATE, SCH>;
+    auto kern = conv_bx3_kernel<KH, S, WM, TM, TN, EPI, GATE, SCH, 0, PL>;
     static bool attr_set = false;
     if (!attr_set) {
         (void)hipFuncSetAttribute(reinterpret_cast<const void*>(kern), hipFuncAttributeMaxDynamicSharedMemorySize, 160 * 1024);
@@ -541,49 +546,56 @@
 
 int g_force_cfg[2] = {tdr_tune_env("TDR_BX_CFG1") ? atoi(tdr_tune_env("TDR_BX_CFG1")) : 0, tdr_tune_env("TDR_BX_CFG3") ? atoi(tdr_tune_env("TDR_BX_CFG3")) : 0};
 
-template <int KH, int S, int WM, int TM, int TN, int EPI, bool GATE>
-int launch_bx_cfg(const ConvArgs& a, int N, hipStream_t st) {
-    if (a.scheme == SCH_HX2) return launch_bx_cfg_s<KH, S, WM, TM, TN, EPI, GATE, SCH_HX2>(a, N, st);
-    if (a.scheme == SCH_H1) return launch_bx_cfg_s<KH, S, WM, TM, TN, EPI, GATE, SCH_H1>(a, N, st);
-    return launch_bx_cfg_s<KH, S, WM, TM, TN, EPI, GATE, SCH_BX3>(a, N, st);
-}
-
-template <int KH, int S, int EPI, bool GATE>
-int launch_bx_shape(const ConvArgs& a, int N, hipStream_t st) {
+template <int KH, int S, int WM, int TM, int TN, int EPI, bool GATE, bool PL>
+int launch_bx_cfg(const ConvArgsT<PL>& a, int N, hipStream_t st) {
+    if (a.scheme == SCH_HX2) return launch_bx_cfg_s<KH, S, WM, TM, TN, EPI, GATE, SCH_HX2, PL>(a, N, st);
+    if constexpr (PL) {
+        if (a.scheme == SCH_H1) {
+            tdr_set_error("tdr_conv_forward: a plane destination (out16) needs wp_fmt 1 or 2");
+            return TDR_ERR_UNSUPPORTED;
+        }
+    } else {
+        if (a.scheme == SCH_H1) return launch_bx_cfg_s<KH, S, WM, TM, TN, EPI, GATE, SCH_H1, PL>(a, N, st);
+    }
+    return launch_bx_cfg_s<KH, S, WM, TM, TN, EPI, GATE, SCH_BX3, PL>(a, N, st);
+}
+
+template <int KH, int S, int EPI, bool GATE, bool PL = false>
+int launch_bx_shape(const ConvArgsT<PL>& a, int N, hipStream_t st) {
     const long pix = (long)a.OH * a.OW;
     auto blocks = [&](int bm, int bn) { return (long)tdr_cdiv(a.Cout, bm) * tdr_cdiv(pix, bn) * N; };
     if constexpr (S == 2) {
-        if (a.Cout <= 32) return launch_bx_cfg<KH, S, 1, 1, 1, EPI, GATE>(a, N, st);
-        if (a.Cout <= 64 || blocks(128, 64) < 512) return launch_bx_cfg<KH, S, 2, 1, 1, EPI, GATE>(a, N, st);
-        return launch_bx_cfg<KH, S, 2, 2, 1, EPI, GATE>(a, N, st);
+        if (a.Cout <= 32) return launch_bx_cfg<KH, S, 1, 1, 1, EPI, GATE, PL>(a, N, st);
+        if (a.Cout <= 64 || blocks(128, 64) < 512) return launch_bx_cfg<KH, S, 2, 1, 1, EPI, GATE, PL>(a, N, st);
+        return launch_bx_cfg<KH, S, 2, 2, 1, EPI, GATE, PL>(a, N, st);
     } else {
         if (a.Cout <= 32) {
-            if (blocks(32, 256) >= 512) return launch_bx_cfg<KH, S, 1, 1, 2, EPI, GATE>(a, N, st);
-            return launch_bx_cfg<KH, S, 1, 1, 1, EPI, GATE>(a, N, st);
+            if (blocks(32, 256) >= 512) return launch_bx_cfg<KH, S, 1, 1, 2, EPI, GATE, PL>(a, N, st);
+            return launch_bx_cfg<KH, S, 1, 1, 1, EPI, GATE, PL>(a, N, st);
         }
         if (g_force_cfg[KH == 1 ? 0 : 1] == 0 && a.scheme == SCH_BX3 && a.Cin <= (KH == 1 ? 128 : 64) && blocks(64, 128) >= 2048)
-            return launch_bx_cfg<KH, S, 2, 1, 2, EPI, GATE>(a, N, st);
+            return launch_bx_cfg<KH, S, 2, 1, 2, EPI, GATE, PL>(a, N, st);
         if constexpr (KH == 1) {
             const int force = g_force_cfg[0];
-            if (force == 1) return launch_bx_cfg<KH, S, 2, 2, 2, EPI, GATE>(a, N, st);
-            if (force == 2) return launch_bx_cfg<KH, S, 2, 1, 4, EPI, GATE>(a, N, st);
-            if (force == 3) return launch_bx_cfg<KH, S, 2, 1, 2, EPI, GATE>(a, N, st);
-            if (force == 4) return launch_bx_cfg<KH, S, 1, 1, 2, EPI, GATE>(a, N, st);
-            if (force == 5) return launch_bx_cfg<KH, S, 4, 2, 2, EPI, GATE>(a, N, st);
-            if (a.Cout > 64 && blocks(128, 128) >= 512) return launch_bx_cfg<KH, S, 2, 2, 2, EPI, GATE>(a, N, st);
+            if (force == 1) return launch_bx_cfg<KH, S, 2, 2, 2, EPI, GATE, PL>(a, N, st);
+            if (force == 2) return launch_bx_cfg<KH, S, 2, 1, 4, EPI, GATE, PL>(a, N, st);
+            if (force == 3) return launch_bx_cfg<KH, S, 2, 1, 2, EPI, GATE, PL>(a, N, st);
+            if (force == 4) return launch_bx_cfg<KH, S, 1, 1, 2, EPI, GATE, PL>(a, N, st);
+            if (force == 5) return launch_bx_cfg<KH, S, 4, 2, 2, EPI, GATE, PL>(a, N, st);
+            if (a.Cout > 64 && blocks(128, 128) >= 512) return launch_bx_cfg<KH, S, 2, 2, 2, EPI, GATE, PL>(a, N, st);
             if (a.Cin >= 768 && a.Cout >= 256 && blocks(256, 64) >= 256 && blocks(256, 64) <= 512)
-                return launch_bx_cfg<KH, S, 4, 2, 2, EPI, GATE>(a, N, st);
+                return launch_bx_cfg<KH, S, 4, 2, 2, EPI, GATE, PL>(a, N, st);
         } else {
             const int force3 = g_force_cfg[1];
-            if (force3 == 1) return launch_bx_cfg<KH, S, 2, 2, 4, EPI, GATE>(a, N, st);
-            if (force3 == 2) return launch_bx_cfg<KH, S, 2, 1, 4, EPI, GATE>(a, N, st);
-            if (force3 == 3) return launch_bx_cfg<KH, S, 2, 1, 2, EPI, GATE>(a, N, st);
-            if (force3 == 4) return launch_bx_cfg<KH, S, 2, 2, 2, EPI, GATE>(a, N, st);
+            if (force3 == 1) return launch_bx_cfg<KH, S, 2, 2, 4, EPI, GATE, PL>(a, N, st);
+            if (force3 == 2) return launch_bx_cfg<KH, S, 2, 1, 4, EPI, GATE, PL>(a, N, st);
+            if (force3 == 3) return launch_bx_cfg<KH, S, 2, 1, 2, EPI, GATE, PL>(a, N, st);
+            if (force3 == 4) return launch_bx_cfg<KH, S, 2, 2, 2, EPI, GATE, PL>(a, N, st);
             const bool tall_ok = blocks(128, 256) >= 1024 || a.Cout % 128 != 0 || a.scheme != SCH_HX2;
-            if (a.Cout > 64 && blocks(128, 256) >= 512 && tall_ok) return launch_bx_cfg<KH, S, 2, 2, 4, EPI, GATE>(a, N, st);
-        }
-        if (blocks(64, 256) >= 512) return launch_bx_cfg<KH, S, 2, 1, 4, EPI, GATE>(a, N, st);
-        return launch_bx_cfg<KH, S, 2, 1, 2, EPI, GATE>(a, N, st);
+            if (a.Cout > 64 && blocks(128, 256) >= 512 && tall_ok) return launch_bx_cfg<KH, S, 2, 2, 4, EPI, GATE, PL>(a, N, st);
+        }
+        if (blocks(64, 256) >= 512) return launch_bx_cfg<KH, S, 2, 1, 4, EPI, GATE, PL>(a, N, st);
+        return launch_bx_cfg<KH, S, 2, 1, 2, EPI, GATE, PL>(a, N, st);
     }
 }
 
@@ -669,7 +681,8 @@
 
 int tdr_conv_forward_bx3(const TdrConvDesc* d, void* stream) {
     TDR_REQUIRE(d->dil == 1 && d->wp_ns % 4 == 0, "tdr_conv_forward: split-bf16 path needs dil=1 (and wp_ns a multiple of 4 floats)");
-    ConvArgs a;
+    ConvArgsPL a;
+    a.out16 = nullptr; a.out16_ns = 0; a.out16_fmt = 0;
     a.in = d->in; a.in_ns = d->in_ns; a.Cin = d->Cin; a.H = d->H; a.W = d->W;
     a.wp = (const float*)d->wp; a.wp_ns = d->wp_ns; a.Mpad = d->Mpad; a.Cout = d->Cout;
     a.scheme = d->wp_fmt == 3 ? SCH_H1 : (d->wp_fmt == 2 ? SCH_HX2 : SCH_BX3);
@@ -684,12 +697,32 @@
     a.res = d->res; a.res_ns = d->res_ns; a.mask = d->mask; a.mask_ns = d->mask_ns;
     a.aux = d->aux; a.aux_ns = d->aux_ns; a.relu = d->relu;
     auto al16 = [](const void* p) { return (reinterpret_cast<uintptr_t>(p) & 15) == 0; };
+    if (d->out16) {
+        const int Co = d->epi == EPI_PSHUF ? d->Cout / 4 : d->Cout, HO = d->epi == EPI_PSHUF ? 2 * d->OH : d->OH, WO = d->epi == EPI_PSHUF ? 2 * d->OW : d->OW;
+        TDR_REQUIRE(d->out16_fmt == PF_TRI || d->out16_fmt == PF_PAIR, "tdr_conv_forward: out16_fmt %d (1: bf16 triple, 2: fp16 pair)", d->out16_fmt);
+        TDR_REQUIRE((d->epi == EPI_STD || (d->epi == EPI_PSHUF && d->Cout % 4 == 0)) && Co % 16 == 0,
+                    "tdr_conv_forward: a plane destination needs epi STD / PSHUF and a multiple of 16 output channels (got epi %d, %d)", d->epi, Co);
+        TDR_REQUIRE((reinterpret_cast<uintptr_t>(d->out16) & 15) == 0 && d->out16_ns >= 0, "tdr_conv_forward: out16 must be 16-byte aligned");
+        a.out16 = (uint4*)d->out16;
+        a.out16_fmt = d->out16_fmt;
+        a.out16_ns = d->out16_ns ? d->out16_ns : (long)(Co / 8) * (d->out16_fmt == PF_TRI ? 3 : 2) * (HO + 2) * (WO + 2);
+    }
     a.vec_epi = (d->OW % 4 == 0 && d->out_ns % 4 == 0 && al16(d->out) && (!d->res || (d->res_ns % 4 == 0 && al16(d->res))) &&
                  (!d->mask || (d->mask_ns % 4 == 0 && al16(d->mask))) && (!d->aux || (d->aux_ns % 4 == 0 && al16(d->aux)))) ? 1 : 0;
     hipStream_t st = (hipStream_t)stream;
     const int N = d->N;
     const int key = d->KH * 100 + d->stride * 10 + d->epi;
     const bool g = d->gate != 0;
+    if (d->out16) {
+        switch (g ? -1 : key) {
+            case 310: return launch_bx_shape<3, 1, EPI_STD, false, true>(a, N, st);
+            case 320: return launch_bx_shape<3, 2, EPI_STD, false, true>(a, N, st);
+            case 212: return launch_bx_shape<2, 1, EPI_PSHUF, false, true>(a, N, st);
+            default: break;
+        }
+        tdr_set_error("tdr_conv_forward(bx3): no plane epilogue for (KH=%d stride=%d epi=%d gate=%d)", d->KH, d->stride, d->epi, d->gate);
+        return TDR_ERR_UNSUPPORTED;
+    }
     switch (key) {
         case 110: return g ? launch_bx_shape<1, 1, EPI_STD, true>(a, N, st) : launch_bx_shape<1, 1, EPI_STD, false>(a, N, st);
         case 111: if (!g) return launch_bx_shape<1, 1, EPI_GATEBWD, false>(a, N, st); break;
diff --git a/textualdegremoval_amd/csrc/tdr_conv_epi.h b/textualdegremoval_amd/csrc/tdr_conv_epi.h
--- a/textualdegremoval_amd/csrc/tdr_conv_epi.h
+++ b/textualdegremoval_amd/csrc/tdr_conv_epi.h
@@ -1,5 +1,7 @@
 #pragma once
+#include <type_traits>
 #include "tdr_common.h"
+#include "tdr_plane_split.h"
 
 namespace {
 
@@ -24,8 +26,14 @@
     int scheme;
 };
 
-template <int TM, int TN, int EPI>
-__device__ __forceinline__ void conv_epilogue(const ConvArgs& a, f32x16 (&acc)[TM][TN], int n, int m0, int wm, int wn,
+struct ConvArgsPL : ConvArgs {
+    uint4* out16; long out16_ns;
+    int out16_fmt;
+};
+template <bool PL> using ConvArgsT = std::conditional_t<PL, ConvArgsPL, ConvArgs>;
+
+template <int TM, int TN, int EPI, int PF = 0>
+__device__ __forceinline__ void conv_epilogue(const ConvArgsT<PF != 0>& a, f32x16 (&acc)[TM][TN], int n, int m0, int wm, int wn,
                                               int oy0, int ox0, int j, int kk) {
     const int TW = 1 << a.tw_log2, SR = 32 >> a.tw_log2;
     const long HWo = (long)a.OH * a.OW;
@@ -42,6 +50,7 @@
                 const long OW2 = 2L * a.OW;
                 const long p2 = pvalid ? (2L * oy) * OW2 + 2L * ox : 0;
                 float2 r0[4], r1[4];
+                float pw[PF != 0 ? 4 : 1][4];
                 if (a.res) {
 #pragma unroll
                     for (int q = 0; q < 4; ++q) {
@@ -57,10 +66,45 @@
                     float v0 = acc[tm][tn][4 * q + 0], v1 = acc[tm][tn][4 * q + 1];
                     float v2 = acc[tm][tn][4 * q + 2], v3 = acc[tm][tn][4 * q + 3];
                     if (a.res) { v0 += r0[q].x; v1 += r0[q].y; v2 += r1[q].x; v3 += r1[q].y; }
-                    if (pvalid && m < a.Cout) {
+                    if (pvalid && m < a.Cout && (PF == 0 || a.out)) {
                         float* o = a.out + (long)n * a.out_ns + (long)(m >> 2) * 4 * HWo + p2;
                         *reinterpret_cast<float2*>(o) = make_float2(v0, v1);
                         *reinterpret_cast<float2*>(o + OW2) = make_float2(v2, v3);
+                    }
+                    if constexpr (PF != 0) { pw[q][0] = v0; pw[q][1] = v1; pw[q][2] = v2; pw[q][3] = v3; }
+                }
+                if constexpr (PF != 0) {
+                    constexpr int NS = PlaneFmt<PF>::NS;
+                    float rcv[8];
+#pragma unroll
+                    for (int q = 0; q < 4; ++q) {
+                        rcv[2 * q] = __shfl_xor(kk ? pw[q][0] : pw[q][2], 32, 64);
+                        rcv[2 * q + 1] = __shfl_xor(kk ? pw[q][1] : pw[q][3], 32, 64);
+                    }
+                    float c0[8], c1[8];
+#pragma unroll
+                    for (int q = 0; q < 4; ++q) {
+                        const float own0 = kk ? pw[q][2] : pw[q][0], own1 = kk ? pw[q][3] : pw[q][1];
+                        c0[2 * q] = kk ? rcv[2 * q] : own0;         c0[2 * q + 1] = kk ? own0 : rcv[2 * q];
+                        c1[2 * q] = kk ? rcv[2 * q + 1] : own1;     c1[2 * q + 1] = kk ? own1 : rcv[2 * q + 1];
+                    }
+                    const int cb = (m0 + (wm * TM + tm) * 32) >> 2;
+                    if (pvalid && cb < (a.Cout >> 2)) {
+                        const int HO = 2 * a.OH, WO = 2 * a.OW, Y = 2 * oy + kk, X = 2 * ox;
+                        const long Wp = WO + 2, PS = (long)(HO + 2) * Wp;
+                        char* base = reinterpret_cast<char*>(a.out16 + (long)n * a.out16_ns + (long)(cb >> 3) * NS * PS);
+                        const long sl = (long)(Y + 1) * Wp + X + 1;
+                        uint2 lo[NS], hi[NS];
+                        plane_split4<PF>(c0[0], c0[1], c0[2], c0[3], lo);
+                        plane_split4<PF>(c0[4], c0[5], c0[6], c0[7], hi);
+#pragma unroll
+                        for (int s = 0; s < NS; ++s) *reinterpret_cast<uint4*>(base + (s * PS + sl) * 16) = make_uint4(lo[s].x, lo[s].y, hi[s].x, hi[s].y);
+                        plane_split4<PF>(c1[0], c1[1], c1[2], c1[3], lo);
+                        plane_split4<PF>(c1[4], c1[5], c1[6], c1[7], hi);
+#pragma unroll
+                        for (int s = 0; s < NS; ++s) *reinterpret_cast<uint4*>(base + (s * PS + sl + 1) * 16) = make_uint4(lo[s].x, lo[s].y, hi[s].x, hi[s].y);
+                        plane_zero_border<NS, uint4>(base, PS, Wp, Y, X, HO, WO);
+                        plane_zero_border<NS, uint4>(base, PS, Wp, Y, X + 1, HO, WO);
                     }
                 }
             } else if (EPI == EPI_GATEBWD) {
@@ -136,11 +180,29 @@
 #pragma unroll
                     for (int r = 0; r < 16; ++r) v[r] = tv[r] > 0.f ? v[r] : 0.f;
                 }
-                float* op = a.out + (long)n * a.out_ns + pix;
-#pragma unroll
-                for (int r = 0; r < 16; ++r) {
-                    const int m = mb + (r & 3) + 8 * (r >> 2);
-                    if (pvalid && m < a.Cout) op[(long)m * HWo] = v[r];
+                if (PF == 0 || a.out) {
+                    float* op = a.out + (long)n * a.out_ns + pix;
+#pragma unroll
+                    for (int r = 0; r < 16; ++r) {
+                        const int m = mb + (r & 3) + 8 * (r >> 2);
+                        if (pvalid && m < a.Cout) op[(long)m * HWo] = v[r];
+                    }
+                }
+                if constexpr (PF != 0) {
+                    constexpr int NS = PlaneFmt<PF>::NS;
+                    const int mt0 = m0 + (wm * TM + tm) * 32;
+                    const long Wp = a.OW + 2, PS = (long)(a.OH + 2) * Wp;
+                    const long sl = (long)(oy + 1) * Wp + ox + 1;
+#pragma unroll
+                    for (int q = 0; q < 4; ++q) {
+                        if (!pvalid || mt0 + 8 * q >= a.Cout) continue;
+                        uint2 pl[NS];
+                        plane_split4<PF>(v[4 * q + 0], v[4 * q + 1], v[4 * q + 2], v[4 * q + 3], pl);
+                        char* base = reinterpret_cast<char*>(a.out16 + (long)n * a.out16_ns + (long)((mt0 >> 3) + q) * NS * PS) + kk * 8;
+#pragma unroll
+                        for (int s = 0; s < NS; ++s) *reinterpret_cast<uint2*>(base + (s * PS + sl) * 16) = pl[s];
+                        plane_zero_border<NS, uint2>(base, PS, Wp, oy, ox, a.OH, a.OW);
+                    }
                 }
             }
         }
diff --git a/textualdegremoval_amd/csrc/tdr_conv_mfma.hip b/textualdegremoval_amd/csrc/tdr_conv_mfma.hip
--- a/textualdegremoval_amd/csrc/tdr_conv_mfma.hip
+++ b/textualdegremoval_amd/csrc/tdr_conv_mfma.hip
@@ -268,12 +268,13 @@
 }
 
 extern "C" int tdr_conv_forward(const TdrConvDesc* d, void* stream) {
-    TDR_REQUIRE(d && d->in && d->wp && d->out, "tdr_conv_forward: null pointer");
+    TDR_REQUIRE(d && d->in && d->wp && (d->out || d->out16), "tdr_conv_forward: null pointer");
     TDR_REQUIRE(d->N > 0 && d->Cin > 0 && d->Cout > 0 && d->OH > 0 && d->OW > 0, "tdr_conv_forward: bad shape");
     TDR_REQUIRE(d->Mpad % 32 == 0 && d->Mpad >= d->Cout, "tdr_conv_forward: Mpad %d invalid for Cout %d", d->Mpad, d->Cout);
     TDR_REQUIRE(d->epi != EPI_GATEBWD || d->aux, "tdr_conv_forward: GATEBWD needs aux");
     if (d->wp_fmt >= 1 && d->wp_fmt <= 3) return tdr_conv_forward_bx3(d, stream);
     TDR_REQUIRE(d->wp_fmt == 0, "tdr_conv_forward: unknown wp_fmt %d", d->wp_fmt);
+    TDR_REQUIRE(d->out && !d->out16, "tdr_conv_forward: the exact-fp32 kernels write fp32 tensors only (out16 needs wp_fmt 1 or 2)");
     ConvArgs a;
     a.in = d->in; a.in_ns = d->in_ns; a.Cin = d->Cin; a.H = d->H; a.W = d->W;
     a.wp = (const float*)d->wp; a.wp_ns = d->wp_ns; a.Mpad = d->Mpad; a.Cout = d->Cout;
diff --git a/textualdegremoval_amd/csrc/tdr_conv_p16.hip b/textualdegremoval_amd/csrc/tdr_conv_p16.hip
--- a/textualdegremoval_amd/csrc/tdr_conv_p16.hip
+++ b/textualdegremoval_amd/csrc/tdr_conv_p16.hip
@@ -2,6 +2,7 @@
 #include <stdint.h>
 #include <type_traits>
 #include "tdr_common.h"
+#include "tdr_plane_split.h"
 #include "../../include/tdr.h"
 
 typedef _Float16 pf16x8 __attribute__((ext_vector_type(8)));
@@ -11,34 +12,7 @@
 
 namespace {
 
-enum { PF_TRI = 1, PF_PAIR = 2 };
-template <int PF> struct PlaneFmt { static constexpr int NS = PF == PF_TRI ? 3 : 2; };
-
-__device__ __forceinline__ _Float16 p16_head(float x) {
-    const _Float16 h = (_Float16)x;
-    return x == 0.f ? __builtin_bit_cast(_Float16, (unsigned short)0x8000) : h;
-}
-__device__ __forceinline__ bool p16_positive(_Float16 head) { return (__builtin_bit_cast(unsigned short, head) & 0x8000u) == 0; }
-__device__ __forceinline__ void p16_split4(float x0, float x1, float x2, float x3, uint2& h, uint2& m) {
-    unsigned h0, h1, m0, m1;
-    tdr_split2_f16(x0, x1, h0, m0);
-    tdr_split2_f16(x2, x3, h1, m1);
-    h0 |= (x0 == 0.f ? 0x8000u : 0u) | (x1 == 0.f ? 0x80000000u : 0u);
-    h1 |= (x2 == 0.f ? 0x8000u : 0u) | (x3 == 0.f ? 0x80000000u : 0u);
-    h = make_uint2(h0, h1);
-    m = make_uint2(m0, m1);
-}
-
-__device__ __forceinline__ void p24_split4(float x0, float x1, float x2, float x3, uint2& h, uint2& m, uint2& l) {
-    unsigned h0, h1, m0, m1, l0, l1;
-    tdr_split3_bf16(x0, x1, h0, m0, l0);
-    tdr_split3_bf16(x2, x3, h1, m1, l1);
-    h0 |= (x0 == 0.f ? 0x8000u : 0u) | (x1 == 0.f ? 0x80000000u : 0u);
-    h1 |= (x2 == 0.f ? 0x8000u : 0u) | (x3 == 0.f ? 0x80000000u : 0u);
-    h = make_uint2(h0, h1);
-    m = make_uint2(m0, m1);
-    l = make_uint2(l0, l1);
-}
+
 template <int PF>
 __device__ __forceinline__ void plane4_to_f32(uint2 v, float (&o)[4]) {
     if constexpr (PF == PF_TRI) {
@@ -765,30 +739,15 @@
         const bool in = y >= 1 && y <= H && x >= 1 && x <= W;
         const float* p = src + (long)n * src_ns + (long)oc * 8 * HW + (in ? (long)(y - 1) * W + x - 1 : 0);
         uint4* o = dst + ((long)n * G + oc) * NS * PS + s;
-        if constexpr (PF == PF_TRI) {
-            float v[8];
-#pragma unroll
-            for (int e = 0; e < 8; ++e) v[e] = in ? p[e * HW] : 0.f;
-            uint2 h0, m0, l0, h1, m1, l1;
-            p24_split4(v[0], v[1], v[2], v[3], h0, m0, l0);
-            p24_split4(v[4], v[5], v[6], v[7], h1, m1, l1);
-            if (!in) { h0 = make_uint2(0, 0); h1 = h0; }
-            o[0] = make_uint4(h0.x, h0.y, h1.x, h1.y);
-            o[PS] = make_uint4(m0.x, m0.y, m1.x, m1.y);
-            o[2 * PS] = make_uint4(l0.x, l0.y, l1.x, l1.y);
-        } else {
-            pf16x8 h, m;
-#pragma unroll
-            for (int e = 0; e < 8; ++e) {
-                float v = in ? p[e * HW] : 0.f;
-                asm volatile("" : "+v"(v));
-                const _Float16 hh = (_Float16)v;
-                h[e] = in ? p16_head(v) : hh;
-                m[e] = (_Float16)(v - (float)hh);
-            }
-            o[0] = __builtin_bit_cast(uint4, h);
-            o[PS] = __builtin_bit_cast(uint4, m);
-        }
+        float v[8];
+#pragma unroll
+        for (int e = 0; e < 8; ++e) v[e] = in ? p[e * HW] : 0.f;
+        uint2 p0[NS], p1[NS];
+        plane_split4<PF>(v[0], v[1], v[2], v[3], p0);
+        plane_split4<PF>(v[4], v[5], v[6], v[7], p1);
+        if (!in) { p0[0] = make_uint2(0, 0); p1[0] = p0[0]; }
+#pragma unroll
+        for (int q = 0; q < NS; ++q) o[q * PS] = make_uint4(p0[q].x, p0[q].y, p1[q].x, p1[q].y);
     }
 }
 
diff --git a/textualdegremoval_amd/csrc/tdr_error.cpp b/textualdegremoval_amd/csrc/tdr_error.cpp
--- a/textualdegremoval_amd/csrc/tdr_error.cpp
+++ b/textualdegremoval_amd/csrc/tdr_error.cpp
@@ -9,4 +9,4 @@
     va_end(ap);
 }
 extern "C" const char* tdr_last_error(void) { return g_err; }
-extern "C" int tdr_version(void) { return 110; }
+extern "C" int tdr_version(void) { return 111; }
diff --git a/textualdegremoval_amd/csrc/tdr_plane_split.h b/textualdegremoval_amd/csrc/tdr_plane_split.h
--- /dev/null
+++ b/textualdegremoval_amd/csrc/tdr_plane_split.h
@@ -0,0 +1,61 @@
+#pragma once
+#include "tdr_common.h"
+
+namespace {
+
+enum { PF_TRI = 1, PF_PAIR = 2 };
+template <int PF> struct PlaneFmt { static constexpr int NS = PF == PF_TRI ? 3 : 2; };
+
+__device__ __forceinline__ _Float16 p16_head(float x) {
+    const _Float16 h = (_Float16)x;
+    return x == 0.f ? __builtin_bit_cast(_Float16, (unsigned short)0x8000) : h;
+}
+__device__ __forceinline__ bool p16_positive(_Float16 head) { return (__builtin_bit_cast(unsigned short, head) & 0x8000u) == 0; }
+__device__ __forceinline__ void p16_split4(float x0, float x1, float x2, float x3, uint2& h, uint2& m) {
+    unsigned h0, h1, m0, m1;
+    tdr_split2_f16(x0, x1, h0, m0);
+    tdr_split2_f16(x2, x3, h1, m1);
+    h0 |= (x0 == 0.f ? 0x8000u : 0u) | (x1 == 0.f ? 0x80000000u : 0u);
+    h1 |= (x2 == 0.f ? 0x8000u : 0u) | (x3 == 0.f ? 0x80000000u : 0u);
+    h = make_uint2(h0, h1);
+    m = make_uint2(m0, m1);
+}
+
+__device__ __forceinline__ void p24_split4(float x0, float x1, float x2, float x3, uint2& h, uint2& m, uint2& l) {
+    unsigned h0, h1, m0, m1, l0, l1;
+    tdr_split3_bf16(x0, x1, h0, m0, l0);
+    tdr_split3_bf16(x2, x3, h1, m1, l1);
+    h0 |= (x0 == 0.f ? 0x8000u : 0u) | (x1 == 0.f ? 0x80000000u : 0u);
+    h1 |= (x2 == 0.f ? 0x8000u : 0u) | (x3 == 0.f ? 0x80000000u : 0u);
+    h = make_uint2(h0, h1);
+    m = make_uint2(m0, m1);
+    l = make_uint2(l0, l1);
+}
+
+template <int PF>
+__device__ __forceinline__ void plane_split4(float x0, float x1, float x2, float x3, uint2 (&pl)[PlaneFmt<PF>::NS]) {
+    if constexpr (PF == PF_TRI) p24_split4(x0, x1, x2, x3, pl[0], pl[1], pl[2]);
+    else p16_split4(x0, x1, x2, x3, pl[0], pl[1]);
+}
+
+template <int NS, typename T>
+__device__ __forceinline__ void plane_zero_border(char* base, long PS, long Wp, int Y, int X, int HO, int WO) {
+    const bool top = Y == 0, bot = Y == HO - 1, lef = X == 0, rig = X == WO - 1;
+    if (top | bot | lef | rig) {
+        const T z{};
+        auto zero_at = [&](long sl) {
+#pragma unroll
+            for (int s = 0; s < NS; ++s) *reinterpret_cast<T*>(base + (s * PS + sl) * 16) = z;
+        };
+        if (top) zero_at(X + 1);
+        if (bot) zero_at((long)(HO + 1) * Wp + X + 1);
+        if (lef) zero_at((long)(Y + 1) * Wp);
+        if (rig) zero_at((long)(Y + 1) * Wp + WO + 1);
+        if (top && lef) zero_at(0);
+        if (top && rig) zero_at(WO + 1);
+        if (bot && lef) zero_at((long)(HO + 1) * Wp);
+        if (bot && rig) zero_at((long)(HO + 1) * Wp + WO + 1);
+    }
+}
+
+}
diff --git a/textualdegremoval_amd/engine.py b/textualdegremoval_amd/engine.py
--- a/textualdegremoval_amd/engine.py
+++ b/textualdegremoval_amd/engine.py
@@ -220,14 +220,14 @@
     return dout
 
 
-def conv_fwd(x, w, b, stride, pad, res=None, relu=False, out=None):
+def conv_fwd(x, w, b, stride, pad, res=None, relu=False, out=None, out16=None, want32=True):
     Cout, Cin, KH, _ = w.shape
     wp, mp, *_ = K.pack_weights(w, PACK_FWD)
-    out = K.conv_forward(x, wp, mp, Cout, KH, stride=stride, pad=pad, bias=b, res=res, relu=relu, out=out)
+    out = K.conv_forward(x, wp, mp, Cout, KH, stride=stride, pad=pad, bias=b, res=res, relu=relu, out=out, out16=out16, want32=want32)
     return out
 
 
-def conv_bwd(dout, x, w, stride, pad, need_dx=True, add_to_dx=None, bias=True, into=None):
+def conv_bwd(dout, x, w, stride, pad, need_dx=True, add_to_dx=None, bias=True, into=None, dx16=None, want_dx32=True):
     Cout, Cin, KH, _ = w.shape
 
     def leaf():
@@ -253,13 +253,15 @@
         N, _, OH, OW = dout.shape
         if stride == 1:
             wp, mp, *_ = K.pack_weights(w, PACK_DGRAD_S1)
-            dx = K.conv_forward(dout, wp, mp, Cin, KH, pad=KH - 1 - pad, res=add_to_dx)
+            dx = K.conv_forward(dout, wp, mp, Cin, KH, pad=KH - 1 - pad, res=add_to_dx, out16=dx16, want32=want_dx32)
+        elif dx16 is not None and not (KH == 3 and stride == 2 and pad == 1):
+            raise NotImplementedError(f'plane data gradient KH={KH} stride={stride} pad={pad}')
         elif KH == 2 and stride == 2 and pad == 0:
             wp, mp, *_ = K.pack_weights(w, PACK_DGRAD_2X2S2)
             dx = K.conv_forward(dout, wp, mp, 4 * Cin, 1, epi=EPI_PSHUF, res=add_to_dx)
         elif KH == 3 and stride == 2 and pad == 1:
             wp, mp, *_ = K.pack_weights(w, PACK_DGRAD_3X3S2)
-            dx = K.conv_forward(dout, wp, mp, 4 * Cin, 2, pad=0, OH=OH, OW=OW, epi=EPI_PSHUF, res=add_to_dx)
+            dx = K.conv_forward(dout, wp, mp, 4 * Cin, 2, pad=0, OH=OH, OW=OW, epi=EPI_PSHUF, res=add_to_dx, out16=dx16, want32=want_dx32)
         else:
             raise NotImplementedError(f'conv dgrad KH={KH} stride={stride} pad={pad}')
     L.maybe_join()
@@ -294,6 +296,7 @@
 
 P16_ON = True
 P16_MIN_C = None
+PLANE_EPILOGUE = True
 
 
 def _p16_level(Cc, n_blocks):
@@ -308,14 +311,22 @@
     for lvl in range(levels):
         k = lvl + 1
         xin = x
-        a = conv_fwd(xin, P[f'{pre}conv_L{k}.weight'], P[f'{pre}conv_L{k}.bias'], 1 if lvl == 0 else 2, 1, relu=True)
+        wL, bL, sL = P[f'{pre}conv_L{k}.weight'], P[f'{pre}conv_L{k}.bias'], 1 if lvl == 0 else 2
+        Cc = wL.shape[0]
+        a16 = None
+        if _p16_level(Cc, cnt[lvl]) and PLANE_EPILOGUE:
+            fmt = K.plane_fmt()
+            Ho, Wo = ((s + 2 - 3) // sL + 1 for s in xin.shape[-2:])
+            a16 = K.P16.empty(xin.shape[0], Cc, Ho, Wo, xin.device, fmt)
+            a = conv_fwd(xin, wL, bL, sL, 1, relu=True, out16=a16, want32=fmt != K.FMT_BX3)
+        else:
+            a = conv_fwd(xin, wL, bL, sL, 1, relu=True)
         blocks = []
         x = a
-        Cc = a.shape[1]
         if _p16_level(Cc, cnt[lvl]):
             fmt = K.plane_fmt()
             tri = fmt == K.FMT_BX3
-            x16, x32 = K.p16_from_f32(a, fmt=fmt), a
+            x16, x32 = (a16 if a16 is not None else K.p16_from_f32(a, fmt=fmt)), a
             for i in range(cnt[lvl]):
                 bp = f'{pre}blk_L{k}.{i}.'
                 wp1, mp1, *_ = K.pack_weights(P[bp + 'conv1.weight'], PACK_FWD)
@@ -338,7 +349,7 @@
                 x = o
         feats.append(x if not deep_only or lvl == levels - 1 else None)
         if keep:
-            saved.append((xin, a, blocks))
+            saved.append((xin, a16 if a16 is not None else a, blocks))
     return feats, (saved if keep else None)
 
 
@@ -352,14 +363,15 @@
 
 
 def _encoder_bwd_levels(dfeats, P, pre, cnt, saved, G, dnext):
+    dnext16 = None
     for lvl in reversed(range(len(dfeats))):
         k = lvl + 1
         xin, a, blocks = saved[lvl]
-        d = dnext if dnext is not None else dfeats[lvl]
-        if d is None:
+        d = dnext if (dnext is not None or dnext16 is not None) else dfeats[lvl]
+        if d is None and dnext16 is None:
             continue
         if blocks and isinstance(blocks[0][0], K.P16):
-            d16, d32 = K.p16_from_f32(d, fmt=blocks[0][0].fmt), d
+            d16, d32 = (dnext16 if dnext16 is not None else K.p16_from_f32(d, fmt=blocks[0][0].fmt)), d
             fmts = {t.fmt for bl in blocks for t in bl} | {d16.fmt}
             grouped = GROUP_LEAVES and 2 * cnt[lvl] > 1 and len(fmts) == 1
             late = []
@@ -412,8 +424,12 @@
                 d = K.conv_forward(dh, wp, mp, Cc, 3, pad=1, res=d, mask=a if i == 0 else None)
         dpre = d if cnt[lvl] > 0 else K.relu_bwd(d, a)
         w = P[f'{pre}conv_L{k}.weight']
+        dnext16, below = None, saved[lvl - 1][2] if lvl > 0 else None
+        if PLANE_EPILOGUE and below and isinstance(below[0][0], K.P16):
+            dnext16 = K.P16.empty(*xin.shape, xin.device, below[0][0].fmt)
         dnext, G[f'{pre}conv_L{k}.weight'], G[f'{pre}conv_L{k}.bias'] = conv_bwd(
-            dpre, xin, w, 1 if lvl == 0 else 2, 1, need_dx=(lvl > 0), add_to_dx=dfeats[lvl - 1] if lvl > 0 else None)
+            dpre, xin, w, 1 if lvl == 0 else 2, 1, need_dx=(lvl > 0), add_to_dx=dfeats[lvl - 1] if lvl > 0 else None,
+            dx16=dnext16, want_dx32=dnext16 is None or dnext16.fmt != K.FMT_BX3)
     L.maybe_join()
     return None
 
diff --git a/textualdegremoval_amd/kernels.py b/textualdegremoval_amd/kernels.py
--- a/textualdegremoval_amd/kernels.py
+++ b/textualdegremoval_amd/kernels.py
@@ -399,7 +399,7 @@
 
 def conv_forward(x, wp, Mpad, Cout, KH, stride=1, dil=1, pad=0, OH=None, OW=None, out=None, Cin=None, epi=EPI_STD,
                  gate=False, kscale=None, wp_ns=0, bias=None, scale=None, bias2=None, bias2_mul=1.0, res=None,
-                 mask=None, aux=None, relu=False):
+                 mask=None, aux=None, relu=False, out16=None, want32=True):
     lib = _lib.load()
     N, Cx, H, W = x.shape
     if Cin is None:
@@ -407,7 +407,11 @@
     if OH is None:
         OH = (H + 2 * pad - dil * (KH - 1) - 1) // stride + 1
         OW = (W + 2 * pad - dil * (KH - 1) - 1) // stride + 1
-    if out is None:
+    oshape = (N, Cout // 4, 2 * OH, 2 * OW) if epi == EPI_PSHUF else (N, Cout, OH, OW)
+    if out16 is not None:
+        assert epi != EPI_GATEBWD and (out16.N, out16.C, out16.H, out16.W) == oshape, 'plane destination of another shape'
+    assert want32 or out16 is not None
+    if out is None and want32:
         if epi == EPI_PSHUF:
             out = torch.empty(N, Cout // 4, 2 * OH, 2 * OW, dtype=torch.float32, device=x.device)
         elif epi == EPI_GATEBWD:
@@ -423,7 +427,10 @@
     d.kscale, d.kscale_ns = _p(kscale), _vec_ns(kscale)
     d.wp, d.wp_ns, d.Mpad = wp.data_ptr(), wp_ns, Mpad
     d.wp_fmt = getattr(wp, 'fmt', FMT_F32)
-    d.out, d.out_ns = out.data_ptr(), _dense_nchw(out)
+    if want32:
+        d.out, d.out_ns = out.data_ptr(), _dense_nchw(out)
+    if out16 is not None:
+        d.out16, d.out16_fmt = out16.data_ptr(), out16.fmt
     d.epi = epi
     d.bias, d.bias_ns = _p(bias), _vec_ns(bias)
     d.scale, d.scale_ns = _p(scale), _vec_ns(scale)
@@ -435,7 +442,9 @@
     if _survey is not None and d.wp_fmt in (FMT_HX2, FMT_H1):
         _survey.probe(x, 'grad' if BACKWARD_PHASE else 'fwd')
     check(lib.tdr_conv_forward(C.byref(d), _stream()), 'tdr_conv_forward')
-    return out
+    if _survey is not None and out16 is not None and out16.fmt == FMT_HX2:
+        _survey.probe(out if want32 else out16.to_f32(), 'grad' if BACKWARD_PHASE else 'fwd')
+    return out if want32 else None
 
 
 class P16:
```

Result: no change. 59.90 (median of 6 runs) (+0.4%).
